# withterm/term

Hardware: AMD Instinct MI355X
Metric: validated rows/sec, 16-col null+range+unique suite (higher is better)
Workload: dtype int64+f64; 1 GPU; 16-col (8 int64 + 8 float64, 12 nullable) null+range+unique suite: completeness x16, min/max/mean x16, uniqueness x2; rows_total=1000000000, rows_per_gpu=1000000000, cols=16, parallelism=row-range shards x1, HSA_ENABLE_IPC_MODE_LEGACY=0, suite_algorithmic_bytes=129500000000, verified=True

## Files before the change

term_amd/csrc/api_internal.h:

```cpp
#pragma once
#include <hip/hip_runtime.h>
#include <math.h>
#include <stdarg.h>
#include <stdio.h>
#include <stdlib.h>
#include <string.h>

#include <algorithm>
#include <atomic>
#include <condition_variable>
#include <mutex>
#include <thread>

#include "internal.h"
#include "kll_device.h"
#include "regex_device.h"
#include "side_check.h"
#include "spearman_device.h"
#include "timegap_device.h"

using namespace tgx;

typedef long double xdouble;
constexpr size_t kArenaBytes = 8u << 20;
constexpr size_t kArenaMaxBuffer = 256u << 10;
constexpr int64_t kCoalesceMaxRows = 1 << 16;
constexpr int64_t kCoalesceFlushRows = 4 << 20;
constexpr size_t kCoalesceFlushBatches = 4096;
constexpr size_t kCoalesceArenaMax = 128u << 20;
constexpr uint32_t kWireMagic = 0x53584754;
constexpr uint32_t kWireVersion = 3;

struct Context {
  std::mutex mu;
  bool inited = false;
  int device = -1;
  int n_cu = 256;
  uint64_t distinct_hint = 0;
  bool no_coalesce = false;
  char arch[64] = {0};
};
extern TGX_HIDDEN Context g_ctx;

struct BatchKeyFacts {
  bool range_known = false;
  int64_t lo = 0, hi = 0;
  bool device_keys = false;
  int64_t data_bytes = -1;
  bool sampled = false;
  DistinctSample sample;
};

struct NumericPrep {
  bool prepared = false;
  bool partitioned = false;
  uint32_t sub_bits = 0;
  bool key16 = false;
  uint64_t n_buckets = 0;
  bool range_known = false;
  int64_t lo = 0, hi = 0;
};

struct BatchTraits {
  bool any_host = false, any_utf8 = false;
  bool any_strings = false;
  bool coalescible = true;
  bool retained = false;
};

struct DistinctTotals {
  uint64_t total = 0, non_null = 0, distinct = 0, twice = 0, empty_rows = 0;
};
static inline void distinct_fold_totals(DistinctState &d, const DistinctTotals &t) {
  d.h_total += t.total;
  d.h_non_null += t.non_null;
  d.h_distinct += t.distinct - (t.empty_rows > 0 ? 1 : 0);
  d.h_twice += t.twice - (t.empty_rows > 1 ? 1 : 0);
  d.h_empty_rows += t.empty_rows;
}
struct Gathered {
  std::vector<ScanAcc> scan;
  std::vector<CountAcc> count;
  std::vector<ComomentAcc> como;
  std::vector<DistinctTotals> distinct;
  std::vector<std::vector<uint8_t>> hll;
};

struct WindowPrep {
  bool ok = true;
  int32_t vb_count = 0;
  int32_t vb_index[kGatherViewBufs];
  int64_t vb_min[kGatherViewBufs], vb_end[kGatherViewBufs];
  bool new_dict = false;
  int64_t dict_first = 0, dict_end = 0;
};

static inline bool is_numeric(int t) { return t == TGX_INT64 || t == TGX_FLOAT64; }
static inline bool is_numeric32(int t) { return t == TGX_INT32 || t == TGX_FLOAT32; }
static inline bool is_narrow_int(int t) { return (t >= TGX_INT8 && t <= TGX_UINT32) || t == TGX_BOOL; }
static inline bool is_widened(int t) { return is_numeric32(t) || is_narrow_int(t); }
static inline bool is_keys_only(int t) { return t == TGX_UINT64 || t == TGX_BOOL; }
static inline size_t narrow_bytes(int t, int64_t slots) {
  switch (t) {
    case TGX_INT8: case TGX_UINT8: return (size_t)slots;
    case TGX_INT16: case TGX_UINT16: return (size_t)slots * 2;
    case TGX_BOOL: return (size_t)((slots + 7) / 8);
    default: return (size_t)slots * 4;
  }
}
static inline int widened_type(int t) { return t == TGX_FLOAT32 ? TGX_FLOAT64 : TGX_INT64; }
static inline int widen_mode(int t) {
  switch (t) {
    case TGX_FLOAT32: return 1;
    case TGX_INT8: return 2;
    case TGX_INT16: return 3;
    case TGX_UINT8: return 4;
    case TGX_UINT16: return 5;
    case TGX_UINT32: return 6;
    case TGX_BOOL: return 7;
    default: return 0;
  }
}
static inline bool is_string(int t) { return t == TGX_UTF8 || t == TGX_LARGE_UTF8; }
static inline bool is_any_string(int t) { return is_string(t) || t == TGX_UTF8_VIEW; }

TGX_HIDDEN void copy_pool_shutdown();
TGX_HIDDEN void coalesce_drop(tgx_state *st);
TGX_HIDDEN ScanAcc scan_acc_identity();
TGX_HIDDEN void host_two_sum(double &s, double &c, double x);
TGX_HIDDEN void scan_acc_merge(ScanAcc &a, const ScanAcc &b);
TGX_HIDDEN xdouble como_sum(const ComomentAcc &a, int k);
TGX_HIDDEN void como_store(ComomentAcc &a, int k, xdouble v);
TGX_HIDDEN void como_rebase(ComomentAcc &b, double px, double py);
TGX_HIDDEN void como_acc_merge(ComomentAcc &a, const ComomentAcc &b_in);
TGX_HIDDEN void state_init_host(tgx_state *st, const tgx_plan *plan);
TGX_HIDDEN void prof_resolve(tgx_state *st);
TGX_HIDDEN tgx_status distinct_totals(tgx_state *st, size_t slot, DistinctTotals *t, tgx_error *err,
                                  const unsigned long long *pre = nullptr);
TGX_HIDDEN tgx_status gather(tgx_state *st, Gathered *g, tgx_error *err);
TGX_HIDDEN double key_to_double(int64_t k);
TGX_HIDDEN double i128_to_double(uint64_t lo, int64_t hi);
TGX_HIDDEN void fill_stats(const ScanAcc &a, bool variance, tgx_result *r);
TGX_HIDDEN double hll_sigma(double x);
TGX_HIDDEN double hll_tau(double x);
TGX_HIDDEN uint64_t hll_estimate(const std::vector<uint8_t> &regs);
TGX_HIDDEN tgx_status stage_column(tgx_state *st, const tgx_column &c, tgx_column *out, tgx_error *err,
                               bool widen32 = true);
TGX_HIDDEN void fill_scan_desc(const tgx_column &c, bool variance, const double *pivot, ScanColDesc *d);
TGX_HIDDEN int scan_blocks_for(const ScanColDesc &d, int n_cols_in_launch, int per_cu = 8);
TGX_HIDDEN tgx_status como_pivots(tgx_state *st, const ComomentLaunch &L, int n_pairs, tgx_error *err);
TGX_HIDDEN tgx_status update_validate(const tgx_plan *plan, tgx_state *st, const tgx_column *columns, size_t n_columns,
                                  int64_t *nrows_out, BatchTraits *traits, tgx_error *err);
TGX_HIDDEN tgx_status update_impl(const tgx_plan *plan, tgx_state *st, const tgx_column *columns, int64_t nrows,
                              tgx_error *err, const std::vector<BatchKeyFacts> *facts = nullptr);
TGX_HIDDEN tgx_status coalesce_append(const tgx_plan *plan, tgx_state *st, const tgx_column *columns, int64_t nrows,
                                  const BatchTraits &traits, bool *taken, tgx_error *err);
TGX_HIDDEN tgx_status distinct_read_counters(tgx_state *st, DistinctState &ds, unsigned long long *out,
                                         tgx_error *err);
TGX_HIDDEN tgx_status distinct_tuple_update(tgx_state *st, size_t slot, const tgx_column *dev, tgx_error *err,
                                        const tgx_column *orig = nullptr);
TGX_HIDDEN tgx_status distinct_prepare_numeric(tgx_state *st, size_t slot, const tgx_column &c,
                                           const BatchKeyFacts &facts, NumericPrep *prep, tgx_error *err);
TGX_HIDDEN tgx_status distinct_update(tgx_state *st, size_t slot, const tgx_column &c, const BatchKeyFacts &facts,
                                  const NumericPrep &prep, tgx_error *err,
                                  const std::vector<DictGather> *gathers = nullptr, int stats_slot = -1,
                                  const tgx_column *orig = nullptr);
TGX_HIDDEN tgx_status pinned_readback(tgx_state *st, size_t bytes, tgx_error *err);
TGX_HIDDEN tgx_status distinct_sample_all(tgx_state *st, const tgx_column *dev, std::vector<BatchKeyFacts> &facts,
                                      tgx_error *err);
TGX_HIDDEN void stream_copy(void *dst, const void *src, size_t bytes);
TGX_HIDDEN void host_minmax_i64_plain(const int64_t *v, const uint8_t *validity, int64_t bit0, int64_t n, int64_t *lo,
                                  int64_t *hi);
TGX_HIDDEN void host_minmax_i64(const int64_t *v, const uint8_t *validity, int64_t bit0, int64_t n, int64_t *lo, int64_t *hi);
TGX_HIDDEN tgx_status coalesce_arena_ready(tgx_state *st, tgx_error *err);
TGX_HIDDEN tgx_status coalesce_prepare_window(const tgx_column &c, int64_t nrows, const CoalesceColumn &cc, int col,
                                          WindowPrep *w, tgx_error *err);
TGX_HIDDEN size_t coalesce_host_bytes(const tgx_plan *plan, const tgx_column *columns, int64_t nrows,
                                  const std::vector<WindowPrep> &prep);
TGX_HIDDEN tgx_status coalesce_release_set(tgx_state *st, int set, tgx_error *err);
```

term_amd/csrc/distinct_state.cpp:

```cpp
#include "api_internal.h"

tgx_status distinct_read_counters(tgx_state *st, DistinctState &ds, unsigned long long *out,
                                         tgx_error *err) {
  memset(out, 0, kNumDistinctCounters * sizeof(unsigned long long));
  if (!ds.counters.p) return TGX_OK;
  HIP_TRY(hipMemcpyAsync(out, ds.counters.p, kNumDistinctCounters * sizeof(unsigned long long),
                         hipMemcpyDeviceToHost, st->stream));
  HIP_TRY(hipStreamSynchronize(st->stream));
  return TGX_OK;
}

tgx_status pinned_readback(tgx_state *st, size_t bytes, tgx_error *err) {
  if (bytes <= st->h_pinned_cap) return TGX_OK;
  pinned_free(st->h_pinned, st->h_pinned_cap);
  st->h_pinned = nullptr;
  st->h_pinned_cap = 0;
  const size_t want = std::max<size_t>(bytes + bytes / 2, 4096);
  HIP_TRY(pinned_alloc(&st->h_pinned, want));
  st->h_pinned_cap = want;
  return TGX_OK;
}

namespace {

// ... 326 lines not shown
  FpLists l1, l2;
  uint32_t *fb_lo = nullptr;
  TGX_TRY(fp_lists_stage(st, ds, c.length, true, &l1, &l2, &fb_lo, err));
  ProfScope ps(st, "distinct", 0), ps_lists(st, "distinct_lists", 0);
  unsigned long long *counters = ds.counters.as<unsigned long long>();
  const Utf8ColDesc d = utf8_desc(kept, kept.variadic, st->plan->fp_key, false);
  launch_fp_partition_utf8(d, l1, fb_lo, counters, st->stream);
  launch_fp_partition_lists(l1, l2, counters, st->stream);
  if (ds.exact)
    launch_fp_count_exact_utf8(l2, mult ? 1 : 0, ds.fp_per_list.as<uint2>(), l1.offered, d, counters, st->stream);
  else
    launch_fp_count(l2, mult ? 1 : 0, ds.fp_per_list.as<uint2>(), l1.offered, counters, st->stream);
  ds.retained.push_back(kept);
  return TGX_OK;
}

tgx_status fp_lists_tuple_update(tgx_state *st, size_t slot, const TupleDesc &d,
                                        const std::vector<const tgx_column *> &cols, tgx_error *err) {
  DistinctState &ds = st->distinct[slot];
  const bool mult = st->plan->distinct[slot].multiplicity;
  FpLists l1, l2;
  uint32_t *fb_lo = nullptr;
  TGX_TRY(fp_lists_stage(st, ds, d.length, true, &l1, &l2, &fb_lo, err));
  ProfScope ps(st, "distinct", 0), ps_lists(st, "distinct_lists", 0);
  unsigned long long *counters = ds.counters.as<unsigned long long>();
  launch_fp_partition_tuples(d, l1, fb_lo, counters, st->stream);
  launch_fp_partition_lists(l1, l2, counters, st->stream);
  if (ds.exact)
    launch_fp_count_exact_tuple(l2, mult ? 1 : 0, ds.fp_per_list.as<uint2>(), d, counters, st->stream);
  else
    launch_fp_count(l2, mult ? 1 : 0, ds.fp_per_list.as<uint2>(), nullptr, counters, st->stream);
  for (const tgx_column *c : cols) ds.retained.push_back(*c);
  return TGX_OK;
}

}

tgx_status distinct_tuple_update(tgx_state *st, size_t slot, const tgx_column *dev, tgx_error *err,
                                        const tgx_column *orig) {
  const DistinctTask &task = st->plan->distinct[slot];
  DistinctState &ds = st->distinct[slot];
  std::vector<const tgx_column *> cols;
  bool any_view = false;
  for (int c2 : task.tuple) {
    cols.push_back(&dev[c2]);
    any_view |= dev[c2].type == TGX_UTF8_VIEW || (orig && is_widened(orig[c2].type));
  }
  TupleDesc d;
  TGX_TRY(tuple_desc_of(st, cols, task.multiplicity, &d, err));
  ds.col_type = TGX_UTF8;
  ds.total_rows += d.length;
  if (d.length == 0) return TGX_OK;
  if (ds.fp_staged) TGX_TRY(distinct_resolve(st, slot, err));
  bool exact_lists_ok = orig != nullptr && d.length < (int64_t)1 << 32;
  if (orig)
    for (int c2 : task.tuple) exact_lists_ok &= orig[c2].mem == TGX_MEM_DEVICE && !is_widened(orig[c2].type);
  if (ds.mode == DistinctMode::kUndecided && !any_view && (!ds.exact || exact_lists_ok) && fp_lists_fit_rows(d.length))
    return fp_lists_tuple_update(st, slot, d, cols, err);
  if (ds.mode == DistinctMode::kUndecided) {
    ds.mode = DistinctMode::kHash;
    ds.wide = true;
  }
  ProfScope ps(st, "distinct", 0);
  return table_insert_tuple(st, slot, d, err);
}

namespace {

void bitmap_shape(const DistinctState &ds, int64_t length, bool mult, uint32_t *sub_bits_out, bool *key16_out,
                         uint64_t *n_buckets_out, bool *partitioned_out) {
  const uint64_t bucket_target = mult ? 1024 : 256;
  uint32_t sub_bits = 14;
  while (sub_bits < (mult ? 19u : 20u) && ((ds.range + (1ull << sub_bits) - 1) >> sub_bits) > bucket_target) sub_bits++;
  const bool key16 = !mult && sub_bits <= 16;
  const uint64_t n_buckets = (ds.range + (1ull << sub_bits) - 1) >> sub_bits;
  uint64_t cap_slots = (uint64_t)length / std::max<uint64_t>(n_buckets, 1);
  cap_slots = cap_slots + cap_slots / 4 + 16 * (((uint64_t)length >> 15) + 1) + 4096;
  *sub_bits_out = sub_bits;
  *key16_out = key16;
  *n_buckets_out = n_buckets;
  const char *min_env = getenv("TGX_PARTITION_MIN_ROWS");
  const int64_t min_rows = min_env ? std::max<int64_t>(1, atoll(min_env)) : (int64_t)1 << 20;
  *partitioned_out = length >= min_rows && n_buckets <= kMaxPartitions && (uint64_t)length * 64 >= ds.range &&
                     cap_slots < (1ull << 32) - 64;
}

bool distinct_wants_sample(const DistinctState &ds, const BatchKeyFacts &facts, const tgx_column &c) {
  return ds.mode == DistinctMode::kUndecided && c.type == TGX_INT64 && !ds.has_hint && !facts.range_known &&
         !ds.remembered && c.length >= (1 << 16);
}
bool distinct_wants_exact_range(const DistinctState &ds, const BatchKeyFacts &facts, const tgx_column &c) {
  if (!facts.device_keys || c.type != TGX_INT64 || ds.has_hint || facts.range_known || c.length < (1 << 16))
    return false;
  return ds.mode == DistinctMode::kUndecided ||
         (ds.mode == DistinctMode::kBitmap && ds.speculative && !ds.partitioned && !ds.outliers_possible);
}

}

tgx_status distinct_sample_all(tgx_state *st, const tgx_column *dev, std::vector<BatchKeyFacts> &facts,
                               tgx_error *err) {
  const tgx_plan *plan = st->plan;
  std::vector<size_t> who;
  for (size_t q = 0; q < plan->distinct.size(); q++) {
    const DistinctTask &t = plan->distinct[q];
    if (!t.tuple.empty() || !is_numeric(dev[t.column].type) || dev[t.column].length == 0) continue;
    bool lane = false;
    for (size_t h = 0; h < plan->hll.size(); h++)
      lane |= plan->hll[h].distinct_slot == (int)q && st->hll_mode[h] == 1;
    if (lane) continue;
    if (distinct_wants_sample(st->distinct[q], facts[q], dev[t.column]) ||
        distinct_wants_exact_range(st->distinct[q], facts[q], dev[t.column]))
      who.push_back(q);
  }
  if (who.empty()) return TGX_OK;
  TGX_TRY(pinned_readback(st, who.size() * sizeof(DistinctSample), err));
  DistinctSample *got = (DistinctSample *)st->h_pinned;
  for (size_t k = 0; k < who.size(); k++) {
    DistinctState &ds = st->distinct[who[k]];
    const tgx_column &c = dev[plan->distinct[who[k]].column];
    DistinctColDesc d = numeric_desc(c, false);
    d.pad = distinct_wants_exact_range(ds, facts[who[k]], c) ? 1 : 0;
    HIP_TRY(ds.sample.reserve(sizeof(DistinctSample)));
    launch_distinct_init(ds.sample.as<DistinctSample>(), nullptr, st->stream);
    launch_distinct_sample(d, ds.sample.as<DistinctSample>(), st->stream);
    HIP_TRY(hipMemcpyAsync(&got[k], ds.sample.p, sizeof(DistinctSample), hipMemcpyDeviceToHost, st->stream));
  }
  HIP_TRY(hipStreamSynchronize(st->stream));
  for (size_t k = 0; k < who.size(); k++) {
    BatchKeyFacts &kf = facts[who[k]];
    if (distinct_wants_exact_range(st->distinct[who[k]], kf, dev[plan->distinct[who[k]].column])) {
      if (got[k].count) {
        kf.range_known = true;
        kf.lo = got[k].min_v;
        kf.hi = got[k].max_v;
      }
      continue;
    }
    kf.sample = got[k];
    kf.sampled = true;
  }
  return TGX_OK;
}

namespace {

tgx_status bitmap_grow(tgx_state *st, DistinctState &ds, bool mult, int64_t lo, int64_t hi, int64_t incoming,
                              tgx_error *err) {
  const uint64_t old_top = (uint64_t)ds.base + (ds.range - 1);
  auto u = [](int64_t v) { return (uint64_t)v ^ 0x8000000000000000ull; };
  const bool below = u(lo) < u(ds.base), above = u(hi) > u((int64_t)old_top);
  if (!below && !above) return TGX_OK;
  constexpr uint64_t kSlice = 1ull << 20;
  uint64_t add_below = 0, add_above = 0;
  if (below) {
    const uint64_t need = u(ds.base) - u(lo);
    add_below = (std::max(need, ds.range) + kSlice - 1) / kSlice * kSlice;
    if (add_below > u(ds.base)) add_below = u(ds.base) / kSlice * kSlice;
    if (add_below < need) return TGX_OK;
  }
  if (above) {
    const uint64_t need = u(hi) - u((int64_t)old_top);
    add_above = std::max(need, ds.range);
    const uint64_t room = 0xFFFFFFFFFFFFFFFFull - u((int64_t)old_top);
    if (add_above > room) add_above = room;
    if (add_above < need) return TGX_OK;
  }
  auto sum3 = [](uint64_t a, uint64_t b, uint64_t c, uint64_t *out) {
    uint64_t t = 0;
    return !__builtin_add_overflow(a, b, &t) && !__builtin_add_overflow(t, c, out);
  };
  uint64_t new_range = 0;
  const bool fits = sum3(ds.range, add_below, add_above, &new_range);
  const uint64_t rows_seen = (uint64_t)std::max<int64_t>(ds.total_rows + incoming, 1);
  if (!fits || new_range >= (1ull << 34) || new_range / 16 > std::max<uint64_t>(rows_seen, g_ctx.distinct_hint)) {
    add_below = below ? ((u(ds.base) - u(lo)) + kSlice - 1) / kSlice * kSlice : 0;
    add_above = above ? u(hi) - u((int64_t)old_top) : 0;
    uint64_t tight = 0;
    if (!sum3(ds.range, add_below, add_above, &tight)) return TGX_OK;
    if (tight >= (1ull << 34) || tight / 16 > std::max<uint64_t>(rows_seen, g_ctx.distinct_hint)) return TGX_OK;
  }
  const uint64_t range = ds.range + add_below + add_above;
  const size_t old_words = (size_t)ds.bitmap_words;
  const size_t words = (size_t)(((range + kSlice - 1) >> 20) << 15) + 4;
  const size_t shift_words = (size_t)(add_below >> 5);
  auto regrow = [&](DevBuf &buf) -> tgx_status {
    DevBuf bigger;
    HIP_TRY(bigger.reserve(words * 4));
    HIP_TRY(hipMemsetAsync(bigger.p, 0, words * 4, st->stream));
    HIP_TRY(hipMemcpyAsync((uint32_t *)bigger.p + shift_words, buf.p, old_words * 4, hipMemcpyDeviceToDevice, st->stream));
    st->parked.emplace_back(std::move(buf));
    buf = std::move(bigger);
    return TGX_OK;
  };
  TGX_TRY(regrow(ds.seen));
  if (mult) TGX_TRY(regrow(ds.twice));
  ds.base = (int64_t)((uint64_t)ds.base - add_below);
  ds.range = range;
  ds.bitmap_words = words - 4;
  return TGX_OK;
}

}

tgx_status distinct_prepare_numeric(tgx_state *st, size_t slot, const tgx_column &c, const BatchKeyFacts &facts,
                                    NumericPrep *prep, tgx_error *err) {
  const DistinctTask &task = st->plan->distinct[slot];
  DistinctState &ds = st->distinct[slot];
  const bool mult = task.multiplicity;
  prep->prepared = true;
  prep->partitioned = false;
  prep->range_known = facts.range_known;
  prep->lo = facts.lo;
  prep->hi = facts.hi;
  if (ds.mode == DistinctMode::kUndecided) {
    bool have_range = false;
    int64_t lo = 0, hi = 0;
    if (c.type == TGX_INT64 && ds.has_hint) {
      have_range = true;
      lo = ds.hint_lo;
      hi = ds.hint_hi;
    } else if (c.type == TGX_INT64 && facts.range_known) {
      have_range = true;
      lo = facts.lo;
      hi = facts.hi;
    } else if (c.type == TGX_INT64 && ds.remembered && c.length >= (1 << 16)) {
      have_range = true;
      lo = ds.remembered_lo;
      hi = ds.remembered_hi;
    } else if (distinct_wants_sample(ds, facts, c)) {
      DistinctSample got = facts.sample;
      if (!facts.sampled) {
        HIP_TRY(ds.sample.reserve(sizeof(DistinctSample)));
        launch_distinct_init(ds.sample.as<DistinctSample>(), nullptr, st->stream);
        launch_distinct_sample(numeric_desc(c, false), ds.sample.as<DistinctSample>(), st->stream);
        HIP_TRY(hipMemcpyAsync(&got, ds.sample.p, sizeof(got), hipMemcpyDeviceToHost, st->stream));
        HIP_TRY(hipStreamSynchronize(st->stream));
      }
      if (got.count == 0 && c.length > 65536) {
        DistinctColDesc d = numeric_desc(c, false);
        d.pad = 1;
        HIP_TRY(ds.sample.reserve(sizeof(DistinctSample)));
        launch_distinct_init(ds.sample.as<DistinctSample>(), nullptr, st->stream);
        launch_distinct_sample(d, ds.sample.as<DistinctSample>(), st->stream);
        HIP_TRY(hipMemcpyAsync(&got, ds.sample.p, sizeof(got), hipMemcpyDeviceToHost, st->stream));
        HIP_TRY(hipStreamSynchronize(st->stream));
      }
      if (got.count == 0) return TGX_OK;
      have_range = true;
      lo = got.min_v;
      hi = got.max_v;
    }
    bool use_bitmap = false;
    if (c.type == TGX_INT64 && have_range) {
      uint64_t width = (uint64_t)hi - (uint64_t)lo;
      uint64_t expect = std::max<uint64_t>((uint64_t)c.length, g_ctx.distinct_hint);
      if (width < (1ull << 34) && width / 16 <= expect) {
        uint64_t slack = ds.has_hint ? 0 : std::min<uint64_t>(width / 64 + 4096, 1ull << 30);
        int64_t base = (lo < INT64_MIN + (int64_t)slack) ? INT64_MIN : lo - (int64_t)slack;
        uint64_t top = (hi > INT64_MAX - (int64_t)slack) ? (uint64_t)INT64_MAX : (uint64_t)(hi + (int64_t)slack);
        ds.base = base;
        ds.range = top - (uint64_t)base + 1;
        use_bitmap = true;
      }
    }
    if (use_bitmap) {
      size_t words = (size_t)(((ds.range + (1u << 20) - 1) >> 20) << 15) + 4;
      ds.bitmap_words = words - 4;
      if (ds.seen.cap < words * 4 && ds.spare_seen.cap >= words * 4) std::swap(ds.seen, ds.spare_seen);
      if (ds.twice.cap < words * 4 && ds.spare_twice.cap >= words * 4) std::swap(ds.twice, ds.spare_twice);
      HIP_TRY(ds.seen.reserve(words * 4));
      HIP_TRY(hipMemsetAsync(ds.seen.p, 0, words * 4, st->stream));
      if (mult) {
        HIP_TRY(ds.twice.reserve(words * 4));
        HIP_TRY(hipMemsetAsync(ds.twice.p, 0, words * 4, st->stream));
      }
      ds.mode = DistinctMode::kBitmap;
      ds.speculative = !ds.has_hint;
      if (ds.speculative && !facts.range_known) {
        ds.remembered = true;
        ds.remembered_lo = lo;
        ds.remembered_hi = hi;
      }
    } else {
      ds.mode = DistinctMode::kHash;
      ds.remembered = false;
    }
  }
  if (ds.mode == DistinctMode::kBitmap && ds.speculative && !ds.partitioned && facts.range_known &&
      !ds.outliers_possible)
    TGX_TRY(bitmap_grow(st, ds, mult, facts.lo, facts.hi, c.length, err));
  if (ds.mode == DistinctMode::kBitmap && ds.speculative) {
    auto u = [](int64_t v) { return (uint64_t)v ^ 0x8000000000000000ull; };
    const bool covered = facts.range_known && u(facts.lo) >= u(ds.base) && u(facts.hi) - u(ds.base) < ds.range;
    if (!covered) ds.outliers_possible = true;
  }
  if (ds.mode == DistinctMode::kBitmap) {
    bitmap_shape(ds, c.length, mult, &prep->sub_bits, &prep->key16, &prep->n_buckets, &prep->partitioned);
    if (ds.partitioned) prep->partitioned = false;
  }
  return TGX_OK;
}

namespace {

tgx_status distinct_run_numeric(tgx_state *st, size_t slot, const tgx_column &c, const NumericPrep &prep,
                                       int stats_slot, tgx_error *err, const tgx_column *orig) {
  const DistinctTask &task = st->plan->distinct[slot];
  const tgx_column &keep = (orig && orig->mem == TGX_MEM_DEVICE && is_widened(orig->type)) ? *orig : c;
  DistinctState &ds = st->distinct[slot];
  const bool mult = task.multiplicity;
  const DistinctColDesc d = numeric_desc(c, mult);
  const uint64_t bytes = (uint64_t)c.length * 8 + (c.validity ? (uint64_t)(c.length + 7) / 8 : 0);
  if (ds.mode == DistinctMode::kUndecided) return TGX_OK;
  if (ds.mode == DistinctMode::kBitmap) {
    if (ds.speculative) ds.retained.push_back(keep);
    if (prep.partitioned) {
      PartitionParams pp;
      memset(&pp, 0, sizeof(pp));
      pp.values = c.values;
      pp.validity = c.validity;
      pp.offset = c.offset;
      pp.length = c.length;
      pp.base = ds.base;
      pp.range = ds.range;
      pp.sub_bits = prep.sub_bits;
      pp.n_buckets = (uint32_t)prep.n_buckets;
      const uint64_t tiles = ((uint64_t)c.length + kPartitionTile - 1) / kPartitionTile;
      pp.bucket0 = 0;
      pp.n_lists = pp.n_buckets;
      if (prep.range_known) {
        auto u = [](int64_t v) { return (uint64_t)v ^ 0x8000000000000000ull; };
        const uint64_t ub = u(ds.base);
        const uint64_t rlo = u(prep.lo) > ub ? u(prep.lo) - ub : 0;
        uint64_t rhi = u(prep.hi) > ub ? u(prep.hi) - ub : 0;
        rhi = std::min(rhi, ds.range - 1);
        if (rlo <= rhi) {
          pp.bucket0 = (uint32_t)(rlo >> pp.sub_bits);
          pp.n_lists = (uint32_t)(rhi >> pp.sub_bits) - pp.bucket0 + 1;
        }
      }
      const char *p20 = getenv("TGX_PACK20");
      const bool no_pack20 = p20 && atoi(p20) == 0;
      const bool pack20 = !prep.key16 && prep.sub_bits <= (mult ? 19u : 20u) && !no_pack20;
      uint64_t cap = (uint64_t)c.length / pp.n_lists;
      cap = cap + cap / 4 + (prep.key16 ? 32 : pack20 ? 24 : 16) * tiles + 4096;
      pp.cap = prep.key16 ? (cap + 31) & ~31ull : pack20 ? (cap + 23) / 24 * 24 : (cap + 15) & ~15ull;
      if (pp.cap >= (1ull << 32) - 64) return fail(err, TGX_INTERNAL, "distinct: list capacity out of range");
      pp.want_multiplicity = mult ? 1 : 0;
      pp.key16 = prep.key16 ? 1 : pack20 ? 2 : 0;
      pp.force_form = ds.remembered_form;
      HIP_TRY(ds.lists.reserve(prep.key16 ? (uint64_t)pp.n_lists * pp.cap * sizeof(uint16_t)
                               : pack20   ? (uint64_t)pp.n_lists * pp.cap / 3 * 8
                                          : (uint64_t)pp.n_lists * pp.cap * sizeof(uint32_t)));
      HIP_TRY(ds.cursors.reserve((2 * pp.n_buckets + 1) * sizeof(unsigned long long)));
      pp.lists = ds.lists.as<uint32_t>();
      pp.cursors = ds.cursors.as<unsigned long long>();
      pp.seen = ds.seen.as<uint32_t>();
      pp.twice = mult ? ds.twice.as<uint32_t>() : nullptr;
      const int grid = partition_grid(c.length, g_ctx.n_cu);
      if (stats_slot >= 0) {
        HIP_TRY(ds.stat_partials.reserve((size_t)(grid + 1) * sizeof(ScanPartial)));
        HIP_TRY(ds.outlier_stats.reserve(sizeof(OutlierStats)));
        pp.stats = ds.stat_partials.as<ScanPartial>();
        pp.outliers = ds.outlier_stats.as<OutlierStats>();
      }
      unsigned long long *cnt = ds.counters.as<unsigned long long>();
      static_assert(kCntDistinct == 0 && kCntTwice == 1, "partition_init_kernel clears the two totals together");
      launch_partition_init(pp, cnt + kCntDistinct, st->stream);
      {
        ProfScope ps(st, "distinct", bytes);
        launch_partition(pp, cnt, g_ctx.n_cu, st->stream);
        HIP_TRY(launch_bucket_apply(pp, cnt, st->stream));
      }
      if (stats_slot >= 0) {
        ScanLaunch L;
        memset(&L, 0, sizeof(L));
        L.cols[0].length = c.length;
        L.cols[0].is_float = 0;
        L.acc_index[0] = stats_slot;
        launch_scan_reduce_only(L, 1, grid, pp.stats, st->d_scan_acc.as<ScanAcc>(), st->stream, pp.outliers);
      }
    } else {
      ProfScope ps(st, "distinct", bytes);
      launch_distinct_bitmap(d, bitmap_view(ds), ds.counters.as<unsigned long long>(), st->stream);
    }
  } else {
    if (ds.fp_staged) TGX_TRY(distinct_resolve(st, slot, err));
    if (ds.capacity == 0 && fp_lists_fit(c)) {
      FpLists l1, l2;
      uint32_t *fb_lo = nullptr;
      TGX_TRY(fp_lists_stage(st, ds, c.length, false, &l1, &l2, &fb_lo, err));
      ProfScope ps(st, "distinct", bytes), ps_lists(st, "distinct_lists", 0);
      launch_key_lists(d, l1, l2, mult ? 1 : 0, ds.fp_per_list.as<uint2>(), ds.counters.as<unsigned long long>(),
                       st->stream);
      ds.retained.push_back(keep);
      return TGX_OK;
    }
    TGX_TRY(hash_ensure(st, ds, mult, (uint64_t)c.length, err));
    ProfScope ps(st, "distinct", bytes);
    launch_distinct_hash(d, hash_view(ds), ds.counters.as<unsigned long long>(), st->stream);
  }
  return TGX_OK;
}

tgx_status retained_numeric_view(tgx_state *st, const tgx_column &col, std::vector<std::unique_ptr<DevBuf>> &tmp,
                                        tgx_column *out, tgx_error *err) {
  *out = col;
  if (!is_widened(col.type)) return TGX_OK;
  const int64_t e0 = col.offset & ~(int64_t)63;
  const int64_t slots = col.offset - e0 + col.length;
  tmp.emplace_back(new DevBuf());
  DevBuf *w = tmp.back().get();
  HIP_TRY(w->reserve((size_t)slots * 8 + 16));
  launch_widen32((const uint8_t *)col.values + narrow_bytes(col.type, e0), w->p, slots, widen_mode(col.type), g_ctx.n_cu,
                 st->stream);
  out->type = widened_type(col.type);
  out->values = w->p;
  out->validity = col.validity ? col.validity + (e0 >> 3) : nullptr;
  out->offset = col.offset - e0;
  return TGX_OK;
}

}

tgx_status distinct_update(tgx_state *st, size_t slot, const tgx_column &c, const BatchKeyFacts &facts,
                           const NumericPrep &prep, tgx_error *err, const std::vector<DictGather> *gathers,
                           int stats_slot, const tgx_column *orig) {
  const DistinctTask &task = st->plan->distinct[slot];
  DistinctState &ds = st->distinct[slot];
  const bool mult = task.multiplicity;
  if (is_any_string(c.type)) {
    ds.col_type = c.type;
    ds.total_rows += c.length;
    if (c.length == 0) return TGX_OK;
    if (ds.fp_staged) TGX_TRY(distinct_resolve(st, slot, err));
    const bool exact_lists_ok = orig && orig->mem == TGX_MEM_DEVICE && c.length < (int64_t)1 << 32;
    if (ds.mode == DistinctMode::kUndecided && (!ds.exact || exact_lists_ok) && fp_lists_fit(c))
      return fp_lists_update(st, slot, c, err);
    if (ds.mode == DistinctMode::kUndecided) {
      ds.mode = DistinctMode::kHash;
      ds.wide = true;
    }
    ProfScope ps(st, "distinct", 0);
    return table_insert_utf8(st, slot, c, facts.data_bytes, err);
  }
  if (c.type == TGX_DICT32_UTF8) {
    const tgx_column &dict = *c.dictionary;
    ds.col_type = c.type;
    ds.total_rows += c.length;
    if (c.length == 0 || dict.length == 0) return TGX_OK;
    if (ds.mode == DistinctMode::kUndecided) {
      ds.mode = DistinctMode::kHash;
      ds.wide = true;
    }
    TGX_TRY(hash_ensure(st, ds, mult, (uint64_t)std::min<int64_t>(c.length, dict.length), err));
    const size_t uw = dict_usage_words(dict.length);
    HIP_TRY(ds.dict_usage.reserve(2 * uw * 4 + 16));
    const size_t scratch = dict_usage_scratch_bytes(c.length, dict.length, mult ? 1 : 0, g_ctx.n_cu);
    if (scratch)
      HIP_TRY(ds.dict_scratch.reserve(scratch));
    else
      HIP_TRY(hipMemsetAsync(ds.dict_usage.p, 0, 2 * uw * 4, st->stream));
    uint32_t *u_seen = ds.dict_usage.as<uint32_t>(), *u_twice = u_seen + uw;
    ProfScope ps(st, "distinct", 0);
    if (gathers && !gathers->empty() && scratch) {
      const uint8_t *hits[4];
      unsigned long long *pc[4];
      int32_t niv[4];
      const int k = (int)std::min<size_t>(gathers->size(), 4);
      for (int i = 0; i < k; i++) {
        hits[i] = (*gathers)[i].hits;
        pc[i] = (*gathers)[i].counters;
        niv[i] = (*gathers)[i].null_is_valid;
      }
      launch_dict_usage_fused((const int32_t *)c.values, c.validity, c.offset, c.length, dict.length, mult ? 1 : 0, k,
                              hits, pc, niv, u_seen, u_twice, ds.dict_scratch.as<uint32_t>(),
                              ds.counters.as<unsigned long long>(), g_ctx.n_cu, st->stream);
    } else {
      launch_dict_usage((const int32_t *)c.values, c.validity, c.offset, c.length, dict.validity, dict.offset,
                        dict.length, mult ? 1 : 0, u_seen, u_twice, ds.dict_scratch.as<uint32_t>(),
                        ds.counters.as<unsigned long long>(), g_ctx.n_cu, st->stream);
    }
    if (ds.exact) TGX_TRY(key_store_reserve_utf8(st, ds, dict, u_seen, facts.data_bytes, err));
    launch_dict_insert(utf8_desc(dict, nullptr, st->plan->fp_key, mult), u_seen, u_twice, hash_view(ds),
                       ds.counters.as<unsigned long long>(), st->stream);
    return TGX_OK;
  }
  if (!is_numeric(c.type))
    return fail(err, TGX_UNSUPPORTED, "DISTINCT on column type %d is not supported yet", c.type);
  ds.col_type = c.type;
  ds.total_rows += c.length;
  if (c.length == 0) return TGX_OK;
  NumericPrep ready = prep;
  if (!ready.prepared) TGX_TRY(distinct_prepare_numeric(st, slot, c, facts, &ready, err));
  return distinct_run_numeric(st, slot, c, ready, stats_slot, err, orig);
}

tgx_status tgx::distinct_resolve(tgx_state *st, size_t slot, tgx_error *err) {
  DistinctState &ds = st->distinct[slot];
  std::vector<std::unique_ptr<DevBuf>> widened;
  if (ds.fp_staged && st->device_ready) {
    const bool mult = st->plan->distinct[slot].multiplicity;
    unsigned long long c[kNumDistinctCounters];
    TGX_TRY(distinct_read_counters(st, ds, c, err));
    ds.fp_staged = false;
    const bool exact_lists = ds.fp_exact_lists;
    ds.fp_exact_lists = false;
    if (c[kCntOutOfRange] != 0 || (exact_lists && !ds.retained.empty())) {
      if (ds.retained.empty())
        return fail(err, TGX_INTERNAL, "distinct: overflowed fingerprint lists and no batch to redo");
      HIP_TRY(hipMemsetAsync(ds.counters.p, 0, kNumDistinctCounters * sizeof(unsigned long long), st->stream));
      const DistinctTask &task = st->plan->distinct[slot];
      if (!task.tuple.empty()) {
        std::vector<const tgx_column *> cols;
        for (const tgx_column &col : ds.retained) cols.push_back(&col);
        TupleDesc d;
        TGX_TRY(tuple_desc_of(st, cols, mult, &d, err));
        TGX_TRY(table_insert_tuple(st, slot, d, err));
      } else {
        for (const tgx_column &kept : ds.retained) {
          tgx_column col;
          TGX_TRY(retained_numeric_view(st, kept, widened, &col, err));
          if (ds.wide) {
            TGX_TRY(table_insert_utf8(st, slot, col, -1, err));
            continue;
          }
          TGX_TRY(hash_ensure(st, ds, mult, (uint64_t)col.length, err));
          launch_distinct_hash(numeric_desc(col, mult), hash_view(ds), ds.counters.as<unsigned long long>(), st->stream);
        }
      }
    } else if (exact_lists) {
      FpLists l1, l2;
      fp_views(ds, &l1, &l2);
      TGX_TRY(hash_ensure(st, ds, mult, c[kCntDistinct], err));
      unsigned long long cur = 0;
      HIP_TRY(hipMemcpyAsync(&cur, ds.key_cursor.p, sizeof(cur), hipMemcpyDeviceToHost, st->stream));
      HIP_TRY(hipStreamSynchronize(st->stream));
      TGX_TRY(key_store_ensure(st, ds, cur, 2 * (c[kCntDistinct] + 1), err));
      ds.key_words_ub = cur + 2 * (c[kCntDistinct] + 1);
      TGX_TRY(key_store_measure_begin(st, ds, (uint64_t)kFpFan * kFpFan * l2.cap, err));
      HIP_TRY(hipMemsetAsync(ds.counters.p, 0, 2 * sizeof(unsigned long long), st->stream));
      launch_fp_demote(l2, ds.fp_fb_lo.as<uint32_t>(), hash_view(ds), mult ? 1 : 0, ds.counters.as<unsigned long long>(),
                       st->stream);
    } else {
      FpLists l1, l2;
      fp_views(ds, &l1, &l2);
      TGX_TRY(hash_ensure(st, ds, mult, c[kCntDistinct], err));
      if (ds.wide)
        launch_fp_insert(l2, hash_view(ds), mult ? 1 : 0, st->stream);
      else
        launch_key_insert(l2, hash_view(ds), mult ? 1 : 0, st->stream);
    }
    HIP_TRY(hipStreamSynchronize(st->stream));
    ds.retained.clear();
    return TGX_OK;
  }
  if (!ds.speculative || ds.retained.empty() || !st->device_ready) {
    ds.retained.clear();
    return TGX_OK;
  }
  const bool mult = st->plan->distinct[slot].multiplicity;
  unsigned long long c[kNumDistinctCounters];
  TGX_TRY(distinct_read_counters(st, ds, c, err));
  const uint64_t n_out = c[kCntOutOfRange];
  if (n_out == 0 || ds.mode != DistinctMode::kBitmap) {
    ds.retained.clear();
    ds.outliers_possible = false;
    return TGX_OK;
  }
  const int64_t old_base = ds.base;
  const uint64_t old_range = ds.range;
  ds.remembered = false;
  TGX_TRY(bitmap_to_hash(st, ds, mult, n_out, err));
  TGX_TRY(hash_ensure(st, ds, mult, n_out, err));
  for (const tgx_column &kept : ds.retained) {
    tgx_column col;
    TGX_TRY(retained_numeric_view(st, kept, widened, &col, err));
    launch_distinct_outliers(numeric_desc(col, mult), old_base, old_range, hash_view(ds), ds.counters.as<unsigned long long>(), st->stream);
  }
  HIP_TRY(hipMemsetAsync(ds.counters.as<unsigned long long>() + kCntOutOfRange, 0, sizeof(unsigned long long), st->stream));
  HIP_TRY(hipStreamSynchronize(st->stream));
  ds.retained.clear();
  ds.speculative = false;
  return TGX_OK;
}

tgx_status tgx::distinct_resolve_all(tgx_state *st, tgx_error *err) {
  bool pending = false;
  for (auto &ds : st->distinct) pending |= (ds.speculative || ds.fp_staged) && !ds.retained.empty();
  if (!pending || !st->device_ready || !st->d_distinct_counters.p) {
    for (auto &ds : st->distinct) ds.retained.clear();
    return TGX_OK;
  }
  std::vector<unsigned long long> all(st->distinct.size() * kNumDistinctCounters);
  TGX_TRY(pinned_readback(st, all.size() * sizeof(unsigned long long), err));
  HIP_TRY(hipMemcpyAsync(st->h_pinned, st->d_distinct_counters.p, all.size() * sizeof(unsigned long long),
                         hipMemcpyDeviceToHost, st->stream));
  HIP_TRY(hipStreamSynchronize(st->stream));
  memcpy(all.data(), st->h_pinned, all.size() * sizeof(unsigned long long));
  for (size_t k = 0; k < st->distinct.size(); k++) {
    DistinctState &ds = st->distinct[k];
    if ((ds.speculative || ds.fp_staged) && !ds.retained.empty() &&
        (all[k * kNumDistinctCounters + kCntOutOfRange] != 0 || (ds.fp_staged && ds.fp_exact_lists)))
      TGX_TRY(distinct_resolve(st, k, err));
    else {
      ds.retained.clear();
      ds.outliers_possible = false;
    }
  }
  return TGX_OK;
}


namespace {
uint32_t host_owner_of(uint64_t key, uint32_t world) {
  uint64_t x = key ^ 0x9e3779b97f4a7c15ULL;
  x ^= x >> 30; x *= 0xbf58476d1ce4e5b9ULL; x ^= x >> 27; x *= 0x94d049bb133111ebULL; x ^= x >> 31;
  return (uint32_t)((x >> 32) % world);
}
}

tgx_status tgx::distinct_export_impl(tgx_state *st, size_t slot, uint32_t world,
                                       const void **device_records, uint64_t *counts, tgx_error *err) {
  TGX_TRY(coalesce_flush(st, err));
  DistinctState &ds = st->distinct[slot];
  const bool mult = st->plan->distinct[slot].multiplicity;
  TGX_TRY(state_init_device(st, err));
  TGX_TRY(distinct_resolve(st, slot, err));
  std::vector<unsigned long long> h_counts(world, 0);
  unsigned long long c[kNumDistinctCounters];
  TGX_TRY(distinct_read_counters(st, ds, c, err));
  const uint64_t empty_rows = c[kCntEmptyRows];
  HIP_TRY(ds.export_counts.reserve(2 * world * sizeof(unsigned long long)));
  unsigned long long *d_counts = ds.export_counts.as<unsigned long long>();
  unsigned long long *d_cursors = d_counts + world;
  HIP_TRY(hipMemsetAsync(d_counts, 0, 2 * world * sizeof(unsigned long long), st->stream));
  if (ds.mode == DistinctMode::kHash && ds.wide)
    launch_hash_export_count128(hash_view(ds), world, d_counts, st->stream);
  else if (ds.mode == DistinctMode::kHash)
    launch_hash_export_count(hash_view(ds), world, d_counts, st->stream);
  else if (ds.mode == DistinctMode::kBitmap)
    launch_bitmap_export_count(bitmap_view(ds), world, d_counts, st->stream);
  HIP_TRY(hipMemcpyAsync(h_counts.data(), d_counts, world * sizeof(unsigned long long), hipMemcpyDeviceToHost, st->stream));
  HIP_TRY(hipStreamSynchronize(st->stream));
  uint32_t empty_owner = 0;
  if (empty_rows > 0) {
    empty_owner = host_owner_of(kEmptyKey, world);
    h_counts[empty_owner] += 1;
  }
  std::vector<unsigned long long> starts(world, 0);
  uint64_t total = 0;
  for (uint32_t r = 0; r < world; r++) {
    starts[r] = total;
    total += h_counts[r];
  }
  const size_t rec_bytes = ds.wide ? sizeof(KeyRecord128) : sizeof(KeyRecord);
  HIP_TRY(ds.export_records.reserve(std::max<uint64_t>(total, 1) * rec_bytes));
  HIP_TRY(hipMemcpyAsync(d_cursors, starts.data(), world * sizeof(unsigned long long), hipMemcpyHostToDevice, st->stream));
  HIP_TRY(hipStreamSynchronize(st->stream));
  if (ds.mode == DistinctMode::kHash && ds.wide)
    launch_hash_export_scatter128(hash_view(ds), world, mult ? 1 : 0, d_cursors, ds.export_records.as<KeyRecord128>(),
                                  st->stream);
  else if (ds.mode == DistinctMode::kHash)
    launch_hash_export_scatter(hash_view(ds), world, mult ? 1 : 0, d_cursors, ds.export_records.as<KeyRecord>(), st->stream);
  else if (ds.mode == DistinctMode::kBitmap)
    launch_bitmap_export_scatter(bitmap_view(ds), world, mult ? 1 : 0, d_cursors, ds.export_records.as<KeyRecord>(), st->stream);
  if (empty_rows > 0) {
    KeyRecord rec{kEmptyKey, std::min<uint64_t>(empty_rows, 2)};
    uint64_t pos = starts[empty_owner] + h_counts[empty_owner] - 1;
    HIP_TRY(hipMemcpyAsync(ds.export_records.as<KeyRecord>() + pos, &rec, sizeof(rec), hipMemcpyHostToDevice, st->stream));
  }
  HIP_TRY(hipStreamSynchronize(st->stream));
  for (uint32_t r = 0; r < world; r++) counts[r] = h_counts[r];
  *device_records = ds.export_records.p;
  return TGX_OK;
}

extern "C" size_t tgx_distinct_record_bytes(const tgx_plan *plan, const tgx_state *st, size_t spec_index) {
  if (!plan || !st || st->plan != plan || spec_index >= plan->specs.size() ||
      plan->specs[spec_index].kind != TGX_CHECK_DISTINCT)
    return 0;
  return records_are_wide(st->distinct[plan->bind[spec_index].slot]) ? sizeof(KeyRecord128) : sizeof(KeyRecord);
}

extern "C" tgx_status tgx_distinct_export(const tgx_plan *plan, tgx_state *st, size_t spec_index,
                                          uint32_t world, const void **device_records, uint64_t *counts,
                                          tgx_error *err) try {
  bind_thread();
  size_t slot = 0;
  TGX_TRY(spec_slot(plan, st, spec_index, TGX_CHECK_DISTINCT, "DISTINCT", &slot, err));
  if (world == 0 || world > 256 || !device_records || !counts)
    return fail(err, TGX_INVALID_ARGUMENT, "bad arguments (world must be 1..256)");
  TGX_TRY(need_device(err));
  return distinct_export_impl(st, slot, world, device_records, counts, err);
} catch (...) {
  return tgx::abi_exception(err);
}

tgx_status tgx::distinct_import_records(tgx_state *st, size_t slot, const void *d_recs, uint64_t n, bool wide,
                                          tgx_error *err) {
  DistinctState &ds = st->distinct[slot];
  const bool mult = st->plan->distinct[slot].multiplicity;
  TGX_TRY(state_init_device(st, err));
  TGX_TRY(distinct_resolve(st, slot, err));
  if (ds.mode == DistinctMode::kBitmap) TGX_TRY(bitmap_to_hash(st, ds, mult, n, err));
  if (ds.mode == DistinctMode::kHash && ds.capacity > 0 && ds.wide != wide)
    return fail(err, TGX_INVALID_ARGUMENT, "distinct: cannot unite a Utf8 key set with a numeric one");
  ds.mode = DistinctMode::kHash;
  ds.wide = wide;
  TGX_TRY(hash_ensure(st, ds, mult, n, err));
  if (ds.exact && wide) {
    unsigned long long cur = 0;
    HIP_TRY(hipMemcpyAsync(&cur, ds.key_cursor.p, sizeof(cur), hipMemcpyDeviceToHost, st->stream));
    HIP_TRY(hipStreamSynchronize(st->stream));
    TGX_TRY(key_store_ensure(st, ds, cur, 2 * n, err));
    ds.key_words_ub = cur + 2 * n;
    TGX_TRY(key_store_measure_begin(st, ds, n, err));
  }
  if (wide)
    launch_hash_import128((const KeyRecord128 *)d_recs, n, hash_view(ds), mult ? 1 : 0,
                          ds.counters.as<unsigned long long>(), st->stream);
  else
    launch_hash_import((const KeyRecord *)d_recs, n, hash_view(ds), mult ? 1 : 0,
                       ds.counters.as<unsigned long long>(), st->stream);
  return TGX_OK;
}

tgx_status tgx::distinct_replace_by_records(tgx_state *st, size_t slot, const void *d_recs, uint64_t n, bool wide,
                                            tgx_error *err) {
  DistinctState &ds = st->distinct[slot];
  static_assert(kCntDistinct == 0 && kCntTwice == 1 && kCntEmptyRows == 2, "the three totals of the keys lie together");
  HIP_TRY(hipMemsetAsync(ds.counters.as<unsigned long long>() + kCntDistinct, 0, 3 * sizeof(unsigned long long),
                         st->stream));
  ds.capacity = 0;
  ds.rows_upper_bound = 0;
  ds.mode = DistinctMode::kHash;
  ds.wide = wide;
  TGX_TRY(distinct_import_records(st, slot, d_recs, n, wide, err));
  ds.partitioned = true;
  return TGX_OK;
}

extern "C" tgx_status tgx_distinct_import(const tgx_plan *plan, tgx_state *st, size_t spec_index,
                                          const void *device_records, uint64_t n_records, tgx_error *err) try {
  bind_thread();
  size_t slot = 0;
  TGX_TRY(spec_slot(plan, st, spec_index, TGX_CHECK_DISTINCT, "DISTINCT", &slot, err));
  TGX_TRY(need_device(err));
  TGX_TRY(coalesce_flush(st, err));
  DistinctState &ds = st->distinct[slot];
  TGX_TRY(state_init_device(st, err));
  const bool wide = records_are_wide(ds);
  HIP_TRY(hipStreamSynchronize(st->stream));
  ds.seen.release();
  ds.twice.release();
  ds.keys.release();
  ds.dup.release();
  static_assert(kCntValidRows + 1 == kCntOutOfRange, "the words behind the row counter");
  HIP_TRY(hipMemsetAsync(ds.counters.as<unsigned long long>() + kCntOutOfRange, 0,
                         (kNumDistinctCounters - kCntOutOfRange) * sizeof(unsigned long long), st->stream));
  TGX_TRY(distinct_replace_by_records(st, slot, device_records, n_records, wide, err));
  HIP_TRY(hipStreamSynchronize(st->stream));
  return TGX_OK;
} catch (...) {
  return tgx::abi_exception(err);
}

extern "C" tgx_status tgx_distinct_range_hint(const tgx_plan *plan, tgx_state *st, size_t spec_index, int64_t lo,
                                              int64_t hi, tgx_error *err) try {
  size_t slot = 0;
  TGX_TRY(spec_slot(plan, st, spec_index, TGX_CHECK_DISTINCT, "DISTINCT", &slot, err));
  TGX_TRY(coalesce_flush(st, err));
  DistinctState &ds = st->distinct[slot];
  if (ds.mode != DistinctMode::kUndecided)
    return fail(err, TGX_INVALID_ARGUMENT, "range hint must be given before the first batch (after tgx_state_reset)");
  if (hi < lo) return fail(err, TGX_INVALID_ARGUMENT, "range hint: hi < lo");
  ds.has_hint = true;
  ds.hint_lo = lo;
  ds.hint_hi = hi;
  return TGX_OK;
} catch (...) {
  return tgx::abi_exception(err);
}

extern "C" tgx_status tgx_distinct_bitmap_view(const tgx_plan *plan, tgx_state *st, size_t spec_index, int64_t *base,
                                               uint64_t *n_words, const void **seen, const void **twice,
                                               tgx_error *err) try {
  bind_thread();
  size_t slot = 0;
  TGX_TRY(spec_slot(plan, st, spec_index, TGX_CHECK_DISTINCT, "DISTINCT", &slot, err));
  TGX_TRY(coalesce_flush(st, err));
  TGX_TRY(distinct_resolve(st, slot, err));
  DistinctState &ds = st->distinct[slot];
  if (ds.mode != DistinctMode::kBitmap)
    return fail(err, TGX_UNSUPPORTED, "the key set is not a range bitmap; use tgx_distinct_export / _import");
  HIP_TRY(hipStreamSynchronize(st->stream));
  if (base) *base = ds.base;
  if (n_words) *n_words = ds.bitmap_words;
// ... 59 lines not shown
```

term_amd/csrc/internal.h:

```cpp
#pragma once
#include <hip/hip_runtime.h>
#include <stdint.h>
#include <stdio.h>

#include <atomic>
#include <deque>
#include <map>
#include <memory>
#include <new>
#include <stdexcept>
#include <string>
#include <vector>

#include "../../include/tgx.h"
#include "kernels/device_types.h"
#include "kernels/distinct_types.h"
#include "kll_host.h"

namespace tgx {

inline tgx_status abi_exception(tgx_error *err) {
  tgx_status code = TGX_INTERNAL;
  const char *what = "unknown C++ exception";
  try {
    throw;
  } catch (const std::bad_alloc &) {
    code = TGX_OUT_OF_MEMORY;
    what = "host allocation failed (std::bad_alloc)";
  } catch (const std::exception &e) {
    what = e.what();
  } catch (...) {
  }
  if (err) {
    err->code = (int32_t)code;
    snprintf(err->msg, sizeof(err->msg), "%s", what);
  }
  return code;
}

void launch_scan_pivot(const ScanLaunch &L, int n_cols, double *d_pivots, int32_t *d_pivot_set, PivotSearch *d_search,
                       hipStream_t stream);
void launch_scan_main_only(const ScanLaunch &L, int n_cols, int blocks_per_col, ScanPartial *d_partials,
                           ScanAcc *d_accs, hipStream_t stream);
void launch_scan_kll(const ScanLaunch &L, int n_cols, int blocks_per_col, size_t lds_bytes, ScanPartial *d_partials,
                     hipStream_t stream);
void launch_scan_pairs(const ScanPairLaunch &L, int n_pairs, int blocks_per_pair, size_t lds_bytes,
                       ScanPartial *d_partials, void *d_como_partials, const ComomentAcc *d_como_accs,
                       hipStream_t stream);
void launch_scan_hll(const ScanLaunch &L, int n_cols, int blocks_per_col, ScanPartial *d_partials, hipStream_t stream);
void launch_como_pivot(const ComomentLaunch &L, int n_pairs, ComomentAcc *d_accs, PivotSearch *d_search, hipStream_t stream);
void launch_comoments_reduce(const ComomentLaunch &L, int n_pairs, int blocks_per_pair, const void *d_partials,
                             ComomentAcc *d_accs, hipStream_t stream);
void launch_widen32(const void *src, void *dst, int64_t n, int mode, int n_cu, hipStream_t stream);
void launch_scan_reduce_only(const ScanLaunch &L, int n_cols, int blocks_per_col, ScanPartial *d_partials,
                             ScanAcc *d_accs, hipStream_t stream, const OutlierStats *outliers = nullptr);
void launch_count(const CountLaunch &L, int n_cols, int blocks_per_col, unsigned long long *d_block_counts,
                  CountAcc *d_accs, hipStream_t stream);
size_t comoments_partial_bytes();
void launch_comoments(const ComomentLaunch &L, int n_pairs, int blocks_per_pair, void *d_partials,
                      ComomentAcc *d_accs, hipStream_t stream);
void launch_distinct_hash(const DistinctColDesc &d, const HashSetView &t,
                          unsigned long long *d_counters, hipStream_t stream);
void launch_distinct_bitmap(const DistinctColDesc &d, const BitmapView &bm,
                            unsigned long long *d_counters, hipStream_t stream);
int partition_grid(int64_t length, int n_cu);
void launch_distinct_init(DistinctSample *sample, OutlierStats *outliers, hipStream_t stream);
void launch_partition_init(const PartitionParams &p, unsigned long long *totals, hipStream_t stream);
void launch_distinct_sample(const DistinctColDesc &d, DistinctSample *out, hipStream_t stream);
void launch_distinct_outliers(const DistinctColDesc &d, int64_t base, uint64_t range, const HashSetView &t,
                              unsigned long long *d_counters, hipStream_t stream);
void launch_partition(const PartitionParams &p, unsigned long long *d_counters, int n_cu, hipStream_t stream);
hipError_t launch_bucket_apply(const PartitionParams &p, unsigned long long *d_counters, hipStream_t stream);
void launch_bitmap_adopt(const uint32_t *seen_slices, const uint32_t *twice_slices, uint32_t n_slices,
                         uint64_t slice_words, uint64_t stride_words, uint32_t *out_seen, uint32_t *out_twice,
                         unsigned long long *d_counters, hipStream_t stream);
void launch_bitmap_rebase(const uint32_t *src, uint64_t src_words, long long delta_bits, uint32_t world,
                          uint64_t slice_words, uint64_t row_words, uint64_t col_words, uint32_t *send,
                          hipStream_t stream);
void launch_distinct_utf8(const Utf8ColDesc &d, const HashSetView &t, unsigned long long *d_counters,
                          hipStream_t stream);
void launch_exact_measure_utf8(const Utf8ColDesc &d, const uint32_t *dict_seen, unsigned long long *out,
                               hipStream_t stream);
void launch_exact_measure_tuple(const TupleDesc &d, unsigned long long *out, hipStream_t stream);
void launch_gather_segments(const GatherSeg *d_segs, int n_segs, int parts, hipStream_t stream);
void launch_state_reset(const StateResetArgs &a, hipStream_t stream);
int tgx_num_cus();
void launch_dict_count_hits(const int32_t *indices, const uint8_t *validity, int64_t offset, int64_t length,
                            int64_t dict_length, int dict_has_nulls, const uint8_t *hits, int null_is_valid,
                            unsigned long long *d_counters, int n_cu, hipStream_t stream);
void launch_dict_count(const int32_t *indices, const uint8_t *validity, int64_t offset, int64_t length,
                       const uint8_t *dict_validity, int64_t dict_offset, int64_t dict_length, CountAcc *acc, int n_cu,
                       hipStream_t stream);
int dict_fuse_capacity(int64_t length, int64_t dict_length, int want_mult, int n_cu);
void launch_dict_usage_fused(const int32_t *indices, const uint8_t *validity, int64_t offset, int64_t length,
                             int64_t dict_length, int want_mult, int n_patterns, const uint8_t *const *hits,
                             unsigned long long *const *pattern_counters, const int32_t *null_is_valid, uint32_t *seen,
                             uint32_t *twice, uint32_t *scratch, unsigned long long *d_counters, int n_cu,
                             hipStream_t stream);
size_t dict_usage_words(int64_t dict_length);
size_t dict_usage_scratch_bytes(int64_t length, int64_t dict_length, int want_mult, int n_cu);
void launch_dict_usage(const int32_t *indices, const uint8_t *validity, int64_t offset, int64_t length,
                       const uint8_t *dict_validity, int64_t dict_offset, int64_t dict_length, int want_mult,
                       uint32_t *seen, uint32_t *twice, uint32_t *scratch, unsigned long long *d_counters, int n_cu,
                       hipStream_t stream);
void launch_dict_insert(const Utf8ColDesc &d, const uint32_t *seen, const uint32_t *twice, const HashSetView &t,
                        unsigned long long *d_counters, hipStream_t stream);
void launch_distinct_tuple(const TupleDesc &d, const HashSetView &t, unsigned long long *d_counters,
                           hipStream_t stream);
void launch_fp_partition_utf8(const Utf8ColDesc &d, const FpLists &level1, uint32_t *exact_fb_lo,
                              unsigned long long *d_counters, hipStream_t stream);
void launch_fp_partition_tuples(const TupleDesc &d, const FpLists &level1, uint32_t *exact_fb_lo,
                                unsigned long long *d_counters, hipStream_t stream);
void launch_fp_count_exact_utf8(const FpLists &level2, int want_mult, uint2 *per_list, const uint32_t *offered1,
                                const Utf8ColDesc &d, unsigned long long *d_counters, hipStream_t stream);
void launch_fp_count_exact_tuple(const FpLists &level2, int want_mult, uint2 *per_list, const TupleDesc &d,
                                 unsigned long long *d_counters, hipStream_t stream);
void launch_fp_demote(const FpLists &level2, const uint32_t *fb_lo, const HashSetView &t, int want_mult,
                      unsigned long long *d_counters, hipStream_t stream);
void launch_fp_partition_lists(const FpLists &level1, const FpLists &level2, unsigned long long *d_counters,
                               hipStream_t stream);
void launch_fp_count(const FpLists &level2, int want_mult, uint2 *per_list, const uint32_t *offered1,
                     unsigned long long *d_counters, hipStream_t stream);
void launch_fp_insert(const FpLists &level2, const HashSetView &t, int want_mult, hipStream_t stream);
void launch_key_lists(const DistinctColDesc &d, const FpLists &level1, const FpLists &level2, int want_mult,
                      uint2 *per_list, unsigned long long *d_counters, hipStream_t stream);
void launch_key_insert(const FpLists &level2, const HashSetView &t, int want_mult, hipStream_t stream);
void launch_hash_rehash128(const HashSetView &src, const HashSetView &dst, int want_mult,
                           unsigned long long *d_counters, hipStream_t stream);
void launch_hash_import128(const KeyRecord128 *recs, uint64_t n, const HashSetView &dst, int want_mult,
                           unsigned long long *d_counters, hipStream_t stream);
void launch_hash_export_count128(const HashSetView &src, uint32_t world, unsigned long long *d_counts,
                                 hipStream_t stream);
void launch_hash_export_scatter128(const HashSetView &src, uint32_t world, int want_mult,
                                   unsigned long long *d_cursors, KeyRecord128 *out, hipStream_t stream);
void launch_hash_rehash(const HashSetView &src, const HashSetView &dst, int want_mult,
                        unsigned long long *d_counters, hipStream_t stream);
void launch_bitmap_to_hash(const BitmapView &bm, const HashSetView &dst, int want_mult,
                           unsigned long long *d_counters, hipStream_t stream);
void launch_hash_import(const KeyRecord *recs, uint64_t n, const HashSetView &dst, int want_mult,
                        unsigned long long *d_counters, hipStream_t stream);
void launch_hash_export_count(const HashSetView &src, uint32_t world, unsigned long long *d_counts,
                              hipStream_t stream);
void launch_hash_export_scatter(const HashSetView &src, uint32_t world, int want_mult,
                                unsigned long long *d_cursors, KeyRecord *out, hipStream_t stream);
void launch_bitmap_export_count(const BitmapView &bm, uint32_t world, unsigned long long *d_counts,
                                hipStream_t stream);
void launch_bitmap_export_scatter(const BitmapView &bm, uint32_t world, int want_mult,
                                  unsigned long long *d_cursors, KeyRecord *out, hipStream_t stream);

struct ScanTask {
  int column;
  bool variance;
  bool stats_needed = false;
  bool stats_spec = false;
  bool read_by_spec = false;
};
struct CountTask {
  int column;
};
struct DistinctTask {
  int column;
  bool multiplicity;
  int scan_slot;
  std::vector<int> tuple;
  bool approx_only = false;
  bool exact = false;
};
struct HllTask {
  int column;
  int scan_slot;
  int distinct_slot;
};
struct ComomentTask {
  int col_x, col_y;
};
struct KllTask {
  int column;
  uint32_t k;
};
struct JointTask {
  int col_x, col_y;
  bool binned;
  JointBinning binning;
};
struct TemporalTask {
  int column, column2, spec_index;
  bool set;
  uint32_t flags;
  TemporalParams params;
};
struct HistTask {
  int column;
  bool counted = false;
  std::vector<double> edges;
  uint32_t buckets() const { return counted ? (uint32_t)edges.size() - 1 : 0; }
};

struct ValueRuleTask {
  int column, spec_index, slot, leader;
  bool set;
  tgx_value_rule_params params;
};

struct ValueCountsTask {
  int column, spec_index;
  bool set;
  tgx_value_counts_params params;
};

struct PairCountsTask {
  int col_x, col_y, spec_index;
  bool set;
  tgx_pair_counts_params params;
};

constexpr int kGroupMaxTuple = 8;
struct GroupCountsTask {
  int column, group, spec_index, slot, leader, member;
  int n_tuple;
  int tuple[kGroupMaxTuple];
  bool set;
  tgx_group_counts_params params;
};

struct GroupSumsTask {
  int column, group, spec_index;
  int n_tuple;
  int tuple[kGroupMaxTuple];
  bool set;
  tgx_group_sums_params params;
};

enum KeyProbeMode : uint32_t {
  kKpPlain = 0, kKpCounted = 1, kKpStrings = 2, kKpRows = 3, kKpStringsCounted = 4, kKpRowsStrings = 5,
  kKpTuples = 6, kKpTuplesCounted = 7, kKpRowsTuples = 8
};
inline bool kp_string_set(KeyProbeMode m) { return m == kKpStrings || m == kKpStringsCounted; }
inline bool kp_counts(KeyProbeMode m) { return m == kKpCounted || m == kKpStringsCounted || m == kKpTuplesCounted; }
inline bool kp_gathers(KeyProbeMode m) { return m == kKpRows || m == kKpRowsStrings || m == kKpRowsTuples; }
inline bool kp_string_column(KeyProbeMode m) { return kp_string_set(m) || m == kKpRowsStrings; }
inline bool kp_tuples(KeyProbeMode m) { return m == kKpTuples || m == kKpTuplesCounted || m == kKpRowsTuples; }
inline bool kp_tuple_set(KeyProbeMode m) { return m == kKpTuples || m == kKpTuplesCounted; }
inline bool kp_fingerprint_set(KeyProbeMode m) { return kp_string_set(m) || kp_tuple_set(m); }
constexpr int kKeyProbeMaxTuple = 8;
struct KeyProbeTask {
  int column, spec_index;
  int n_tuple;
  int tuple[kKeyProbeMaxTuple];
  bool set;
  KeyProbeMode mode;
  uint32_t max_value_bytes;
  tgx_key_probe_params params;
};

constexpr int kRowPredicateMaxCols = 8;
struct RowPredicateTask {
  int spec_index;
  int n_columns;
  int columns[kRowPredicateMaxCols];
  bool set;
  tgx_row_predicate_params params;
};

struct TypeClassesTask {
  int column, spec_index;
};

struct SideCheck;
constexpr int kNumSide = 11;

enum class Source { kScan, kCount };

struct SpecBinding {
  int kind;
  int slot;
  Source count_src;
};

}

struct tgx_plan {
  std::vector<tgx_check_spec> specs;
  std::vector<std::string> patterns;
  std::vector<tgx::SpecBinding> bind;
  std::vector<tgx::ScanTask> scan;
  std::vector<tgx::CountTask> count;
  std::vector<tgx::DistinctTask> distinct;
  std::vector<tgx::ComomentTask> como;
  std::vector<tgx::KllTask> kll;
  std::vector<tgx::HllTask> hll;
  std::vector<tgx::JointTask> joint;
  std::vector<tgx::TemporalTask> temporal;
  std::vector<tgx::HistTask> hist;
  std::vector<tgx::ValueRuleTask> rules;
  std::vector<tgx::ValueCountsTask> value_counts;
  std::vector<tgx::PairCountsTask> pair_counts;
  std::vector<tgx::GroupCountsTask> group_counts;
  std::vector<tgx::GroupSumsTask> group_sums;
  std::vector<tgx::KeyProbeTask> key_probes;
  std::vector<tgx::RowPredicateTask> row_predicates;
  std::vector<tgx::TypeClassesTask> type_classes;
  int n_columns_needed = 0;
  std::vector<char> used, reads_values, needs_wide;
  std::vector<char> key_column;
  std::vector<char> side_on[tgx::kNumSide];
  std::vector<char> stats_on;
  tgx::FpKey fp_key;
  mutable std::atomic<bool> fp_key_locked{false};
  void *regex = nullptr;
  void *spearman = nullptr;
  void *timegap = nullptr;
  std::vector<char> timegap_on;
};

namespace tgx {

size_t cache_size_class(size_t bytes);
hipError_t dev_alloc(void **p, size_t *cap, size_t bytes);
void dev_free(void *p, size_t cap);
hipError_t pinned_alloc(void **p, size_t bytes);
void pinned_free(void *p, size_t bytes);
hipError_t stream_acquire(hipStream_t *out, bool high_priority);
void stream_release(hipStream_t s, bool high_priority);
void dev_cache_trim();
void dev_cache_set_live(bool on);
void dev_cache_stats(tgx_cache_stats *out);
struct QuiescedScope {
  QuiescedScope();
  ~QuiescedScope();
  QuiescedScope(const QuiescedScope &) = delete;
  QuiescedScope &operator=(const QuiescedScope &) = delete;
};

struct DevBuf {
  void *p = nullptr;
  size_t cap = 0;
  bool owned = true;
  DevBuf() = default;
  DevBuf(const DevBuf &) = delete;
  DevBuf &operator=(const DevBuf &) = delete;
  DevBuf(DevBuf &&o) noexcept : p(o.p), cap(o.cap), owned(o.owned) {
    o.p = nullptr;
    o.cap = 0;
    o.owned = true;
  }
  DevBuf &operator=(DevBuf &&o) noexcept {
    if (this != &o) {
      release();
      p = o.p;
      cap = o.cap;
      owned = o.owned;
      o.p = nullptr;
      o.cap = 0;
      o.owned = true;
    }
    return *this;
  }
  ~DevBuf() { release(); }
  void release() {
    if (p && owned) dev_free(p, cap);
    p = nullptr;
    cap = 0;
    owned = true;
  }
  void borrow(void *ptr, size_t bytes) {
    release();
    p = ptr;
    cap = bytes;
    owned = false;
  }
  hipError_t reserve(size_t bytes) {
    if (bytes <= cap) return hipSuccess;
    release();
    return dev_alloc(&p, &cap, bytes);
  }
// ... 309 lines not shown
```

term_amd/csrc/kernels/distinct_types.h:

```cpp
#pragma once
#include <stdint.h>

namespace tgx {

constexpr uint64_t kEmptyKey = 0xFFFFFFFFFFFFFFFFULL;

struct DistinctColDesc {
  const void *values;
  const uint8_t *validity;
  int64_t offset;
  int64_t length;
  int32_t want_multiplicity;
  int32_t pad;
};

struct HashSetView {
  uint64_t *keys;
  uint32_t *dup;
  uint64_t mask;
  uint64_t *store;
  unsigned long long *store_cursor;
  uint64_t store_words;
  uint64_t *pending;
  uint32_t *pending_counts;
  uint64_t pending_region;
  uint32_t pending_waves, pad_;
};
inline uint32_t exact_blocks(uint64_t items) {
  uint64_t blocks = (items + 255) / 256;
  if (blocks < 1) blocks = 1;
  if (blocks > 2048) blocks = 2048;
  return (uint32_t)blocks;
}
inline uint32_t exact_waves(uint64_t items) { return exact_blocks(items) * 4; }
inline uint64_t exact_region(uint64_t items) {
  const uint64_t threads = (uint64_t)exact_blocks(items) * 256;
  return (items + threads - 1) / threads * 64;
}

struct FpKey {
  uint32_t k[4], k1[4], k2[4];
};
inline void fp_key_times_two(const uint32_t in[4], uint32_t out[4]) {
  const uint32_t carry = (in[3] >> 31) ? 0x87u : 0u;
  out[3] = (in[3] << 1) | (in[2] >> 31);
  out[2] = (in[2] << 1) | (in[1] >> 31);
  out[1] = (in[1] << 1) | (in[0] >> 31);
  out[0] = (in[0] << 1) ^ carry;
}
inline FpKey fp_key_expand(const uint32_t k[4]) {
  FpKey key;
  for (int i = 0; i < 4; i++) key.k[i] = k[i];
  fp_key_times_two(key.k, key.k1);
  fp_key_times_two(key.k1, key.k2);
  return key;
}

struct Utf8ColDesc {
  const void *offsets;
  const uint8_t *data;
  const uint8_t *validity;
  int64_t offset;
  int64_t length;
  int32_t large_offsets;
  int32_t want_multiplicity;
  const void *views;
  const uint8_t *const *buffers;
  FpKey key;
};

struct BitmapView {
  uint32_t *seen;
  uint32_t *twice;
  int64_t base;
  uint64_t range;
};

constexpr uint32_t kMaxPartitions = 2048;
constexpr uint32_t kListPad = 0xFFFFFFFFu;
constexpr int kRunPad4 = 16, kRunPad2 = 32;
constexpr int kPartitionThreads = 1024;
constexpr int kPartitionKeysPerThread = 32;
constexpr int kPartitionTile = kPartitionThreads * kPartitionKeysPerThread;
constexpr int kSliceWordsLds = 32768;

struct PartitionParams {
  const void *values;
  const uint8_t *validity;
  int64_t offset;
  int64_t length;
  int64_t base;
  uint64_t range;
  uint32_t sub_bits;
  uint32_t n_buckets;
  uint64_t cap;
  uint32_t *lists;
  unsigned long long *cursors;
  uint32_t *seen;
  uint32_t *twice;
  int32_t want_multiplicity;
  int32_t key16;
  struct ScanPartial *stats;
  struct OutlierStats *outliers;
  uint32_t bucket0, n_lists;
  int32_t force_form;
};

struct OutlierStats {
  long long mn, mx;
  unsigned long long lo32_sum;
  long long hi32_sum;
  unsigned long long count;
};

struct DistinctSample {
  int64_t min_v, max_v;
  unsigned long long count;
  unsigned long long pad;
};

struct KeyRecord {
  uint64_t key;
  uint64_t count;
};

struct KeyRecord128 {
  uint64_t a, b;
  uint64_t count;
  uint64_t pad;
};

constexpr int kFpFan = 256;
constexpr int kFpXcds = 8;
constexpr int kFpTile = 2048;
constexpr uint32_t kFpSlots = 4096;
constexpr uint32_t kFpListMax = 24576;
constexpr int64_t kFpMinRows = 1 << 21;
struct FpLists {
  uint64_t *recs;
  uint32_t *offered;
  uint64_t cap;
};

enum {
  kCntDistinct = 0,
  kCntTwice = 1,
  kCntEmptyRows = 2,
  kCntValidRows = 3,
  kCntOutOfRange = 4,
  kCntSpare = 5,
  kCntStoreFull = 6,
  kCntForm = 7,
  kNumDistinctCounters = 8
};

struct TupleCol {
  int32_t kind;
  int32_t dict_large;
  const void *values;
  const void *offsets;
  const uint8_t *data;
  const uint8_t *const *buffers;
  const uint8_t *validity;
  int64_t offset;
  const uint8_t *dict_validity;
  int64_t dict_offset;
};
constexpr int kMaxTupleCols = 8;
struct TupleDesc {
  TupleCol cols[kMaxTupleCols];
  int32_t n_cols;
  int32_t want_multiplicity;
  int64_t length;
  FpKey key;
};
struct KeyProbeTupleDesc {
  TupleDesc d;
  int64_t dict_length[kMaxTupleCols];
};

}
```

term_amd/csrc/kernels/partition.hip:

```cpp
#include <hip/hip_runtime.h>

#include <type_traits>

#include "device_types.h"
#include "distinct_types.h"
#include "keyset_device.h"

namespace tgx {

template <int THREADS, int KPT, bool VALIDITY>
__device__ __forceinline__ void partition_load_tile(const PartitionParams &p, int64_t tile, bool wide,
                                                    int64_t (&key)[KPT], uint32_t &ok) {
  constexpr int kPartitionThreads = THREADS;
  constexpr int kTile = kPartitionThreads * KPT;
  global_i64_ptr vals = (global_i64_ptr)(uintptr_t)((const int64_t *)p.values + p.offset);
  global_u8_ptr vbits = VALIDITY ? (global_u8_ptr)(uintptr_t)p.validity : (global_u8_ptr) nullptr;
  const uint32_t tid = threadIdx.x;
  const int64_t row0 = tile * kTile;
  const bool full = row0 + kTile <= p.length;
  ok = 0;
  if (full && wide) {
    typedef long long i64x2 __attribute__((ext_vector_type(2)));
    typedef const i64x2 __attribute__((address_space(1))) *global_i64x2_ptr;
    global_i64x2_ptr pv = (global_i64x2_ptr)(vals + row0) + tid;
    const bool pair_bytes = vbits && (p.offset & 1) == 0;
    ok = (uint32_t)((1ull << KPT) - 1ull);
    if (pair_bytes) {
      uint8_t vb[KPT / 2];
#pragma unroll
      for (int j = 0; j < KPT / 2; j++) {
        const int64_t bit = p.offset + row0 + (int64_t)j * 2 * kPartitionThreads + 2 * tid;
        vb[j] = vbits[bit >> 3];
      }
      ok = 0;
#pragma unroll
      for (int j = 0; j < KPT / 2; j++) {
        const int64_t bit = p.offset + row0 + (int64_t)j * 2 * kPartitionThreads + 2 * tid;
        ok |= (uint32_t)((vb[j] >> (bit & 7)) & 3) << (2 * j);
      }
    } else if (vbits) {
      ok = 0;
#pragma unroll
      for (int j = 0; j < KPT; j++) {
        const int64_t bit = p.offset + row0 + (int64_t)(j / 2) * 2 * kPartitionThreads + 2 * tid + (j & 1);
        ok |= (uint32_t)TGX_VALID_BIT(vbits, bit) << j;
      }
    }
    if (VALIDITY) asm volatile("" : "+v"(ok));
#pragma unroll
    for (int j = 0; j < KPT / 2; j++) {
      i64x2 v = pv[(int64_t)j * kPartitionThreads];
      key[2 * j] = v.x;
      key[2 * j + 1] = v.y;
    }
  } else {
#pragma unroll
    for (int j = 0; j < KPT; j++) {
      const int64_t i = row0 + (int64_t)j * kPartitionThreads + tid;
      const bool in = i < p.length;
      key[j] = vals[in ? i : p.length - 1];
      bool valid = in;
      if (in && vbits) {
        const int64_t bit = p.offset + i;
        valid = TGX_VALID_BIT(vbits, bit);
      }
      ok |= (uint32_t)valid << j;
    }
  }
}

template <int THREADS, int KPT, int MAXP, int PAD, bool KEY16, bool PACK20, bool CLUSTERED, class MidFn, class StoreFn>
__device__ __forceinline__ void partition_process_tile(const PartitionParams &p, uint32_t *sorted, uint32_t *hist,
                                                       uint32_t *toff, uint32_t *gbase, uint32_t *wave_sums,
                                                       uint32_t *long_runs, const uint32_t (&rel)[KPT], uint64_t ok,
                                                       MidFn &&mid,
                                                       StoreFn &&before_stores) {
  constexpr uint32_t NW = THREADS / 64;
  constexpr int BPT = MAXP / THREADS;
  constexpr int NS = MAXP / (NW * 64);
  static_assert(MAXP % THREADS == 0 && MAXP % (NW * 64) == 0 && PAD % 4 == 0, "shape");
  constexpr uint32_t RPAD = PACK20 ? 24u : KEY16 ? (uint32_t)kRunPad2 : (uint32_t)PAD;
  auto pad_up = [](uint32_t h) -> uint32_t { return PACK20 ? (h + 23u) / 24u * 24u : (h + (RPAD - 1u)) & ~(RPAD - 1u); };
  const bool fill = p.want_multiplicity != 0;
  auto pack6 = [&](uint32_t o, uint32_t h, uint32_t i) -> uint4 {
    uint64_t w[2];
    if (!fill) {
#pragma unroll
      for (int q = 0; q < 2; q++) {
        const uint32_t i0 = i + 3u * q;
        const uint64_t a = sorted[o + (i0 < h ? i0 : h - 1)], b = sorted[o + (i0 + 1 < h ? i0 + 1 : h - 1)],
                       c = sorted[o + (i0 + 2 < h ? i0 + 2 : h - 1)];
        w[q] = a | (b << 20) | (c << 40);
      }
    } else {
#pragma unroll
      for (int q = 0; q < 2; q++) {
        uint64_t e[3];
#pragma unroll
        for (uint32_t j = 0; j < 3; j++) {
          const uint32_t at = i + 3u * q + j;
          e[j] = at < h ? (uint64_t)sorted[o + at] : 0xFFFFFull;
        }
        w[q] = e[0] | (e[1] << 20) | (e[2] << 40);
      }
    }
    return make_uint4((uint32_t)w[0], (uint32_t)(w[0] >> 32), (uint32_t)w[1], (uint32_t)(w[1] >> 32));
  };
  const uint32_t tid = threadIdx.x;
  const uint32_t lane = tid & 63, wave = tid >> 6;
  const uint32_t sub_mask = (uint32_t)((1ull << p.sub_bits) - 1);
  for (uint32_t b = tid; b < (uint32_t)MAXP; b += THREADS) hist[b] = 0;
  constexpr uint32_t kLongRun = 1024, kMaxLongRuns = THREADS * KPT / kLongRun;
  if (CLUSTERED && tid == 0) long_runs[kMaxLongRuns] = 0;
  __syncthreads();
  bool whole = false;
  if (CLUSTERED) {
    uint32_t agreed = 0;
#pragma unroll
    for (int j = 0; j < KPT; j++) {
      const bool okj = (ok >> j) & 1;
      const uint32_t b = rel[j] >> p.sub_bits;
      const uint64_t act = __ballot(okj);
      const uint32_t first = act ? (uint32_t)__builtin_ctzll(act) : 0u;
      const uint32_t b0 = (uint32_t)__builtin_amdgcn_readlane((int)b, (int)first);
      agreed |= (__ballot(okj && b != b0) == 0 ? 1u : 0u) << j;
    }
    whole = agreed == (uint32_t)((1ull << KPT) - 1ull);
  }
  if (CLUSTERED && whole) {
#pragma unroll
    for (int j = 0; j < KPT; j++) {
      const uint64_t act = __ballot((ok >> j) & 1);
      const uint32_t first = act ? (uint32_t)__builtin_ctzll(act) : 64u;
      if (lane == first) atomicAdd(&hist[rel[j] >> p.sub_bits], (uint32_t)__builtin_popcountll(act));
    }
  } else {
#pragma unroll
    for (int j = 0; j < KPT; j++)
      if ((ok >> j) & 1) atomicAdd(&hist[rel[j] >> p.sub_bits], 1u);
  }
  __syncthreads();
  {
    uint32_t h[BPT], sum = 0;
#pragma unroll
    for (int k = 0; k < BPT; k++) {
      h[k] = hist[BPT * tid + k];
      sum += h[k];
    }
    uint32_t incl = sum;
#pragma unroll
    for (int d = 1; d < 64; d <<= 1) {
      uint32_t up = __shfl_up(incl, d, 64);
      if (lane >= (uint32_t)d) incl += up;
    }
    if (lane == 63) wave_sums[wave] = incl;
    __syncthreads();
    uint32_t excl = incl - sum;
    for (uint32_t w = 0; w < wave; w++) excl += wave_sums[w];
#pragma unroll
    for (int k = 0; k < BPT; k++) {
      const uint32_t b = BPT * tid + k;
      toff[b] = excl;
      hist[b] = excl;
      uint32_t g = 0;
      if (h[k] && b - p.bucket0 >= p.n_lists) {
        g = 0xFFFFFFFFu;
      } else if (h[k]) {
        const unsigned long long padded = pad_up(h[k]);
        const unsigned long long at = atomicAdd(&p.cursors[b], padded);
        if (at + padded > p.cap) {
          atomicMin(&p.cursors[p.n_buckets + b], at);
          g = 0xFFFFFFFFu;
        } else {
          g = (uint32_t)at;
          if (CLUSTERED && h[k] >= kLongRun) long_runs[atomicAdd(&long_runs[kMaxLongRuns], 1u)] = b;
        }
      }
      gbase[b] = g;
      excl += h[k];
    }
    if (tid == THREADS - 1) toff[MAXP] = excl;
  }
  __syncthreads();
  __builtin_amdgcn_sched_barrier(0);
  mid();
  __builtin_amdgcn_sched_barrier(0);
  if (CLUSTERED && whole) {
#pragma unroll
    for (int j = 0; j < KPT; j++) {
      const bool okj = (ok >> j) & 1;
      const uint64_t act = __ballot(okj);
      const uint32_t first = act ? (uint32_t)__builtin_ctzll(act) : 64u;
      uint32_t at = 0;
      if (lane == first) at = atomicAdd(&hist[rel[j] >> p.sub_bits], (uint32_t)__builtin_popcountll(act));
      at = (uint32_t)__builtin_amdgcn_readlane((int)at, (int)(first & 63u));
      const uint32_t before =
          __builtin_amdgcn_mbcnt_hi((uint32_t)(act >> 32), __builtin_amdgcn_mbcnt_lo((uint32_t)act, 0u));
      if (okj) sorted[at + before] = rel[j] & sub_mask;
    }
  } else {
#pragma unroll
    for (int j = 0; j < KPT; j++) {
      if (!((ok >> j) & 1)) continue;
      const uint32_t pos = atomicAdd(&hist[rel[j] >> p.sub_bits], 1u);
      sorted[pos] = rel[j] & sub_mask;
    }
  }
  __syncthreads();
  __builtin_amdgcn_sched_barrier(0);
  before_stores();
  __builtin_amdgcn_sched_barrier(0);
  {
    uint32_t m_o[NS], m_h[NS], m_g[NS];
#pragma unroll
    for (int s2 = 0; s2 < NS; s2++) {
      const uint32_t b = (lane + 64 * s2) * NW + wave;
      const bool in = b < p.n_buckets;
      const uint32_t o = in ? toff[b] : 0;
      m_o[s2] = o;
      m_h[s2] = in ? toff[b + 1] - o : 0;
      m_g[s2] = in ? gbase[b] : 0;
    }
    const uint32_t n_meta = (p.n_buckets > wave) ? (p.n_buckets - wave + NW - 1) / NW : 0;
    constexpr uint32_t LPB = (KEY16 || PACK20) ? 4u : 16u, BPS = 64u / LPB, KPL = PACK20 ? 6u : KEY16 ? 8u : 4u;
    const uint32_t grp = lane / LPB, sub = lane % LPB;
#pragma unroll
    for (int s2 = 0; s2 < NS; s2++) {
      const uint32_t m_end = n_meta > 64u * s2 ? (n_meta - 64u * s2 < 64u ? n_meta - 64u * s2 : 64u) : 0;
      for (uint32_t m0 = 0; m0 < m_end; m0 += BPS) {
        const uint32_t m = m0 + grp, src = m & 63;
        const uint32_t o = __shfl(m_o[s2], src, 64), g = __shfl(m_g[s2], src, 64);
        uint32_t h = __shfl(m_h[s2], src, 64);
        if (m >= m_end) h = 0;
        if (CLUSTERED && h >= kLongRun && g != 0xFFFFFFFFu) h = 0;
        if (h == 0) continue;
        const uint32_t b = (m + 64 * s2) * NW + wave;
        if (g != 0xFFFFFFFFu) {
          const uint32_t padded = pad_up(h);
          if (PACK20) {
            uint8_t *dst = (uint8_t *)p.lists + ((uint64_t)(b - p.bucket0) * p.cap + g) / 3 * 8;
            for (uint32_t i = KPL * sub; i < padded; i += KPL * LPB) *(uint4 *)(dst + (uint64_t)(i / 3) * 8) = pack6(o, h, i);
          } else if (KEY16) {
            uint16_t *dst = (uint16_t *)p.lists + (uint64_t)(b - p.bucket0) * p.cap + g;
            for (uint32_t i = KPL * sub; i < padded; i += KPL * LPB) {
              uint32_t k8[8];
#pragma unroll
              for (uint32_t j = 0; j < 8; j++) k8[j] = sorted[o + (i + j < h ? i + j : h - 1)];
              uint4 v;
              v.x = k8[0] | (k8[1] << 16);
              v.y = k8[2] | (k8[3] << 16);
              v.z = k8[4] | (k8[5] << 16);
              v.w = k8[6] | (k8[7] << 16);
              *(uint4 *)&dst[i] = v;
            }
          } else {
            uint32_t *dst = p.lists + (uint64_t)(b - p.bucket0) * p.cap + g;
            for (uint32_t i = KPL * sub; i < padded; i += KPL * LPB) {
              uint4 v;
              v.x = i < h ? sorted[o + i] : kListPad;
              v.y = i + 1 < h ? sorted[o + i + 1] : kListPad;
              v.z = i + 2 < h ? sorted[o + i + 2] : kListPad;
              v.w = i + 3 < h ? sorted[o + i + 3] : kListPad;
              *(uint4 *)&dst[i] = v;
            }
          }
        } else {
          for (uint32_t i = sub; i < h; i += LPB) {
            const uint64_t r = ((uint64_t)b << p.sub_bits) | sorted[o + i];
            const uint32_t bit = 1u << (r & 31);
            const uint32_t prev = atomicOr(&p.seen[r >> 5], bit);
            if ((prev & bit) && p.want_multiplicity) atomicOr(&p.twice[r >> 5], bit);
          }
        }
      }
    }
  }
  if (CLUSTERED) {
    const uint32_t n_long = long_runs[kMaxLongRuns];
    for (uint32_t q = 0; q < n_long; q++) {
      const uint32_t b = long_runs[q];
      const uint32_t o = toff[b], h = toff[b + 1] - o, g = gbase[b];
      const uint32_t padded = pad_up(h);
      if (PACK20) {
        uint8_t *dst = (uint8_t *)p.lists + ((uint64_t)(b - p.bucket0) * p.cap + g) / 3 * 8;
        for (uint32_t i = 6u * tid; i < padded; i += 6u * THREADS) *(uint4 *)(dst + (uint64_t)(i / 3) * 8) = pack6(o, h, i);
      } else if (KEY16) {
        uint16_t *dst = (uint16_t *)p.lists + (uint64_t)(b - p.bucket0) * p.cap + g;
        for (uint32_t i = 8u * tid; i < padded; i += 8u * THREADS) {
          uint32_t k8[8];
#pragma unroll
          for (uint32_t j = 0; j < 8; j++) k8[j] = sorted[o + (i + j < h ? i + j : h - 1)];
          uint4 v;
          v.x = k8[0] | (k8[1] << 16);
          v.y = k8[2] | (k8[3] << 16);
          v.z = k8[4] | (k8[5] << 16);
          v.w = k8[6] | (k8[7] << 16);
          *(uint4 *)&dst[i] = v;
        }
      } else {
        uint32_t *dst = p.lists + (uint64_t)(b - p.bucket0) * p.cap + g;
        for (uint32_t i = 4u * tid; i < padded; i += 4u * THREADS) {
          uint4 v;
          v.x = i < h ? sorted[o + i] : kListPad;
          v.y = i + 1 < h ? sorted[o + i + 1] : kListPad;
          v.z = i + 2 < h ? sorted[o + i + 2] : kListPad;
          v.w = i + 3 < h ? sorted[o + i + 3] : kListPad;
          *(uint4 *)&dst[i] = v;
        }
      }
    }
  }
  __syncthreads();
}

template <int G>
__device__ __forceinline__ bool merge_word_group(uint32_t cw, uint32_t &cb) {
  const uint32_t lane = threadIdx.x & 63;
#pragma unroll
  for (int d = 1; d < G; d <<= 1) {
    const uint32_t ow = __shfl_xor(cw, d, 64), ob = __shfl_xor(cb, d, 64);
    if (ow == cw) cb |= ob;
  }
  const uint32_t lead = lane & ~(uint32_t)(G - 1);
  const uint64_t agree = __ballot(cw == (uint32_t)__shfl(cw, (int)lead, 64));
  const bool whole = ((agree >> lead) & ((1ull << G) - 1)) == ((1ull << G) - 1);
  return !whole || lane == lead;
}

template <int KPT>
__device__ __forceinline__ void partition_relative(const PartitionParams &p, const int64_t (&key)[KPT],
                                                   uint32_t (&rel)[KPT], uint32_t &outm) {
  outm = 0;
#pragma unroll
  for (int j = 0; j < KPT; j++) {
    const uint64_t r = (uint64_t)key[j] - (uint64_t)p.base;
    outm |= (r >= p.range ? 1u : 0u) << j;
    rel[j] = (uint32_t)r;
    asm volatile("" : "+v"(rel[j]));
  }
  __builtin_amdgcn_sched_barrier(0);
}

template <int KPT, bool STATS>
__device__ __forceinline__ void partition_relative_plain(const PartitionParams &p, const int64_t (&key)[KPT],
                                                         uint32_t (&rel)[KPT], uint64_t &ok, unsigned long long &n_out) {
#pragma unroll
  for (int j = 0; j < KPT; j++) {
    const uint64_t r = (uint64_t)key[j] - (uint64_t)p.base;
    if (((ok >> j) & 1) && r >= p.range) {
      ok &= ~(1ull << j);
      n_out++;
      if (STATS) {
        const long long k = (long long)key[j];
        atomicMin(&p.outliers->mn, k);
        atomicMax(&p.outliers->mx, k);
        atomicAdd(&p.outliers->lo32_sum, (unsigned long long)((uint64_t)k & 0xFFFFFFFFull));
        atomicAdd((unsigned long long *)&p.outliers->hi32_sum, (unsigned long long)(k >> 32));
        atomicAdd(&p.outliers->count, 1ull);
      }
    }
    rel[j] = (uint32_t)r;
    asm volatile("" : "+v"(rel[j]));
  }
  __builtin_amdgcn_sched_barrier(0);
}

template <int THREADS, int KPT>
__device__ __forceinline__ void partition_outlier_stats(const PartitionParams &p, int64_t tile, bool wide, uint32_t outm,
                                                     OutlierStats *lds_out) {
  constexpr int kTile = THREADS * KPT;
  global_i64_ptr vals = (global_i64_ptr)(uintptr_t)((const int64_t *)p.values + p.offset);
  const int64_t row0 = tile * kTile;
  const bool paired = row0 + kTile <= p.length && wide;
  unsigned long long cnt = 0;
  for (int j = 0; j < KPT; j++) {
    if (!((outm >> j) & 1)) continue;
    const int64_t i = paired ? row0 + (int64_t)(j / 2) * 2 * THREADS + 2 * threadIdx.x + (j & 1)
                             : row0 + (int64_t)j * THREADS + threadIdx.x;
    const long long k = vals[i];
    if (k < *(volatile long long *)&lds_out->mn) atomicMin(&lds_out->mn, k);
    if (k > *(volatile long long *)&lds_out->mx) atomicMax(&lds_out->mx, k);
    atomicAdd(&lds_out->lo32_sum, (unsigned long long)((uint64_t)k & 0xFFFFFFFFull));
    atomicAdd((unsigned long long *)&lds_out->hi32_sum, (unsigned long long)(k >> 32));
    cnt++;
  }
  atomicAdd(&lds_out->count, cnt);
}

template <int THREADS, int KPT, int MAXP, int PAD, bool VALIDITY, bool KEY16, bool STATS, bool FORM_CLUSTERED, bool PACK20 = false>
__global__ __launch_bounds__(THREADS) __attribute__((amdgpu_waves_per_eu(4, 4))) void partition_kernel(
    PartitionParams p, unsigned long long *counters) {
  if ((p.force_form ? p.force_form == 2 : __builtin_amdgcn_readfirstlane((int)p.cursors[2 * p.n_buckets]) != 0) != FORM_CLUSTERED)
    return;
  constexpr int kTile = THREADS * KPT;
  __shared__ uint32_t sorted[kTile];
  __shared__ uint32_t hist[MAXP];
  __shared__ uint32_t toff[MAXP + 1];
  __shared__ uint32_t gbase[MAXP];
  __shared__ uint32_t wave_sums[16];
  __shared__ uint32_t long_runs[kTile / 1024 + 1];
  __shared__ uint32_t t_lo, t_hi;
  const bool wide = (((uintptr_t)p.values + (uintptr_t)p.offset * 8) & 15) == 0;
  unsigned long long n_valid = 0, n_out = 0;
  const int64_t n_tiles = (p.length + kTile - 1) / kTile;
  uint32_t rel[KPT];
  __shared__ uint32_t st_min, st_max;
  __shared__ unsigned long long st_sum, st_cnt;
  __shared__ OutlierStats st_out;
  if (STATS && threadIdx.x == 0) {
    st_min = 0xFFFFFFFFu;
    st_max = 0;
    st_sum = 0;
    st_cnt = 0;
    st_out.mn = INT64_MAX;
    st_out.mx = INT64_MIN;
    st_out.lo32_sum = 0;
    st_out.hi32_sum = 0;
    st_out.count = 0;
  }
  if (STATS) __syncthreads();
  auto tile_loop = [&](auto clustered_tag) __attribute__((always_inline)) {
  constexpr bool CLUSTERED = decltype(clustered_tag)::value;
  for (int64_t tile = blockIdx.x; tile < n_tiles; tile += gridDim.x) {
    uint64_t ok;
    {
      int64_t key[KPT];
      uint32_t ok32 = 0;
      partition_load_tile<THREADS, KPT, VALIDITY>(p, tile, wide, key, ok32);
      ok = ok32;
      n_valid += __builtin_popcountll(ok);
      if (CLUSTERED) {
        uint32_t outm;
        partition_relative<KPT>(p, key, rel, outm);
        outm &= ok32;
        ok = ok32 & ~outm;
        if (__ballot(outm != 0)) {
          n_out += __builtin_popcount(outm);
          if (STATS && outm) partition_outlier_stats<THREADS, KPT>(p, tile, wide, outm, &st_out);
        }
      } else {
        partition_relative_plain<KPT, STATS>(p, key, rel, ok, n_out);
      }
    }
    if (STATS) {
      uint32_t tmin = 0xFFFFFFFFu, tmax = 0;
      unsigned long long tsum = 0;
#pragma unroll
      for (int j = 0; j < KPT; j++) {
        const bool in = (ok >> j) & 1;
        tmin = (in && rel[j] < tmin) ? rel[j] : tmin;
        tmax = (in && rel[j] > tmax) ? rel[j] : tmax;
        tsum += in ? rel[j] : 0u;
      }
      unsigned long long tcnt = __builtin_popcountll(ok);
#pragma unroll
      for (int d = 32; d >= 1; d >>= 1) {
        const uint32_t omin = __shfl_down(tmin, d, 64), omax = __shfl_down(tmax, d, 64);
        tmin = omin < tmin ? omin : tmin;
        tmax = omax > tmax ? omax : tmax;
        tsum += __shfl_down(tsum, d, 64);
        tcnt += __shfl_down(tcnt, d, 64);
      }
      if ((threadIdx.x & 63) == 0 && tcnt) {
        atomicMin(&st_min, tmin);
        atomicMax(&st_max, tmax);
        atomicAdd(&st_sum, tsum);
        atomicAdd(&st_cnt, tcnt);
      }
    }
    if (CLUSTERED && !p.want_multiplicity) {
      if (threadIdx.x == 0) {
        t_lo = 0xFFFFFFFFu;
        t_hi = 0;
      }
      __syncthreads();
      uint32_t lo = 0xFFFFFFFFu, hi = 0;
#pragma unroll
      for (int j = 0; j < KPT; j++) {
        const bool in = (ok >> j) & 1;
        lo = (in && rel[j] < lo) ? rel[j] : lo;
        hi = (in && rel[j] > hi) ? rel[j] : hi;
      }
#pragma unroll
      for (int d = 32; d >= 1; d >>= 1) {
        const uint32_t olo = __shfl_xor(lo, d, 64), ohi = __shfl_xor(hi, d, 64);
        lo = olo < lo ? olo : lo;
        hi = ohi > hi ? ohi : hi;
      }
      if ((threadIdx.x & 63) == 0 && lo <= hi) {
        atomicMin(&t_lo, lo);
        atomicMax(&t_hi, hi);
      }
      __syncthreads();
      const uint32_t tlo = t_lo, thi = t_hi;
      if (tlo > thi) continue;
      const uint32_t w0 = tlo >> 5, nw = (thi >> 5) - w0 + 1;
      if (nw <= (uint32_t)kTile) {
        for (uint32_t w = threadIdx.x; w < nw; w += THREADS) sorted[w] = 0;
        __syncthreads();
#pragma unroll
        for (int j = 0; j < KPT; j += 2) {
          uint32_t cw = 0xFFFFFFFFu, cb = 0;
          if ((ok >> j) & 1) {
            cw = (rel[j] >> 5) - w0;
            cb = 1u << (rel[j] & 31);
          }
          if ((ok >> (j + 1)) & 1) {
            const uint32_t w1 = (rel[j + 1] >> 5) - w0, b1 = 1u << (rel[j + 1] & 31);
            if (w1 == cw) {
              cb |= b1;
            } else {
              if (cb) atomicOr(&sorted[cw], cb);
              cw = w1;
              cb = b1;
            }
          }
          const bool send = merge_word_group<16>(cw, cb);
          if (send && cb) atomicOr(&sorted[cw], cb);
        }
        __syncthreads();
        for (uint32_t w = threadIdx.x; w < nw; w += THREADS) {
          const uint32_t v = sorted[w];
          if (v) atomicOr(&p.seen[w0 + w], v);
        }
        __syncthreads();
        continue;
      }
    }
    partition_process_tile<THREADS, KPT, MAXP, PAD, KEY16, PACK20, CLUSTERED>(p, sorted, hist, toff, gbase, wave_sums, long_runs, rel, ok,
                                                                      [] {}, [] {});
  }
  };
  tile_loop(std::integral_constant<bool, FORM_CLUSTERED>{});
  if (STATS) {
    __syncthreads();
    if (threadIdx.x == 0) {
      ScanPartial out;
      out.min_k = INT64_MAX;
      out.max_k = INT64_MIN;
      out.sum_lo = 0;
      out.sum_hi = 0;
      out.non_null = (int64_t)st_cnt;
      out.sum = out.comp = out.s1 = out.s2 = 0.0;
      if (st_cnt) {
        out.min_k = (int64_t)((uint64_t)p.base + st_min);
        out.max_k = (int64_t)((uint64_t)p.base + st_max);
        const __int128 sum = (__int128)st_sum + (__int128)st_cnt * (__int128)p.base;
        out.sum_lo = (uint64_t)sum;
        out.sum_hi = (int64_t)(sum >> 64);
      }
      p.stats[blockIdx.x] = out;
      if (st_out.count) {
        atomicMin(&p.outliers->mn, st_out.mn);
        atomicMax(&p.outliers->mx, st_out.mx);
        atomicAdd(&p.outliers->lo32_sum, st_out.lo32_sum);
        atomicAdd((unsigned long long *)&p.outliers->hi32_sum, (unsigned long long)st_out.hi32_sum);
        atomicAdd(&p.outliers->count, st_out.count);
      }
    }
  }
  block_add2_any(n_valid, n_out, &counters[kCntValidRows], &counters[kCntOutOfRange]);
}


template <int LDS_WORDS, bool KEY16 = false, bool PACK20 = false>
__global__ __launch_bounds__(kPartitionThreads) void bucket_apply_kernel(PartitionParams p,
                                                                         unsigned long long *counters) {
  __shared__ __attribute__((aligned(16))) uint32_t lds[LDS_WORDS];
  const uint32_t tid = threadIdx.x;
  const uint32_t b = blockIdx.x;
  const uint32_t slice_words = (uint32_t)((1ull << p.sub_bits) >> 5);
  uint32_t *l_seen = lds;
  uint32_t *l_twice = lds + slice_words;
  uint32_t *g_seen = p.seen + (uint64_t)b * slice_words;
  uint32_t *g_twice = p.want_multiplicity ? p.twice + (uint64_t)b * slice_words : nullptr;
  for (uint32_t w = tid * 4; w < slice_words; w += kPartitionThreads * 4) {
    *(uint4 *)&l_seen[w] = *(const uint4 *)&g_seen[w];
    if (g_twice) *(uint4 *)&l_twice[w] = *(const uint4 *)&g_twice[w];
  }
  __syncthreads();
  unsigned long long cnt = p.cursors[b];
  const unsigned long long limit = p.cursors[p.n_buckets + b];
  if (cnt > limit) cnt = limit;
  const bool clustered = p.cursors[2 * p.n_buckets] != 0;
  const uint32_t li = b - p.bucket0;
  if (li >= p.n_lists) cnt = 0;
  if (PACK20) {
    const uint8_t *list = (const uint8_t *)p.lists + (uint64_t)li * p.cap / 3 * 8;
    constexpr uint64_t kStepP = (uint64_t)kPartitionThreads * 6;
    for (uint64_t w0 = (uint64_t)(tid & ~63u) * 6; w0 < cnt; w0 += 4 * kStepP) {
      const uint64_t i0 = w0 + (uint64_t)(tid & 63u) * 6;
      typedef unsigned int u32x4 __attribute__((ext_vector_type(4)));
      u32x4 k4[4];
#pragma unroll
      for (int q = 0; q < 4; q++) {
        const uint64_t i = i0 + q * kStepP;
        k4[q] = u32x4{0, 0, 0, 0};
        if (i < cnt) k4[q] = __builtin_nontemporal_load((const u32x4 *)(list + i / 3 * 8));
      }
#pragma unroll
      for (int q = 0; q < 4; q++) {
        if (i0 + q * kStepP >= cnt) continue;
        const uint64_t w[2] = {(uint64_t)k4[q].x | ((uint64_t)k4[q].y << 32), (uint64_t)k4[q].z | ((uint64_t)k4[q].w << 32)};
#pragma unroll
        for (int u = 0; u < 6; u++) {
          const uint32_t k = (uint32_t)(w[u / 3] >> (20 * (u % 3))) & 0xFFFFFu;
          const uint32_t bit = 1u << (k & 31);
          if (g_twice) {
            if (k == 0xFFFFFu) continue;
            const uint32_t prev = atomicOr(&l_seen[k >> 5], bit);
            if (prev & bit) atomicOr(&l_twice[k >> 5], bit);
          } else {
            atomicOr(&l_seen[k >> 5], bit);
          }
        }
      }
    }
  } else if (KEY16) {
    const uint16_t *list16 = (const uint16_t *)p.lists + (uint64_t)li * p.cap;
    constexpr uint64_t kStep16 = (uint64_t)kPartitionThreads * 8;
    for (uint64_t w0 = (uint64_t)(tid & ~63u) * 8; w0 < cnt; w0 += 4 * kStep16) {
      const uint64_t i0 = w0 + (uint64_t)(tid & 63u) * 8;
      typedef unsigned int u32x4 __attribute__((ext_vector_type(4)));
      u32x4 k4[4];
#pragma unroll
      for (int q = 0; q < 4; q++) {
        const uint64_t i = i0 + q * kStep16;
        k4[q] = u32x4{0, 0, 0, 0};
        if (i < cnt) k4[q] = __builtin_nontemporal_load((const u32x4 *)&list16[i]);
      }
      if (clustered) {
#pragma unroll
        for (int q = 0; q < 4; q++) {
          const bool in = i0 + q * kStep16 < cnt;
          const uint32_t w4[4] = {k4[q].x, k4[q].y, k4[q].z, k4[q].w};
          uint32_t cw = 0xFFFFFFFFu, cb = 0;
#pragma unroll
          for (int u = 0; u < 8; u++) {
            const uint32_t k = (u & 1) ? w4[u / 2] >> 16 : w4[u / 2] & 0xFFFFu;
            if (!in) continue;
            if ((k >> 5) != cw) {
              if (cb) atomicOr(&l_seen[cw], cb);
              cw = k >> 5;
              cb = 0;
            }
            cb |= 1u << (k & 31);
          }
          const bool send = merge_word_group<4>(cw, cb);
          if (send && cb) atomicOr(&l_seen[cw], cb);
        }
      } else {
#pragma unroll
      for (int q = 0; q < 4; q++) {
        if (i0 + q * kStep16 >= cnt) continue;
        const uint32_t w4[4] = {k4[q].x, k4[q].y, k4[q].z, k4[q].w};
#pragma unroll
        for (int u = 0; u < 4; u++) {
          const uint32_t ka = w4[u] & 0xFFFFu, kb = w4[u] >> 16;
          atomicOr(&l_seen[ka >> 5], 1u << (ka & 31));
          atomicOr(&l_seen[kb >> 5], 1u << (kb & 31));
        }
      }
      }
    }
  } else {
  const uint32_t *list = p.lists + (uint64_t)li * p.cap;
  constexpr uint64_t kStep = (uint64_t)kPartitionThreads * 4;
  for (uint64_t w0 = (uint64_t)(tid & ~63u) * 4; w0 < cnt; w0 += 4 * kStep) {
    const uint64_t i0 = w0 + (uint64_t)(tid & 63u) * 4;
    uint4 k4[4];
#pragma unroll
    for (int q = 0; q < 4; q++) {
      const uint64_t i = i0 + q * kStep;
      typedef unsigned int u32x4 __attribute__((ext_vector_type(4)));
      u32x4 v = {kListPad, kListPad, kListPad, kListPad};
      if (i < cnt) v = __builtin_nontemporal_load((const u32x4 *)&list[i]);
      k4[q] = make_uint4(v.x, v.y, v.z, v.w);
    }
    if (clustered && !g_twice) {
#pragma unroll
      for (int q = 0; q < 4; q++) {
        const uint32_t ks[4] = {k4[q].x, k4[q].y, k4[q].z, k4[q].w};
        uint32_t cw = 0xFFFFFFFFu, cb = 0;
#pragma unroll
        for (int u = 0; u < 4; u++) {
          if (ks[u] == kListPad) continue;
          if ((ks[u] >> 5) != cw) {
            if (cb) atomicOr(&l_seen[cw], cb);
            cw = ks[u] >> 5;
            cb = 0;
          }
          cb |= 1u << (ks[u] & 31);
        }
        const bool send = merge_word_group<8>(cw, cb);
        if (send && cb) atomicOr(&l_seen[cw], cb);
      }
      continue;
    }
#pragma unroll
    for (int q = 0; q < 4; q++) {
      const uint32_t ks[4] = {k4[q].x, k4[q].y, k4[q].z, k4[q].w};
#pragma unroll
      for (int u = 0; u < 4; u++) {
        if (ks[u] == kListPad) continue;
        const uint32_t bit = 1u << (ks[u] & 31);
        if (g_twice) {
          const uint32_t prev = atomicOr(&l_seen[ks[u] >> 5], bit);
          if (prev & bit) atomicOr(&l_twice[ks[u] >> 5], bit);
        } else {
          atomicOr(&l_seen[ks[u] >> 5], bit);
        }
      }
    }
  }
  }
  __syncthreads();
  unsigned long long n_seen = 0, n_twice = 0;
  for (uint32_t w = tid * 4; w < slice_words; w += kPartitionThreads * 4) {
    const uint4 s4 = *(const uint4 *)&l_seen[w];
    *(uint4 *)&g_seen[w] = s4;
    n_seen += __builtin_popcount(s4.x) + __builtin_popcount(s4.y) + __builtin_popcount(s4.z) +
              __builtin_popcount(s4.w);
    if (g_twice) {
      const uint4 t4 = *(const uint4 *)&l_twice[w];
      *(uint4 *)&g_twice[w] = t4;
      n_twice += __builtin_popcount(t4.x) + __builtin_popcount(t4.y) + __builtin_popcount(t4.z) +
                 __builtin_popcount(t4.w);
    }
  }
  block_add2_any(n_seen, n_twice, &counters[kCntDistinct], &counters[kCntTwice]);
}

__global__ __launch_bounds__(1024) void partition_init_kernel(PartitionParams p, unsigned long long *totals) {
  unsigned long long *cursors = p.cursors;
  const uint32_t n_buckets = p.n_buckets;
  OutlierStats *outliers = p.outliers;
  for (uint32_t b = threadIdx.x; b < n_buckets; b += blockDim.x) {
    cursors[b] = 0;
    cursors[n_buckets + b] = ~0ull;
  }
  if (threadIdx.x == 0) {
    if (outliers) {
      outliers->mn = INT64_MAX;
      outliers->mx = INT64_MIN;
      outliers->lo32_sum = 0;
      outliers->hi32_sum = 0;
      outliers->count = 0;
    }
    totals[kCntDistinct] = 0;
    totals[kCntTwice] = 0;
  }
  __shared__ uint32_t agree, asked;
  if (threadIdx.x == 0) agree = asked = 0;
  __syncthreads();
  const uint32_t lane = threadIdx.x & 63, wave = threadIdx.x >> 6;
  const int64_t n_groups = p.length / 128;
  global_i64_ptr vals = (global_i64_ptr)(uintptr_t)((const int64_t *)p.values + p.offset);
  global_u8_ptr vbits = (global_u8_ptr)(uintptr_t)p.validity;
  uint64_t rr[4][2];
  uint32_t vb[4][2];
  bool have[4];
#pragma unroll
  for (int k = 0; k < 4; k++) {
    const uint32_t g = wave + 16u * k;
    have[k] = (int64_t)g < n_groups;
    const int64_t group = n_groups <= 64 ? (int64_t)g : (int64_t)g * (n_groups / 64);
#pragma unroll
    for (int h = 0; h < 2; h++) {
      const int64_t i = group * 128 + h * 64 + lane;
      rr[k][h] = have[k] ? (uint64_t)vals[i] - (uint64_t)p.base : ~0ull;
      vb[k][h] = (have[k] && vbits) ? (uint32_t)TGX_VALID_BIT(vbits, p.offset + i) : 1u;
    }
  }
#pragma unroll
  for (int k = 0; k < 4; k++) {
    if (!have[k]) continue;
    bool same = true;
    uint32_t b0 = 0xFFFFFFFFu;
#pragma unroll
    for (int h = 0; h < 2; h++) {
      const uint64_t r = rr[k][h];
      const bool okr = r < p.range && vb[k][h] != 0;
      const uint64_t act = __ballot(okr);
      if (act == 0) continue;
      const uint32_t b = (uint32_t)(r >> p.sub_bits);
      if (b0 == 0xFFFFFFFFu) b0 = (uint32_t)__builtin_amdgcn_readlane((int)b, (int)__builtin_ctzll(act));
      same = same && __ballot(okr && b != b0) == 0;
    }
    if (lane == 0) {
      atomicAdd(&asked, 1u);
      if (same) atomicAdd(&agree, 1u);
    }
  }
  __syncthreads();
  if (threadIdx.x == 0) {
    const unsigned long long in_order = (asked >= 4 && 4 * agree >= 3 * asked) ? 1ull : 0ull;
    cursors[2 * n_buckets] = in_order;
    totals[kCntForm] = 1ull + in_order;
  }
}

int partition_grid(int64_t length, int n_cu) {
  int64_t n_tiles = (length + kPartitionTile - 1) / kPartitionTile;
  int grid = (int)(n_tiles < (int64_t)n_cu ? n_tiles : (int64_t)n_cu);
  return grid < 1 ? 1 : grid;
}

void launch_partition(const PartitionParams &p, unsigned long long *d_counters, int n_cu,
                      hipStream_t stream) {
  const int grid = partition_grid(p.length, n_cu);
  const bool plain = p.force_form != 2, in_order = p.force_form != 1;
#define TGX_PART(VAL, K16, ST)                                                                                      \
  do {                                                                                                              \
    if (plain)                                                                                                      \
      hipLaunchKernelGGL((partition_kernel<kPartitionThreads, kPartitionKeysPerThread, (int)kMaxPartitions, kRunPad4, VAL, K16, ST, false>), \
                         dim3(grid), dim3(kPartitionThreads), 0, stream, p, d_counters);                            \
    if (in_order)                                                                                                   \
      hipLaunchKernelGGL((partition_kernel<kPartitionThreads, kPartitionKeysPerThread, (int)kMaxPartitions, kRunPad4, VAL, K16, ST, true>), \
                         dim3(grid), dim3(kPartitionThreads), 0, stream, p, d_counters);                            \
  } while (0)
#define TGX_PART20(VAL, ST)                                                                                         \
  do {                                                                                                              \
    if (plain)                                                                                                      \
      hipLaunchKernelGGL((partition_kernel<kPartitionThreads, kPartitionKeysPerThread, (int)kMaxPartitions, kRunPad4, VAL, false, ST, false, true>), \
                         dim3(grid), dim3(kPartitionThreads), 0, stream, p, d_counters);                            \
    if (in_order)                                                                                                   \
      hipLaunchKernelGGL((partition_kernel<kPartitionThreads, kPartitionKeysPerThread, (int)kMaxPartitions, kRunPad4, VAL, false, ST, true, true>), \
                         dim3(grid), dim3(kPartitionThreads), 0, stream, p, d_counters);                            \
  } while (0)
  if (p.key16 == 2) {
    if (p.stats) {
      if (p.validity) TGX_PART20(true, true); else TGX_PART20(false, true);
    } else {
      if (p.validity) TGX_PART20(true, false); else TGX_PART20(false, false);
    }
    return;
  }
  if (p.stats) {
    if (p.key16) {
      if (p.validity) TGX_PART(true, true, true); else TGX_PART(false, true, true);
    } else {
      if (p.validity) TGX_PART(true, false, true); else TGX_PART(false, false, true);
    }
  } else if (p.key16) {
    if (p.validity) TGX_PART(true, true, false); else TGX_PART(false, true, false);
  } else {
    if (p.validity) TGX_PART(true, false, false); else TGX_PART(false, false, false);
  }
#undef TGX_PART
#undef TGX_PART20
}

hipError_t launch_bucket_apply(const PartitionParams &p, unsigned long long *d_counters,
                               hipStream_t stream) {
  const size_t words = ((size_t)1 << p.sub_bits) / 32 * (p.want_multiplicity ? 2 : 1);
  const dim3 grid(p.n_buckets), block(kPartitionThreads);
#define TGX_APPLY(W)                                                                                  \
  if (words <= W) {                                                                                   \
    if (p.key16 == 2)                                                                                 \
      hipLaunchKernelGGL((bucket_apply_kernel<W, false, true>), grid, block, 0, stream, p, d_counters); \
    else if (p.key16)                                                                                 \
      hipLaunchKernelGGL((bucket_apply_kernel<W, true>), grid, block, 0, stream, p, d_counters);      \
    else                                                                                              \
      hipLaunchKernelGGL((bucket_apply_kernel<W, false>), grid, block, 0, stream, p, d_counters);     \
    return hipGetLastError();                                                                         \
  }
  TGX_APPLY(1024)
  TGX_APPLY(2048)
  TGX_APPLY(4096)
  TGX_APPLY(8192)
  TGX_APPLY(16384)
  TGX_APPLY(32768)
#undef TGX_APPLY
  return hipErrorInvalidValue;
}

void launch_partition_init(const PartitionParams &p, unsigned long long *totals, hipStream_t stream) {
  hipLaunchKernelGGL(partition_init_kernel, dim3(1), dim3(1024), 0, stream, p, totals);
}

}
```

term_amd/csrc/kernels/scan.hip:

```cpp
#include <hip/hip_runtime.h>

#include "device_types.h"
#include "distinct_types.h"
#include "pivot_search.h"

namespace tgx {

typedef long long i64x2 __attribute__((ext_vector_type(2)));
typedef const uint64_t __attribute__((address_space(4))) *const_u64_ptr;
typedef const i64x2 __attribute__((address_space(1))) *global_i64x2_ptr;
typedef const int64_t __attribute__((address_space(1))) *global_i64_ptr;
typedef const uint8_t __attribute__((address_space(1))) *global_u8_ptr;
typedef const uint64_t __attribute__((address_space(1))) *global_u64_ptr;

struct LaneAcc {
  int64_t mn, mx;
  uint64_t lo;
  int64_t hi;
  double s, c;
  double s1, s2;
  int64_t cnt;
};

__device__ __forceinline__ void acc_init(LaneAcc &a) {
// ... 702 lines not shown
      hi = __builtin_fmax(hi, __shfl_xor(hi, d, 64));
    }
    if (lo == 0.0) lo = __longlong_as_double(1LL);
    if (hi == 0.0) hi = __longlong_as_double((long long)0x8000000000000001ULL);
    const long long lb = __double_as_longlong(lo), hb = __double_as_longlong(hi);
    c.lo = ((int64_t)__builtin_amdgcn_readfirstlane((int)(lb >> 32)) << 32) |
           (uint32_t)__builtin_amdgcn_readfirstlane((int)lb);
    c.hi = ((int64_t)__builtin_amdgcn_readfirstlane((int)(hb >> 32)) << 32) |
           (uint32_t)__builtin_amdgcn_readfirstlane((int)hb);
  } else {
    int64_t lo = a.mn, hi = a.mx;
#pragma unroll
    for (int d = 32; d >= 1; d >>= 1) {
      const int64_t ol = __shfl_xor(lo, d, 64), oh = __shfl_xor(hi, d, 64);
      lo = ol < lo ? ol : lo;
      hi = oh > hi ? oh : hi;
    }
    c.lo = ((int64_t)__builtin_amdgcn_readfirstlane((int)(lo >> 32)) << 32) |
           (uint32_t)__builtin_amdgcn_readfirstlane((int)lo);
    c.hi = ((int64_t)__builtin_amdgcn_readfirstlane((int)(hi >> 32)) << 32) |
           (uint32_t)__builtin_amdgcn_readfirstlane((int)hi);
  }
}

template <bool XF, bool YF, bool KLL>
__device__ __forceinline__ void pair_rows(const ScanPairDesc &P, LaneAcc &ax, LaneAcc &ay, ColFast<XF> &fx,
                                          ColFast<YF> &fy, unsigned long long &out_x, unsigned long long &out_y,
                                          ComoTile &m, i64x2 vx, i64x2 vy, uint32_t bx, uint32_t by, KllLane &Kx,
                                          KllLane &Ky, double *rx, double *ry, double pvx, double pvy) {
  out_x |= col_fast_value<XF>(fx, ax, vx.x, (bx & 1u) != 0);
  out_x |= col_fast_value<XF>(fx, ax, vx.y, (bx & 2u) != 0);
  out_y |= col_fast_value<YF>(fy, ay, vy.x, (by & 1u) != 0);
  out_y |= col_fast_value<YF>(fy, ay, vy.y, (by & 2u) != 0);
  const double x0 = kll_value<XF>(vx.x), x1 = kll_value<XF>(vx.y);
  const double y0 = kll_value<YF>(vy.x), y1 = kll_value<YF>(vy.y);
  como_tile_add(m, x0 - pvx, y0 - pvy, (bx & by & 1u) != 0);
  como_tile_add(m, x1 - pvx, y1 - pvy, (bx & by & 2u) != 0);
  if (KLL) {
    if (P.x.kll.picks) {
      kll_push<false>(Kx, rx, x0, (bx & 1u) != 0 && x0 == x0);
      kll_push<false>(Kx, rx, x1, (bx & 2u) != 0 && x1 == x1);
    }
    if (P.y.kll.picks) {
      kll_push<false>(Ky, ry, y0, (by & 1u) != 0 && y0 == y0);
      kll_push<false>(Ky, ry, y1, (by & 2u) != 0 && y1 == y1);
    }
  }
}

template <bool F>
__device__ __forceinline__ void col_exact_tile(ColFast<F> &c, LaneAcc &a, i64x2 v0, i64x2 v1, i64x2 v2, i64x2 v3,
                                               uint32_t b0, uint32_t b1, uint32_t b2, uint32_t b3) {
  col_exact_value<F>(c, a, v0.x, (b0 & 1u) != 0);
  col_exact_value<F>(c, a, v0.y, (b0 & 2u) != 0);
  col_exact_value<F>(c, a, v1.x, (b1 & 1u) != 0);
  col_exact_value<F>(c, a, v1.y, (b1 & 2u) != 0);
  col_exact_value<F>(c, a, v2.x, (b2 & 1u) != 0);
  col_exact_value<F>(c, a, v2.y, (b2 & 2u) != 0);
  col_exact_value<F>(c, a, v3.x, (b3 & 1u) != 0);
  col_exact_value<F>(c, a, v3.y, (b3 & 2u) != 0);
  col_refresh_bounds<F>(c, a);
}

template <bool XF, bool YF, bool KLL>
__device__ void pair_ragged(const ScanPairDesc &P, int64_t r0, int64_t r1, int lane, int stride, LaneAcc &ax,
                            LaneAcc &ay, ComoLane &m, int64_t &n_both, KllLane &Kx, KllLane &Ky, double *rx, double *ry,
                            uint32_t wave_slot, double pvx, double pvy) {
  global_i64_ptr xs = (global_i64_ptr)(uintptr_t)((const int64_t *)P.x.values + P.x.offset);
  global_i64_ptr ys = (global_i64_ptr)(uintptr_t)((const int64_t *)P.y.values + P.y.offset);
  global_u8_ptr xv = (global_u8_ptr)(uintptr_t)P.x.validity, yv = (global_u8_ptr)(uintptr_t)P.y.validity;
  for (int64_t i0 = r0; i0 < r1; i0 += stride) {
    const int64_t i = i0 + lane;
    const bool in = i < r1;
    bool vx = in, vy = in;
    if (in && xv) {
      const int64_t b = P.x.offset + i;
      vx = (xv[b >> 3] >> (b & 7)) & 1;
    }
    if (in && yv) {
      const int64_t b = P.y.offset + i;
      vy = (yv[b >> 3] >> (b & 7)) & 1;
    }
    const int64_t xb = in ? xs[i] : 0, yb = in ? ys[i] : 0;
    acc_value<XF, false>(ax, xb, vx, 0.0);
    acc_value<YF, false>(ay, yb, vy, 0.0);
    ax.cnt += vx ? 1 : 0;
    ay.cnt += vy ? 1 : 0;
    const double a = kll_value<XF>(xb), b = kll_value<YF>(yb);
    como_fold(m, a - pvx, b - pvy, vx && vy);
    n_both += (int64_t)__builtin_popcountll(__builtin_amdgcn_ballot_w64(vx && vy));

    if (KLL) {
      if (P.x.kll.picks) {
        kll_push(Kx, rx, a, vx && a == a);
        kll_drain(Kx, rx, P.x.kll, wave_slot, lane);
      }
      if (P.y.kll.picks) {
        kll_push(Ky, ry, b, vy && b == b);
        kll_drain(Ky, ry, P.y.kll, wave_slot, lane);
      }
    }
  }
}

__device__ __forceinline__ void write_partial(ScanPartial *out, const LaneAcc &r, int64_t cnt) {
  ScanPartial p;
  p.non_null = cnt;
  p.min_k = r.mn;
  p.max_k = r.mx;
  p.sum_lo = r.lo;
  p.sum_hi = r.hi;
  p.sum = r.s;
  p.comp = r.c;
  p.s1 = r.s1;
  p.s2 = r.s2;
  *out = p;
}

template <bool XF, bool YF, bool KLL>
__device__ __forceinline__ void pair_body(const ScanPairDesc &P, ScanPartial *out_x, ScanPartial *out_y,
                                          ComomentPartial *out_c, int wave, int lane, double pvx, double pvy) {
  LaneAcc ax, ay;
  acc_init(ax);
  acc_init(ay);
  ComoLane m;
#pragma unroll
  for (int k = 0; k < 5; k++) m.s[k] = m.c[k] = 0.0;
  KllLane Kx, Ky;
  kll_lane_init(Kx, P.x.kll.top);
  kll_lane_init(Ky, P.y.kll.top);
  double *rx = nullptr, *ry = nullptr;
  if (KLL) {
    const size_t rx_n = P.x.kll.picks ? ((size_t)1 << P.x.kll.top) + kTileRows : 0;
    const size_t ry_n = P.y.kll.picks ? ((size_t)1 << P.y.kll.top) + kTileRows : 0;
    rx = scan_dyn_lds + (size_t)wave * (rx_n + ry_n);
    ry = rx + rx_n;
  }
  const int64_t wave_global = (int64_t)blockIdx.x * kWavesPerBlock + wave;
  const int64_t n_waves = (int64_t)gridDim.x * kWavesPerBlock;
  const uint32_t wave_slot = (uint32_t)wave_global;
  const ScanColDesc &cx = P.x, &cy = P.y;
  int64_t cnt_x = 0, cnt_y = 0, n_both = 0;
  uint32_t lane_cnt_x = 0, lane_cnt_y = 0, lane_both = 0;
  ColFast<XF> fx;
  ColFast<YF> fy;
  col_fast_init<XF>(fx);
  col_fast_init<YF>(fy);
  if (cx.n_tiles > 0) {
    global_i64x2_ptr px = (global_i64x2_ptr)(uintptr_t)((const int64_t *)cx.values + cx.offset + cx.head);
    global_i64x2_ptr py = (global_i64x2_ptr)(uintptr_t)((const int64_t *)cy.values + cy.offset + cy.head);
    const bool hx = cx.validity != nullptr, hy = cy.validity != nullptr;
    global_u8_ptr vbx = (global_u8_ptr)(uintptr_t)(cx.validity + ((cx.offset + cx.head) >> 3));
    global_u8_ptr vby = (global_u8_ptr)(uintptr_t)(cy.validity + ((cy.offset + cy.head) >> 3));
    const int32_t n_tiles32 = (int32_t)cx.n_tiles, step32 = (int32_t)n_waves;
    for (int32_t t = (int32_t)wave_global; t < n_tiles32; t += step32) {
      const int64_t p = (int64_t)t * (kTileRows / 2) + lane;
      const i64x2 x0 = __builtin_nontemporal_load(px + p), x1 = __builtin_nontemporal_load(px + p + 64);
      const i64x2 x2 = __builtin_nontemporal_load(px + p + 128), x3 = __builtin_nontemporal_load(px + p + 192);
      const i64x2 y0 = __builtin_nontemporal_load(py + p), y1 = __builtin_nontemporal_load(py + p + 64);
      const i64x2 y2 = __builtin_nontemporal_load(py + p + 128), y3 = __builtin_nontemporal_load(py + p + 192);
      uint32_t bx0 = 3, bx1 = 3, bx2 = 3, bx3 = 3, by0 = 3, by1 = 3, by2 = 3, by3 = 3;
      {
        const int64_t vbyte = (int64_t)t * (kTileRows / 8) + (lane >> 2);
        const uint32_t sh2 = 2u * (uint32_t)(lane & 3);
        if (hx) {
          const uint32_t v0 = vbx[vbyte], v1 = vbx[vbyte + 16], v2 = vbx[vbyte + 32], v3 = vbx[vbyte + 48];
          bx0 = (v0 >> sh2) & 3u;
          bx1 = (v1 >> sh2) & 3u;
          bx2 = (v2 >> sh2) & 3u;
          bx3 = (v3 >> sh2) & 3u;
        }
        if (hy) {
          const uint32_t v0 = vby[vbyte], v1 = vby[vbyte + 16], v2 = vby[vbyte + 32], v3 = vby[vbyte + 48];
          by0 = (v0 >> sh2) & 3u;
          by1 = (v1 >> sh2) & 3u;
          by2 = (v2 >> sh2) & 3u;
          by3 = (v3 >> sh2) & 3u;
        }
      }
      ComoTile q;
#pragma unroll
      for (int k = 0; k < 5; k++) q.t[k] = 0.0;
      lane_cnt_x += (bx0 & 1u) + (bx0 >> 1) + (bx1 & 1u) + (bx1 >> 1) + (bx2 & 1u) + (bx2 >> 1) + (bx3 & 1u) + (bx3 >> 1);
      lane_cnt_y += (by0 & 1u) + (by0 >> 1) + (by1 & 1u) + (by1 >> 1) + (by2 & 1u) + (by2 >> 1) + (by3 & 1u) + (by3 >> 1);
      {
        const uint32_t c0 = bx0 & by0, c1 = bx1 & by1, c2 = bx2 & by2, c3 = bx3 & by3;
        lane_both += (c0 & 1u) + (c0 >> 1) + (c1 & 1u) + (c1 >> 1) + (c2 & 1u) + (c2 >> 1) + (c3 & 1u) + (c3 >> 1);
      }
      unsigned long long out_x = 0, out_y = 0;
      pair_rows<XF, YF, KLL>(P, ax, ay, fx, fy, out_x, out_y, q, x0, y0, bx0, by0, Kx, Ky, rx, ry, pvx, pvy);
      pair_rows<XF, YF, KLL>(P, ax, ay, fx, fy, out_x, out_y, q, x1, y1, bx1, by1, Kx, Ky, rx, ry, pvx, pvy);
      pair_rows<XF, YF, KLL>(P, ax, ay, fx, fy, out_x, out_y, q, x2, y2, bx2, by2, Kx, Ky, rx, ry, pvx, pvy);
      pair_rows<XF, YF, KLL>(P, ax, ay, fx, fy, out_x, out_y, q, x3, y3, bx3, by3, Kx, Ky, rx, ry, pvx, pvy);
      if (out_x) col_exact_tile<XF>(fx, ax, x0, x1, x2, x3, bx0, bx1, bx2, bx3);
      if (out_y) col_exact_tile<YF>(fy, ay, y0, y1, y2, y3, by0, by1, by2, by3);
      como_tile_flush(m, q);
      if (XF) {
        two_sum_add(ax.s, ax.c, fx.tsum);
        fx.tsum = 0.0;
      }
      if (YF) {
        two_sum_add(ay.s, ay.c, fy.tsum);
        fy.tsum = 0.0;
      }
      if (KLL) {
        if (P.x.kll.picks) kll_drain(Kx, rx, P.x.kll, wave_slot, lane);
        if (P.y.kll.picks) kll_drain(Ky, ry, P.y.kll, wave_slot, lane);
      }
    }
    if (blockIdx.x == gridDim.x - 1) {
      const int64_t tail0 = cx.head + cx.n_tiles * kTileRows;
      if (wave == 0)
        pair_ragged<XF, YF, KLL>(P, 0, cx.head, lane, 64, ax, ay, m, n_both, Kx, Ky, rx, ry, wave_slot, pvx, pvy);
      if (wave == 1)
        pair_ragged<XF, YF, KLL>(P, tail0, cx.length, lane, 64, ax, ay, m, n_both, Kx, Ky, rx, ry, wave_slot, pvx, pvy);
    }
  } else {
    pair_ragged<XF, YF, KLL>(P, wave_global * 64, cx.length, lane, (int)(n_waves * 64), ax, ay, m, n_both, Kx, Ky,
                             rx, ry, wave_slot, pvx, pvy);
  }
  if (KLL) {
    Kx.mn = __builtin_fmin(Kx.mn, fx.dmn);
    Kx.mx = __builtin_fmax(Kx.mx, fx.dmx);
    Ky.mn = __builtin_fmin(Ky.mn, fy.dmn);
    Ky.mx = __builtin_fmax(Ky.mx, fy.dmx);
    if (P.x.kll.picks) kll_finish_wave(Kx, rx, P.x.kll, wave_slot, lane);
    if (P.y.kll.picks) kll_finish_wave(Ky, ry, P.y.kll, wave_slot, lane);
  }
  ax.cnt += lane_cnt_x;
  ay.cnt += lane_cnt_y;
  {
    int64_t both = lane_both;
#pragma unroll
    for (int d = 32; d >= 1; d >>= 1) both += shfl_down_i64(both, d);
    n_both += __shfl(both, 0, 64);
  }
#pragma unroll
  for (int d = 32; d >= 1; d >>= 1) {
    LaneAcc bx = acc_shfl_down(ax, d), by = acc_shfl_down(ay, d);
    acc_merge(ax, bx, XF);
    acc_merge(ay, by, YF);
#pragma unroll
    for (int k = 0; k < 5; k++) {
      const double os = __shfl_down(m.s[k], d, 64), oc = __shfl_down(m.c[k], d, 64);
      m.c[k] += oc;
      two_sum_add(m.s[k], m.c[k], os);
    }
  }
  __shared__ LaneAcc s_x[kWavesPerBlock], s_y[kWavesPerBlock];
  __shared__ ComoLane s_m[kWavesPerBlock];
  __shared__ int64_t s_n[kWavesPerBlock][3];
  if (lane == 0) {
    s_x[wave] = ax;
    s_y[wave] = ay;
    s_m[wave] = m;
    s_n[wave][0] = cnt_x;
    s_n[wave][1] = cnt_y;
    s_n[wave][2] = n_both;
  }
  __syncthreads();
  if (threadIdx.x == 0) {
    LaneAcc rxa = s_x[0], rya = s_y[0];
    ComomentPartial c;
    c.n = s_n[0][2];
    int64_t cx_n = s_n[0][0], cy_n = s_n[0][1];
#pragma unroll
    for (int k = 0; k < 5; k++) {
      c.s[k] = s_m[0].s[k];
      c.c[k] = s_m[0].c[k];
    }
    for (int w = 1; w < kWavesPerBlock; w++) {
      acc_merge(rxa, s_x[w], XF);
      acc_merge(rya, s_y[w], YF);
      cx_n += s_n[w][0];
      cy_n += s_n[w][1];
      c.n += s_n[w][2];
      for (int k = 0; k < 5; k++) {
        c.c[k] += s_m[w].c[k];
        two_sum_add(c.s[k], c.c[k], s_m[w].s[k]);
      }
    }
    write_partial(out_x, rxa, cx_n + rxa.cnt);
    write_partial(out_y, rya, cy_n + rya.cnt);
    *out_c = c;
  }
}

template <bool XF, bool YF, bool KLL>
__global__ __launch_bounds__(kScanBlock) void scan_pair_kernel(const ScanPairLaunch L, int first,
                                                                ScanPartial *__restrict__ partials,
                                                                ComomentPartial *__restrict__ como,
                                                                const ComomentAcc *__restrict__ como_accs) {
  const int pair = first + (int)blockIdx.y;
  const ScanPairDesc &P = L.pairs[pair];
  const double pvx = como_accs[P.como_acc].px, pvy = como_accs[P.como_acc].py;
  const int wave = __builtin_amdgcn_readfirstlane(threadIdx.x >> 6);
  const int lane = threadIdx.x & 63;
  ScanPartial *ox = partials + ((size_t)2 * pair) * gridDim.x + blockIdx.x;
  ScanPartial *oy = partials + ((size_t)2 * pair + 1) * gridDim.x + blockIdx.x;
  ComomentPartial *oc = como + (size_t)pair * gridDim.x + blockIdx.x;
  pair_body<XF, YF, KLL>(P, ox, oy, oc, wave, lane, pvx, pvy);
}

__global__ __launch_bounds__(64) void scan_reduce_kernel(const ScanLaunch L,
                                                          const ScanPartial *__restrict__ partials,
                                                          int blocks_per_col,
                                                          ScanAcc *__restrict__ accs,
                                                          const OutlierStats *__restrict__ outliers) {
  const int col = blockIdx.x;
  const int lane = threadIdx.x;
  if (L.acc_index[col] < 0) return;
  const ScanColDesc c = L.cols[col];
  const ScanPartial *p = partials + (size_t)col * blocks_per_col;
  LaneAcc a;
  acc_init(a);
  if (outliers && lane == 0 && outliers->count) {
    LaneAcc b;
    acc_init(b);
    b.mn = outliers->mn;
    b.mx = outliers->mx;
    const __int128 sum = (__int128)(unsigned __int128)outliers->lo32_sum + (((__int128)outliers->hi32_sum) << 32);
    b.lo = (uint64_t)sum;
    b.hi = (int64_t)(sum >> 64);
    b.cnt = (int64_t)outliers->count;
    acc_merge(a, b, c.is_float);
  }
  for (int i0 = lane; i0 < blocks_per_col; i0 += 256) {
    LaneAcc b[4];
#pragma unroll
    for (int u = 0; u < 4; u++) {
      const int i = i0 + 64 * u;
      if (i < blocks_per_col) {
        b[u].mn = p[i].min_k;
        b[u].mx = p[i].max_k;
        b[u].lo = p[i].sum_lo;
        b[u].hi = p[i].sum_hi;
        b[u].s = p[i].sum;
        b[u].c = p[i].comp;
        b[u].s1 = p[i].s1;
        b[u].s2 = p[i].s2;
        b[u].cnt = p[i].non_null;
      }
    }
#pragma unroll
    for (int u = 0; u < 4; u++)
      if (i0 + 64 * u < blocks_per_col) acc_merge(a, b[u], c.is_float);
  }
#pragma unroll
  for (int d = 32; d >= 1; d >>= 1) {
    LaneAcc b = acc_shfl_down(a, d);
    acc_merge(a, b, c.is_float);
  }
  if (lane == 0) scan_fold(accs[L.acc_index[col]], a, c);
}

__global__ __launch_bounds__(256) void scan_pivot_kernel(const ScanLaunch L,
                                                          double *__restrict__ pivots,
                                                          int32_t *__restrict__ pivot_set,
                                                          PivotSearch *__restrict__ search) {
  const ScanColDesc c = L.cols[blockIdx.y];
  if (!c.want_variance || c.length <= 0) return;
  const int slot = L.acc_index[blockIdx.y];
  __shared__ double s_sum[256], s_one[256];
  __shared__ int s_cnt[256];
  __shared__ int s_done;
  global_i64_ptr vals = (global_i64_ptr)(uintptr_t)((const int64_t *)c.values + c.offset);
  global_i32_ptr vals32 = (global_i32_ptr)(uintptr_t)((const int32_t *)c.values + c.offset);
  global_u8_ptr vbits = (global_u8_ptr)(uintptr_t)c.validity;
  auto valid = [&](int64_t i) {
    if (!c.validity) return true;
    const int64_t b = c.offset + i;
    return ((vbits[b >> 3] >> (b & 7)) & 1) != 0;
  };
  auto value = [&](int64_t i) {
    if (c.elem32) return c.is_float ? (double)__int_as_float(vals32[i]) : (double)vals32[i];
    return c.is_float ? __longlong_as_double(vals[i]) : (double)vals[i];
  };
  if (threadIdx.x == 0) s_done = pivot_set[slot];
  __syncthreads();
  const int64_t n = c.length < 4096 ? c.length : 4096;
  for (int look = 0; look < 2 && blockIdx.x == 0 && !s_done; look++) {
    const int64_t step = look == 0 ? 1 : c.length / n;
    if (look == 1 && step == 1) break;
    double sum = 0.0, one = 0.0;
    int cnt = 0;
    for (int64_t k = threadIdx.x; k < n; k += 256) {
      const int64_t i = k * step;
      if (!valid(i)) continue;
      const double x = value(i);
      if (x - x != 0.0) continue;
      if (cnt == 0) one = x;
      sum += x;
      cnt++;
    }
    s_sum[threadIdx.x] = sum;
    s_one[threadIdx.x] = one;
    s_cnt[threadIdx.x] = cnt;
    __syncthreads();
    if (threadIdx.x == 0) {
      double t = 0.0, first = 0.0;
      int k = 0;
      for (int i = 0; i < 256; i++) {
        if (k == 0 && s_cnt[i] > 0) first = s_one[i];
        t += s_sum[i];
        k += s_cnt[i];
      }
      if (k > 0) {
        double p = t / (double)k;
        if (p - p != 0.0) p = first;
        pivots[slot] = p;
        pivot_set[slot] = 1;
        s_done = 1;
      }
    }
    __syncthreads();
  }
  if (blockIdx.x > 0 && !s_done) {
    const int64_t i = threadIdx.x;
    bool hit = false;
    if (i < c.length && valid(i)) {
      const double x = value(i);
      hit = x - x == 0.0;
    }
    if (__syncthreads_or(hit)) return;
  }
  if (!s_done) {
    int64_t lo, hi;
    pivot_search_stretch(c.length, &lo, &hi);
    const int64_t end_byte = (c.offset + c.length + 7) >> 3;
    const int64_t row = first_valid_finite_row(
        lo, hi, [&](int64_t r) { return validity_bits64((const uint8_t *)c.validity, c.offset + r, end_byte); },
        [&](int64_t i) {
          const double x = value(i);
          return x - x == 0.0;
        });
    pivot_search_offer(&search[slot], row);
  }
}

__global__ __launch_bounds__(64) void scan_pivot_finish_kernel(const ScanLaunch L, double *__restrict__ pivots,
                                                                int32_t *__restrict__ pivot_set,
                                                                PivotSearch *__restrict__ search) {
  const ScanColDesc c = L.cols[blockIdx.x];
  if (!c.want_variance || c.length <= 0 || threadIdx.x != 0) return;
  const int slot = L.acc_index[blockIdx.x];
  const unsigned long long best = search[slot].best;
  if (!best) return;
  search[slot].best = 0;
  if (pivot_set[slot]) return;
  const int64_t i = (int64_t)~best;
  double x;
  if (c.elem32)
    x = c.is_float ? (double)__int_as_float(((const int32_t *)c.values)[c.offset + i])
                   : (double)((const int32_t *)c.values)[c.offset + i];
  else
    x = c.is_float ? __longlong_as_double(((const int64_t *)c.values)[c.offset + i])
                   : (double)((const int64_t *)c.values)[c.offset + i];
  pivots[slot] = x;
  pivot_set[slot] = 1;
}

__global__ __launch_bounds__(256) void count_kernel(const CountLaunch L,
                                                     unsigned long long *__restrict__ block_counts,
                                                     CountAcc *__restrict__ direct) {
  const CountColDesc c = L.cols[blockIdx.y];
  const int64_t bit0 = c.offset, bit1 = c.offset + c.length;
  const uintptr_t base = (uintptr_t)c.validity;
  const int64_t mis = (int64_t)(base & 7);
  global_u64_ptr words = (global_u64_ptr)(base - mis);
  const int64_t b0 = bit0 + mis * 8, b1 = bit1 + mis * 8;
  const int64_t w0 = b0 >> 6, w1 = (b1 + 63) >> 6;
  int64_t cnt = 0;
  for (int64_t w = w0 + (int64_t)blockIdx.x * blockDim.x + threadIdx.x; w < w1;
       w += (int64_t)gridDim.x * blockDim.x) {
    uint64_t x = words[w];
    if (w == w0) x &= ~0ull << (b0 & 63);
    if (w == w1 - 1 && (b1 & 63)) x &= ~0ull >> (64 - (b1 & 63));
    cnt += __builtin_popcountll(x);
  }
#pragma unroll
  for (int d = 32; d >= 1; d >>= 1) cnt += shfl_down_i64(cnt, d);
  __shared__ int64_t s[kWavesPerBlock];
  if ((threadIdx.x & 63) == 0) s[threadIdx.x >> 6] = cnt;
  __syncthreads();
  if (threadIdx.x == 0) {
    const int64_t total = s[0] + s[1] + s[2] + s[3];
    if (direct && gridDim.x == 1) {
      CountAcc &a = direct[L.acc_index[blockIdx.y]];
      a.total += c.length;
      a.non_null += total;
    } else {
      block_counts[(size_t)blockIdx.y * gridDim.x + blockIdx.x] = (unsigned long long)total;
    }
  }
}

__global__ __launch_bounds__(64) void count_reduce_kernel(const CountLaunch L,
                                                           const unsigned long long *__restrict__ bc,
                                                           int blocks_per_col,
                                                           CountAcc *__restrict__ accs) {
  const int col = blockIdx.x;
  int64_t cnt = 0;
  for (int i = threadIdx.x; i < blocks_per_col; i += 64)
    cnt += (int64_t)bc[(size_t)col * blocks_per_col + i];
#pragma unroll
  for (int d = 32; d >= 1; d >>= 1) cnt += shfl_down_i64(cnt, d);
  if (threadIdx.x == 0) {
    CountAcc &a = accs[L.acc_index[col]];
    a.total += L.cols[col].length;
    a.non_null += cnt;
  }
}

__global__ __launch_bounds__(256) void widen_narrow_kernel(const void *__restrict__ src, long long *__restrict__ dst,
                                                           int64_t n, int mode) {
  const int64_t stride = (int64_t)gridDim.x * blockDim.x;
  for (int64_t i = (int64_t)blockIdx.x * blockDim.x + threadIdx.x; i < n; i += stride) {
    long long v;
    switch (mode) {
      case 2: v = (long long)((const int8_t *)src)[i]; break;
      case 3: v = (long long)((const int16_t *)src)[i]; break;
      case 4: v = (long long)((const uint8_t *)src)[i]; break;
      case 5: v = (long long)((const uint16_t *)src)[i]; break;
      case 6: v = (long long)((const uint32_t *)src)[i]; break;
      default: v = (long long)((((const uint8_t *)src)[i >> 3] >> (i & 7)) & 1); break;
    }
    dst[i] = v;
  }
}

__global__ __launch_bounds__(256) void widen32_kernel(const void *__restrict__ src, void *__restrict__ dst, int64_t n,
                                                      int is_float) {
  const int64_t stride = (int64_t)gridDim.x * blockDim.x;
  const bool aligned = (((uintptr_t)src) & 15) == 0;
  const int64_t n4 = aligned ? n >> 2 : 0;
  for (int64_t q = (int64_t)blockIdx.x * blockDim.x + threadIdx.x; q < n4; q += stride) {
    const int4 v = ((const int4 *)src)[q];
    longlong2 *o = (longlong2 *)dst + 2 * q;
    if (is_float) {
      o[0] = make_longlong2(f32_widen_bits((uint32_t)v.x), f32_widen_bits((uint32_t)v.y));
      o[1] = make_longlong2(f32_widen_bits((uint32_t)v.z), f32_widen_bits((uint32_t)v.w));
    } else {
      o[0] = make_longlong2((long long)v.x, (long long)v.y);
      o[1] = make_longlong2((long long)v.z, (long long)v.w);
    }
  }
  for (int64_t i = 4 * n4 + (int64_t)blockIdx.x * blockDim.x + threadIdx.x; i < n; i += stride) {
    const int v = ((const int *)src)[i];
    ((long long *)dst)[i] = is_float ? f32_widen_bits((uint32_t)v) : (long long)v;
  }
}

void launch_widen32(const void *src, void *dst, int64_t n, int mode, int n_cu, hipStream_t stream) {
  if (n <= 0) return;
  int64_t blocks = (n / 4 + 255) / 256;
  if (blocks > (int64_t)n_cu * 16) blocks = (int64_t)n_cu * 16;
  if (blocks < 1) blocks = 1;
  if (mode >= 2) {
    hipLaunchKernelGGL(widen_narrow_kernel, dim3((int)blocks), dim3(256), 0, stream, src, (long long *)dst, n, mode);
    return;
  }
  hipLaunchKernelGGL(widen32_kernel, dim3((int)blocks), dim3(256), 0, stream, src, dst, n, mode);
}

void launch_scan_pivot(const ScanLaunch &L, int n_cols, double *d_pivots, int32_t *d_pivot_set, PivotSearch *d_search,
                       hipStream_t stream) {
  int64_t longest = 0;
  for (int k = 0; k < n_cols; k++)
    if (L.cols[k].want_variance && L.cols[k].length > longest) longest = L.cols[k].length;
  hipLaunchKernelGGL(scan_pivot_kernel, dim3(pivot_search_blocks(longest), n_cols), dim3(256), 0, stream, L, d_pivots,
                     d_pivot_set, d_search);
  hipLaunchKernelGGL(scan_pivot_finish_kernel, dim3(n_cols), dim3(64), 0, stream, L, d_pivots, d_pivot_set, d_search);
}

void launch_scan_main_only(const ScanLaunch &L, int n_cols, int blocks_per_col, ScanPartial *d_partials,
                           ScanAcc *d_accs, hipStream_t stream) {
  hipLaunchKernelGGL(scan_kernel<3>, dim3(blocks_per_col, n_cols), dim3(kScanBlock), 0, stream, L, d_partials,
                     blocks_per_col == 1 ? d_accs : nullptr);
}

void launch_scan_kll(const ScanLaunch &L, int n_cols, int blocks_per_col, size_t lds_bytes, ScanPartial *d_partials,
                     hipStream_t stream) {
  hipLaunchKernelGGL(scan_kll_kernel<1>, dim3(blocks_per_col, n_cols), dim3(kScanBlock), lds_bytes, stream, L,
                     d_partials);
}

void launch_scan_hll(const ScanLaunch &L, int n_cols, int blocks_per_col, ScanPartial *d_partials, hipStream_t stream) {
  hipLaunchKernelGGL(scan_hll_kernel<3>, dim3(blocks_per_col, n_cols), dim3(kScanBlock), 0, stream, L, d_partials);
  const int slices = blocks_per_col >= 64 ? 32 : (blocks_per_col >= 8 ? 4 : 1);
  const int rows_per_slice = (blocks_per_col + slices - 1) / slices;
  hipLaunchKernelGGL(hll_reduce_kernel, dim3(kHllRegisters / 4 / 256 * slices, n_cols), dim3(256), 0, stream, L,
                     blocks_per_col, rows_per_slice);
}

template <bool KLL>
__global__ __launch_bounds__(kScanBlock) __attribute__((amdgpu_waves_per_eu(4, 4))) void scan_pair_ff_kernel(
    const ScanPairLaunch L, int first, ScanPartial *__restrict__ partials, ComomentPartial *__restrict__ como,
    const ComomentAcc *__restrict__ como_accs) {
  const int pair = first + (int)blockIdx.y;
  const ScanPairDesc &P = L.pairs[pair];
  const double pvx = como_accs[P.como_acc].px, pvy = como_accs[P.como_acc].py;
  const int wave = __builtin_amdgcn_readfirstlane(threadIdx.x >> 6);
  const int lane = threadIdx.x & 63;
  ScanPartial *ox = partials + ((size_t)2 * pair) * gridDim.x + blockIdx.x;
  ScanPartial *oy = partials + ((size_t)2 * pair + 1) * gridDim.x + blockIdx.x;
  ComomentPartial *oc = como + (size_t)pair * gridDim.x + blockIdx.x;
  pair_body<true, true, KLL>(P, ox, oy, oc, wave, lane, pvx, pvy);
}

template <bool XF, bool YF>
static void launch_scan_pairs_of(const ScanPairLaunch &L, int first, int count, int blocks_per_pair, size_t lds_bytes,
                                 ScanPartial *d_partials, void *d_como_partials, const ComomentAcc *d_como_accs,
                                 hipStream_t stream) {
  if (XF && YF) {
    if (lds_bytes)
      hipLaunchKernelGGL(scan_pair_ff_kernel<true>, dim3(blocks_per_pair, count), dim3(kScanBlock), lds_bytes, stream, L,
                         first, d_partials, (ComomentPartial *)d_como_partials, d_como_accs);
    else
      hipLaunchKernelGGL(scan_pair_ff_kernel<false>, dim3(blocks_per_pair, count), dim3(kScanBlock), 0, stream, L, first,
                         d_partials, (ComomentPartial *)d_como_partials, d_como_accs);
    return;
  }
  if (lds_bytes)
    hipLaunchKernelGGL((scan_pair_kernel<XF, YF, true>), dim3(blocks_per_pair, count), dim3(kScanBlock), lds_bytes, stream,
                       L, first, d_partials, (ComomentPartial *)d_como_partials, d_como_accs);
  else
    hipLaunchKernelGGL((scan_pair_kernel<XF, YF, false>), dim3(blocks_per_pair, count), dim3(kScanBlock), 0, stream, L,
                       first, d_partials, (ComomentPartial *)d_como_partials, d_como_accs);
}

void launch_scan_pairs(const ScanPairLaunch &L, int n_pairs, int blocks_per_pair, size_t lds_bytes,
                       ScanPartial *d_partials, void *d_como_partials, const ComomentAcc *d_como_accs,
                       hipStream_t stream) {
  int first = 0;
  while (first < n_pairs) {
    const bool xf = L.pairs[first].x.is_float != 0, yf = L.pairs[first].y.is_float != 0;
    int count = 1;
    while (first + count < n_pairs && (L.pairs[first + count].x.is_float != 0) == xf &&
           (L.pairs[first + count].y.is_float != 0) == yf)
      count++;
    if (xf && yf)
      launch_scan_pairs_of<true, true>(L, first, count, blocks_per_pair, lds_bytes, d_partials, d_como_partials, d_como_accs, stream);
    else if (xf)
      launch_scan_pairs_of<true, false>(L, first, count, blocks_per_pair, lds_bytes, d_partials, d_como_partials, d_como_accs, stream);
    else if (yf)
      launch_scan_pairs_of<false, true>(L, first, count, blocks_per_pair, lds_bytes, d_partials, d_como_partials, d_como_accs, stream);
    else
      launch_scan_pairs_of<false, false>(L, first, count, blocks_per_pair, lds_bytes, d_partials, d_como_partials, d_como_accs, stream);
    first += count;
  }
}

void launch_scan_reduce_only(const ScanLaunch &L, int n_cols, int blocks_per_col, ScanPartial *d_partials,
                             ScanAcc *d_accs, hipStream_t stream, const OutlierStats *outliers) {
  hipLaunchKernelGGL(scan_reduce_kernel, dim3(n_cols), dim3(64), 0, stream, L, d_partials, blocks_per_col,
                     d_accs, outliers);
}

void launch_count(const CountLaunch &L, int n_cols, int blocks_per_col, unsigned long long *d_block_counts,
                  CountAcc *d_accs, hipStream_t stream) {
  hipLaunchKernelGGL(count_kernel, dim3(blocks_per_col, n_cols), dim3(256), 0, stream, L, d_block_counts,
                     blocks_per_col == 1 ? d_accs : nullptr);
  if (blocks_per_col > 1)
    hipLaunchKernelGGL(count_reduce_kernel, dim3(n_cols), dim3(64), 0, stream, L, d_block_counts,
                       blocks_per_col, d_accs);
}

__global__ __launch_bounds__(256) void state_reset_kernel(StateResetArgs a) {
  for (int r = 0; r < a.n_zero; r++) {
    uint32_t *p = (uint32_t *)a.zero[r];
    const uint32_t words = a.zero_bytes[r] >> 2;
    for (uint32_t i = blockIdx.x * 256u + threadIdx.x; i < words; i += gridDim.x * 256u) p[i] = 0;
  }
  constexpr uint32_t W = sizeof(ScanAcc) / 8;
  static_assert(sizeof(ScanAcc) % 8 == 0 && offsetof(ScanAcc, min_k) == 16 && offsetof(ScanAcc, max_k) == 24, "layout");
  long long *dst = (long long *)a.ident;
  for (uint32_t i = blockIdx.x * 256u + threadIdx.x; i < a.n_ident * W; i += gridDim.x * 256u) {
    const uint32_t w = i % W;
    dst[i] = w == 2 ? INT64_MAX : w == 3 ? INT64_MIN : 0;
  }
}
void launch_state_reset(const StateResetArgs &a, hipStream_t stream) {
  uint32_t most = a.n_ident * (uint32_t)sizeof(ScanAcc);
  for (int r = 0; r < a.n_zero; r++) most = a.zero_bytes[r] > most ? a.zero_bytes[r] : most;
  const unsigned blocks = most <= 4096u ? 1u : (most / 4096u > 64u ? 64u : most / 4096u);
  hipLaunchKernelGGL(state_reset_kernel, dim3(blocks), dim3(256), 0, stream, a);
}

}
```

term_amd/csrc/update.cpp:

```cpp
#include "api_internal.h"

#include <chrono>
namespace {
struct UpdateMarks {
  bool on;
  std::chrono::steady_clock::time_point t0;
  char line[512];
  int len = 0;
  UpdateMarks() {
    static const bool enabled = getenv("TGX_UPDATE_TIMING") != nullptr;
    on = enabled;
    if (on) t0 = std::chrono::steady_clock::now();
  }
  void mark(const char *what) {
    if (!on) return;
    const double us = std::chrono::duration<double, std::micro>(std::chrono::steady_clock::now() - t0).count();
    len += snprintf(line + len, sizeof(line) - (size_t)len > 0 ? sizeof(line) - (size_t)len : 0, " %s %.1f", what, us);
    if (len > (int)sizeof(line) - 1) len = (int)sizeof(line) - 1;
  }
  ~UpdateMarks() {
    if (on && len) fprintf(stderr, "tgx_update (us):%s\n", line);
  }
};
thread_local UpdateMarks *tl_marks = nullptr;
// ... 167 lines not shown
  if (want < 1) want = 1;
  return (int)want;
}

tgx_status como_pivots(tgx_state *st, const ComomentLaunch &L, int n_pairs, tgx_error *err) {
  (void)err;
  bool want = false;
  for (int k = 0; k < n_pairs; k++) want |= L.pairs[k].length > 0;
  if (want)
    launch_como_pivot(L, n_pairs, st->d_como_acc.as<ComomentAcc>(),
                      st->d_pivot_search.as<PivotSearch>() + st->plan->scan.size(), st->stream);
  return TGX_OK;
}


tgx_status update_validate(const tgx_plan *plan, tgx_state *st, const tgx_column *columns, size_t n_columns,
                                  int64_t *nrows_out, BatchTraits *traits, tgx_error *err) {
  (void)n_columns;
  const std::vector<char> &used = plan->used, &reads_values = plan->reads_values;
  int64_t nrows = -1;
  for (int i = 0; i < plan->n_columns_needed; i++) {
    if (!used[i]) continue;
    const tgx_column &c = columns[i];
    if (c.length < 0 || c.offset < 0) return fail(err, TGX_INVALID_ARGUMENT, "column %d: negative length/offset", i);
    if (nrows < 0) nrows = c.length;
    if (c.length != nrows)
      return fail(err, TGX_INVALID_ARGUMENT, "column %d has %lld rows, expected %lld", i, (long long)c.length,
                  (long long)nrows);
    if (c.type < TGX_INT64 || c.type > TGX_BOOL) return fail(err, TGX_INVALID_ARGUMENT, "column %d: unknown type %d", i, c.type);
    if (is_keys_only(c.type) && plan->stats_on[i])
      return fail(err, TGX_UNSUPPORTED, "column %d: a %s column takes COUNT and DISTINCT checks only", i,
                  c.type == TGX_BOOL ? "Boolean" : "UInt64");
    for (int k = 0; k < kNumSide; k++)
      if (plan->side_on[k][i]) TGX_TRY(kSideKinds[k].check_column(plan, i, c, err));
    if (plan->timegap_on[i]) TGX_TRY(timegap_check_type(plan, i, c.type, err));
    if (c.mem != TGX_MEM_HOST && c.mem != TGX_MEM_DEVICE)
      return fail(err, TGX_INVALID_ARGUMENT, "column %d: unknown memory space %d", i, c.mem);
    if (st->col_types[i] == 0) st->col_types[i] = c.type;
    if (st->col_types[i] != c.type)
      return fail(err, TGX_INVALID_ARGUMENT, "column %d changed type between batches (%d -> %d)", i,
                  st->col_types[i], c.type);
    const bool host = c.mem == TGX_MEM_HOST;
    traits->any_host |= host;
    traits->any_utf8 |= c.type == TGX_UTF8;
    traits->any_strings |= is_any_string(c.type) || c.type == TGX_DICT32_UTF8;
    traits->coalescible &= is_numeric(c.type) || is_numeric32(c.type) || c.type == TGX_UINT64 ||
                           (is_narrow_int(c.type) && host) ||
                           (is_string(c.type) && host) ||
                           (c.type == TGX_UTF8_VIEW && host) ||
                           (c.type == TGX_DICT32_UTF8 && host && c.dictionary && c.dictionary->mem == TGX_MEM_HOST);
    if (c.length > 0) {
      if ((is_numeric(c.type) || is_widened(c.type) || c.type == TGX_UINT64) && reads_values[i] && !c.values)
        return fail(err, TGX_INVALID_ARGUMENT, "column %d: values is NULL", i);
      if ((c.type == TGX_UTF8 || c.type == TGX_LARGE_UTF8) && !c.offsets)
        return fail(err, TGX_INVALID_ARGUMENT, "column %d: offsets is NULL", i);
    }
    if (c.type == TGX_UTF8_VIEW && c.length > 0) {
      if (!c.values) return fail(err, TGX_INVALID_ARGUMENT, "column %d: views (values) is NULL", i);
      if (c.n_variadic < 0 || (c.n_variadic > 0 && !c.variadic))
        return fail(err, TGX_INVALID_ARGUMENT, "column %d: malformed variadic buffer list", i);
      if (c.mem == TGX_MEM_HOST && c.n_variadic > 0 && !c.variadic_sizes)
        return fail(err, TGX_INVALID_ARGUMENT, "column %d: HOST Utf8View columns need variadic_sizes", i);
    }
    if (c.type == TGX_DICT32_UTF8) {
      const tgx_column *dc = c.dictionary;
      if (!dc || !is_string(dc->type))
        return fail(err, TGX_INVALID_ARGUMENT, "column %d: a Dictionary<Int32, Utf8> column needs a Utf8/LargeUtf8 dictionary", i);
      if (dc->length < 0 || dc->offset < 0 || (dc->length > 0 && !dc->offsets))
        return fail(err, TGX_INVALID_ARGUMENT, "column %d: malformed dictionary", i);
      if (c.length > 0 && reads_values[i] && !c.values)
        return fail(err, TGX_INVALID_ARGUMENT, "column %d: indices (values) is NULL", i);
    }
  }
  *nrows_out = nrows < 0 ? 0 : nrows;
  return TGX_OK;
}


extern "C" tgx_status tgx_update(const tgx_plan *plan, tgx_state *st, const tgx_column *columns,
                                 size_t n_columns, tgx_error *err) try {
  if (!plan || !st || st->plan != plan) return fail(err, TGX_INVALID_ARGUMENT, "state does not belong to plan");
  if ((int)n_columns < plan->n_columns_needed)
    return fail(err, TGX_INVALID_ARGUMENT, "plan reads column %d but only %zu columns were passed",
                plan->n_columns_needed - 1, n_columns);
  if (n_columns > 0 && !columns) return fail(err, TGX_INVALID_ARGUMENT, "columns is NULL");
  UpdateMarks marks;
  struct MarksScope {
    MarksScope(UpdateMarks *m) { tl_marks = m->on ? m : nullptr; }
    ~MarksScope() { tl_marks = nullptr; }
  } marks_scope(&marks);
  TGX_TRY(need_device(err));
  bool any_retained = false, any_plain_host = false;
  for (int i = 0; i < plan->n_columns_needed; i++) {
    if (!plan->used[i]) continue;
    const tgx_column &c = columns[i];
    any_retained |= c.mem == TGX_MEM_HOST_RETAINED || (c.dictionary && c.dictionary->mem == TGX_MEM_HOST_RETAINED);
    any_plain_host |= c.mem == TGX_MEM_HOST || (c.dictionary && c.dictionary->mem == TGX_MEM_HOST);
  }
  static thread_local std::vector<tgx_column> as_host, as_host_dicts;
  if (any_retained) {
    as_host.assign(columns, columns + n_columns);
    as_host_dicts.clear();
    as_host_dicts.reserve(n_columns);
    for (size_t i = 0; i < n_columns; i++) {
      if ((int)i >= plan->n_columns_needed || !plan->used[i]) continue;
      tgx_column &c = as_host[i];
      if (c.mem == TGX_MEM_HOST_RETAINED) c.mem = TGX_MEM_HOST;
      if (c.dictionary && c.dictionary->mem == TGX_MEM_HOST_RETAINED) {
        as_host_dicts.push_back(*c.dictionary);
        as_host_dicts.back().mem = TGX_MEM_HOST;
        c.dictionary = &as_host_dicts.back();
      }
    }
    columns = as_host.data();
  }
  int64_t nrows = 0;
  BatchTraits traits;
  traits.retained = any_retained && !any_plain_host;
  TGX_TRY(update_validate(plan, st, columns, n_columns, &nrows, &traits, err));
  for (auto &side : st->side)
    if (side) TGX_TRY(side->accepts(st, nrows, err));
  if (nrows == 0) {
    st->batches++;
    return TGX_OK;
  }
  const Coalescer &co = st->coalesce;
  if (traits.coalescible && nrows > 0 && nrows <= kCoalesceMaxRows && !co.disabled && !co.flushing) {
    bool taken = false;
    TGX_TRY(coalesce_append(plan, st, columns, nrows, traits, &taken, err));
    if (taken) return TGX_OK;
  }
  update_mark("validated");
  bind_thread();
  TGX_TRY(coalesce_flush(st, err));
  update_mark("flushed");
  const tgx_status rc = update_impl(plan, st, columns, nrows, err);
  update_mark("done");
  return rc;
} catch (...) {
  return tgx::abi_exception(err);
}

namespace {

struct StagedBatch {
  std::vector<tgx_column> dev;
  bool any_host = false;
  bool arena_in_use = false;
};

struct FusedPair {
  int como, x, y;
  ScanColDesc dx, dy;
};

struct BatchFusion {
  std::vector<int> kll_on_col, pair_of_col, hll_on_col;
  std::vector<char> kll_fused, como_fused;
  std::vector<char> distinct_idle;
  std::vector<FusedPair> fused_pairs;
  std::vector<BatchKeyFacts> key_facts;
  std::vector<NumericPrep> dprep;
  std::vector<int> stats_by_partition;
  std::vector<char> distinct_done;

  int stats_slot(const tgx_plan *plan, size_t q) const {
    const int s = plan->distinct[q].scan_slot;
    return (s >= 0 && stats_by_partition[s] == (int)q) ? s : -1;
  }
};

int scan_slot_of(const tgx_plan *plan, int col) {
  for (size_t q = 0; q < plan->scan.size(); q++)
    if (plan->scan[q].column == col) return (int)q;
  return -1;
}

int fused_blocks(const ScanColDesc &d, int n_tasks) {
  const int64_t units = d.n_tiles > 0 ? d.n_tiles : (d.length + 63) / 64;
  int64_t want = (units + 4 * kWavesPerBlock - 1) / (4 * kWavesPerBlock);
  const int64_t cap = std::max(32, (g_ctx.n_cu * 3) / std::max(1, n_tasks));
  return (int)std::max<int64_t>(1, std::min(want, cap));
}

int64_t rows_per_wave(const ScanColDesc &d, int blocks) {
  const int64_t waves = (int64_t)blocks * kWavesPerBlock;
  if (d.n_tiles > 0) return (d.n_tiles + waves - 1) / waves * kTileRows;
  return ((d.length + 63) / 64 + waves - 1) / waves * 64;
}

tgx_status stage_batch(const tgx_plan *plan, tgx_state *st, const tgx_column *columns, StagedBatch *b, tgx_error *err) {
  st->staging_used = 0;
  if (st->arena_used) (void)hipStreamSynchronize(st->stream);
  st->arena_used = 0;
  st->host_direct = false;
  st->dict_views.clear();
  st->pending_widen.clear();
  std::vector<tgx_column> &dev = b->dev;
  dev.assign(plan->n_columns_needed, tgx_column());
  const std::vector<char> &needs_wide = plan->needs_wide;
  for (int i = 0; i < plan->n_columns_needed; i++) {
    if (!plan->used[i]) continue;
    if (columns[i].mem == TGX_MEM_HOST && columns[i].length > 0) b->any_host = true;
    if (columns[i].length == 0) {
      dev[i] = columns[i];
      if ((is_numeric32(dev[i].type) && needs_wide[i]) || is_narrow_int(dev[i].type)) dev[i].type = widened_type(dev[i].type);
      if (dev[i].type == TGX_UINT64) dev[i].type = TGX_INT64;
      continue;
    }
    const bool widen = needs_wide[i] != 0 || (is_narrow_int(columns[i].type) && plan->reads_values[i]);
    if (is_narrow_int(columns[i].type) && !widen) {
      tgx_column bare = columns[i];
      bare.type = TGX_INT64;
      bare.values = nullptr;
      TGX_TRY(stage_column(st, bare, &dev[i], err, false));
      continue;
    }
    TGX_TRY(stage_column(st, columns[i], &dev[i], err, widen));
  }
  update_mark("staged");
  b->arena_in_use = st->arena_used != 0;
  if (b->arena_in_use)
    HIP_TRY(hipMemcpyAsync(st->arena_dev[st->arena_cur].p, st->arena_host[st->arena_cur], st->arena_used,
                           hipMemcpyHostToDevice, st->stream));
  for (const auto &w : st->pending_widen) launch_widen32(w.src, w.dst, w.n, w.mode, g_ctx.n_cu, st->stream);
  st->pending_widen.clear();
  return TGX_OK;
}

BatchFusion decide_fusion(const tgx_plan *plan, tgx_state *st, const tgx_column *dev, int64_t nrows,
                          const std::vector<BatchKeyFacts> *facts) {
  const int n_plan_cols = plan->n_columns_needed;
  BatchFusion f;
  f.kll_on_col.assign(n_plan_cols, -1);
  f.pair_of_col.assign(n_plan_cols, -1);
  f.hll_on_col.assign(n_plan_cols, -1);
  f.kll_fused.assign(plan->kll.size(), 0);
  f.como_fused.assign(plan->como.size(), 0);
  f.distinct_idle.assign(plan->distinct.size(), 0);
  f.key_facts = facts ? *facts : std::vector<BatchKeyFacts>(plan->distinct.size());
  f.dprep.resize(plan->distinct.size());
  f.stats_by_partition.assign(plan->scan.size(), -1);
  f.distinct_done.assign(plan->distinct.size(), 0);
  auto plain8 = [&](int col) { return is_numeric(dev[col].type) && dev[col].values != nullptr; };
  for (size_t q = 0; q < plan->hll.size(); q++) {
    const HllTask &t = plan->hll[q];
    const int type = dev[t.column].type;
    const bool numeric = is_numeric(type) || is_numeric32(type);
    const bool lane = numeric && plan->distinct[t.distinct_slot].approx_only && !plan->scan[t.scan_slot].variance;
    if (st->hll_mode[q] == 0) st->hll_mode[q] = lane ? 1 : 2;
    if (st->hll_mode[q] == 1) {
      if (dev[t.column].values) f.hll_on_col[t.column] = (int)q;
      f.distinct_idle[t.distinct_slot] = 1;
    }
  }
  auto has_hll = [&](int col) { return f.hll_on_col[col] >= 0; };
  if (nrows >= (1 << 20)) {
    for (size_t q = 0; q < plan->kll.size(); q++) {
      const int col = plan->kll[q].column;
      if (plain8(col) && !has_hll(col) && f.kll_on_col[col] < 0 && kll_scan_eligible(nrows)) {
        f.kll_on_col[col] = (int)q;
        f.kll_fused[q] = 1;
      }
    }
    for (size_t q = 0; q < plan->como.size() && f.fused_pairs.size() < (size_t)kMaxPairsPerLaunch; q++) {
      const int x = plan->como[q].col_x, y = plan->como[q].col_y;
      if (x == y || !plain8(x) || !plain8(y) || f.pair_of_col[x] >= 0 || f.pair_of_col[y] >= 0) continue;
      if (has_hll(x) || has_hll(y)) continue;
      const int sx = scan_slot_of(plan, x), sy = scan_slot_of(plan, y);
      if ((sx >= 0 && plan->scan[sx].variance) || (sy >= 0 && plan->scan[sy].variance)) continue;
      FusedPair fp;
      fp.como = (int)q;
      fp.x = x;
      fp.y = y;
      fill_scan_desc(dev[x], false, nullptr, &fp.dx);
      fill_scan_desc(dev[y], false, nullptr, &fp.dy);
      if (fp.dx.head != fp.dy.head || fp.dx.n_tiles != fp.dy.n_tiles) continue;
      f.pair_of_col[x] = f.pair_of_col[y] = (int)f.fused_pairs.size();
      f.como_fused[q] = 1;
      f.fused_pairs.push_back(fp);
    }
  }
  return f;
}

tgx_status early_key_passes(const tgx_plan *plan, tgx_state *st, const tgx_column *dev, const tgx_column *columns,
                            BatchFusion *f, tgx_error *err) {
  update_mark("fused");
  TGX_TRY(distinct_sample_all(st, dev, f->key_facts, err));
  update_mark("sampled");
  auto numeric_pass = [&](size_t q) {
    const DistinctTask &t = plan->distinct[q];
    return t.tuple.empty() && !f->distinct_idle[q] && is_numeric(dev[t.column].type) && dev[t.column].length > 0;
  };
  for (size_t q = 0; q < plan->distinct.size(); q++) {
    const DistinctTask &t = plan->distinct[q];
    if (!numeric_pass(q)) continue;
    TGX_TRY(distinct_prepare_numeric(st, q, dev[t.column], f->key_facts[q], &f->dprep[q], err));
    if (f->dprep[q].partitioned && dev[t.column].type == TGX_INT64 && t.scan_slot >= 0 &&
        !plan->scan[t.scan_slot].variance && f->pair_of_col[t.column] < 0 && f->kll_on_col[t.column] < 0)
      f->stats_by_partition[t.scan_slot] = (int)q;
  }
  update_mark("prepared");
  for (size_t q = 0; q < plan->distinct.size(); q++) {
    const DistinctTask &t = plan->distinct[q];
    if (!numeric_pass(q)) continue;
    TGX_TRY(distinct_update(st, q, dev[t.column], f->key_facts[q], f->dprep[q], err, nullptr, f->stats_slot(plan, q),
                            &columns[t.column]));
    f->distinct_done[q] = 1;
  }
  update_mark("keys_queued");
  if (!st->keys_ready) HIP_TRY(hipEventCreateWithFlags(&st->keys_ready, hipEventDisableTiming));
  HIP_TRY(hipEventRecord(st->keys_ready, st->stream));
  update_mark("event");
  bool all_early = true;
  for (size_t q = 0; q < plan->distinct.size(); q++) all_early &= f->distinct_done[q] || f->distinct_idle[q];
  for (size_t q = 0; q < plan->distinct.size(); q++) {
    const DistinctTask &t = plan->distinct[q];
    if (!f->distinct_done[q] || t.scan_slot < 0 || st->distinct[q].has_hint) continue;
    all_early &= f->stats_by_partition[t.scan_slot] == (int)q;
  }
  st->keys_ready_recorded = all_early && (st->passes == 0 || st->keys_ready_recorded);
  st->passes++;
  return TGX_OK;
}

enum class ScanLane { kPlain, kKll, kHll };
struct LaneColumns {
  std::vector<ScanColDesc> descs;
  std::vector<int32_t> acc_index;
  std::vector<int> kll_slots;
  void add(const ScanColDesc &d, int32_t acc, int kll = -1) {
    descs.push_back(d);
    acc_index.push_back(acc);
    if (kll >= 0) kll_slots.push_back(kll);
  }
};

tgx_status launch_scan_lane(tgx_state *st, ScanLane lane, const LaneColumns &cols, int64_t nrows, int scan_per_cu,
                            tgx_error *err) {
  for (size_t c0 = 0; c0 < cols.descs.size(); c0 += kMaxColsPerLaunch) {
    const int n = (int)std::min<size_t>(kMaxColsPerLaunch, cols.descs.size() - c0);
    ScanLaunch L;
    memset(&L, 0, sizeof(L));
    int blocks = 1;
    uint64_t chunk_bytes = 0;
    bool chunk_var = false;
    for (int k = 0; k < n; k++) {
      L.cols[k] = cols.descs[c0 + k];
      L.acc_index[k] = cols.acc_index[c0 + k];
      const int want = lane == ScanLane::kKll    ? fused_blocks(L.cols[k], n)
                       : lane == ScanLane::kHll ? scan_blocks_for(L.cols[k], n)
                                                : scan_blocks_for(L.cols[k], n, scan_per_cu);
      blocks = std::max(blocks, want);
      chunk_bytes += (uint64_t)L.cols[k].length * (L.cols[k].elem32 ? 4 : 8) +
                     (L.cols[k].validity ? (uint64_t)(L.cols[k].length + 7) / 8 : 0);
      chunk_var |= L.cols[k].want_variance != 0;
    }
    size_t lds = 0;
    if (lane == ScanLane::kKll)
      for (int k = 0; k < n; k++) {
        TGX_TRY(kll_scan_prepare(st, (size_t)cols.kll_slots[c0 + k], nrows, blocks * kWavesPerBlock,
                                 rows_per_wave(L.cols[k], blocks), &L.cols[k].kll, err));
        lds = std::max(lds, (size_t)kWavesPerBlock * (((size_t)1 << L.cols[k].kll.top) + kTileRows) * sizeof(double));
      }
    HIP_TRY(st->d_scan_partials.reserve((size_t)n * blocks * sizeof(ScanPartial)));
    if (lane == ScanLane::kHll) {
      HIP_TRY(st->d_hll_rows.reserve((size_t)n * blocks * kHllRegisters));
      for (int k = 0; k < n; k++) L.cols[k].hll = st->d_hll_rows.as<uint8_t>() + (size_t)k * blocks * kHllRegisters;
    }
    if (chunk_var)
      launch_scan_pivot(L, n, st->d_pivots.as<double>(), st->d_pivot_set.as<int32_t>(), st->d_pivot_search.as<PivotSearch>(),
                        st->stream);
    {
      ProfScope ps(st, "scan", chunk_bytes);
      if (lane == ScanLane::kPlain) {
        launch_scan_main_only(L, n, blocks, st->d_scan_partials.as<ScanPartial>(), st->d_scan_acc.as<ScanAcc>(),
                              st->stream);
      } else if (lane == ScanLane::kKll) {
        launch_scan_kll(L, n, blocks, lds, st->d_scan_partials.as<ScanPartial>(), st->stream);
      } else {
        ProfScope ps_hll(st, "scan_hll", chunk_bytes);
        launch_scan_hll(L, n, blocks, st->d_scan_partials.as<ScanPartial>(), st->stream);
      }
    }
    if (lane != ScanLane::kPlain || blocks > 1)
      launch_scan_reduce_only(L, n, blocks, st->d_scan_partials.as<ScanPartial>(), st->d_scan_acc.as<ScanAcc>(),
                              st->stream);
  }
  return TGX_OK;
}

ComomentColDesc como_desc(const tgx_column &x, const tgx_column &y) {
  ComomentColDesc d;
  d.x = x.values;
  d.y = y.values;
  d.xv = x.validity;
  d.yv = y.validity;
  d.xoff = x.offset;
  d.yoff = y.offset;
  d.length = x.length;
  d.x_is_float = x.type == TGX_FLOAT64;
  d.y_is_float = y.type == TGX_FLOAT64;
  return d;
}

tgx_status launch_fused_pairs(const tgx_plan *plan, tgx_state *st, const tgx_column *dev, int64_t nrows,
                              const BatchFusion &f, tgx_error *err) {
  std::vector<FusedPair> pairs = f.fused_pairs;
  const int n = (int)pairs.size();
  std::stable_sort(pairs.begin(), pairs.end(), [](const FusedPair &a, const FusedPair &b) {
    return 2 * a.dx.is_float + a.dy.is_float > 2 * b.dx.is_float + b.dy.is_float;
  });
  ScanPairLaunch PL;
  ScanLaunch RL;
  ComomentLaunch CL;
  memset(&PL, 0, sizeof(PL));
  memset(&RL, 0, sizeof(RL));
  memset(&CL, 0, sizeof(CL));
  int blocks = 1;
  uint64_t chunk_bytes = 0;
  for (int k = 0; k < n; k++) blocks = std::max(blocks, fused_blocks(pairs[k].dx, n));
  size_t lds = 0;
  for (int k = 0; k < n; k++) {
    FusedPair &fp = pairs[k];
    ScanPairDesc &P = PL.pairs[k];
    P.x = fp.dx;
    P.y = fp.dy;
    P.x_acc = scan_slot_of(plan, fp.x);
    P.y_acc = scan_slot_of(plan, fp.y);
    P.como_acc = fp.como;
    size_t rings = 0;
    for (int side = 0; side < 2; side++) {
      ScanColDesc &d = side ? P.y : P.x;
      const int col = side ? fp.y : fp.x;
      if (f.kll_on_col[col] >= 0) {
        TGX_TRY(kll_scan_prepare(st, (size_t)f.kll_on_col[col], nrows, blocks * kWavesPerBlock,
                                 rows_per_wave(d, blocks), &d.kll, err));
        rings += ((size_t)1 << d.kll.top) + kTileRows;
      }
      chunk_bytes += (uint64_t)d.length * 8 + (d.validity ? (uint64_t)(d.length + 7) / 8 : 0);
    }
    lds = std::max(lds, (size_t)kWavesPerBlock * rings * sizeof(double));
    RL.cols[2 * k] = P.x;
    RL.cols[2 * k + 1] = P.y;
    RL.acc_index[2 * k] = P.x_acc;
    RL.acc_index[2 * k + 1] = P.y_acc;
    CL.pairs[k] = como_desc(dev[fp.x], dev[fp.y]);
    CL.acc_index[k] = fp.como;
  }
  TGX_TRY(como_pivots(st, CL, n, err));
  HIP_TRY(st->d_scan_partials.reserve((size_t)2 * n * blocks * sizeof(ScanPartial)));
  HIP_TRY(st->d_como_partials.reserve((size_t)n * blocks * comoments_partial_bytes()));
  {
    ProfScope ps(st, "scan", chunk_bytes);
    launch_scan_pairs(PL, n, blocks, lds, st->d_scan_partials.as<ScanPartial>(), st->d_como_partials.p,
                      st->d_como_acc.as<ComomentAcc>(), st->stream);
  }
  launch_scan_reduce_only(RL, 2 * n, blocks, st->d_scan_partials.as<ScanPartial>(), st->d_scan_acc.as<ScanAcc>(),
                          st->stream);
  launch_comoments_reduce(CL, n, blocks, st->d_como_partials.p, st->d_como_acc.as<ComomentAcc>(), st->stream);
  return TGX_OK;
}

tgx_status scan_columns(const tgx_plan *plan, tgx_state *st, const tgx_column *dev, int64_t nrows,
                        const BatchFusion &f, tgx_error *err) {
  const int scan_per_cu = st->exchange_expected ? 6 : 8;
  LaneColumns plain, kll, hll;
  for (size_t s = 0; s < plan->scan.size(); s++) {
    const ScanTask &t = plan->scan[s];
    const tgx_column &c = dev[t.column];
    if (!is_numeric(c.type) && !is_numeric32(c.type)) {
      if (t.stats_spec)
        return fail(err, TGX_INVALID_ARGUMENT, "NUMERIC_STATS on non-numeric column %d (type %d)", t.column, c.type);
      continue;
    }
    if (f.pair_of_col[t.column] >= 0) continue;
    if (f.stats_by_partition[s] >= 0) continue;
    if (f.kll_on_col[t.column] < 0 && f.hll_on_col[t.column] < 0 && !t.read_by_spec) {
      bool all_hinted = true, any_distinct = false;
      for (size_t dd = 0; dd < plan->distinct.size(); dd++)
        if (plan->distinct[dd].scan_slot == (int)s) {
          any_distinct = true;
          all_hinted &= st->distinct[dd].has_hint;
        }
      if (any_distinct && all_hinted) continue;
    }
    ScanColDesc d;
    fill_scan_desc(c, t.variance, st->d_pivots.as<double>() + s, &d);
    if (f.hll_on_col[t.column] >= 0 && !t.variance) {
      d.skip_stats = t.stats_needed ? 0 : 1;
      d.hll_regs = st->d_hll.as<uint8_t>() + (size_t)f.hll_on_col[t.column] * kHllRegisters;
      hll.add(d, (int32_t)s);
    } else if (f.kll_on_col[t.column] >= 0) {
      kll.add(d, (int32_t)s, f.kll_on_col[t.column]);
    } else {
      plain.add(d, (int32_t)s);
    }
  }
  for (size_t q = 0; q < plan->kll.size(); q++) {
    const int col = plan->kll[q].column;
    if (!f.kll_fused[q] || f.pair_of_col[col] >= 0 || scan_slot_of(plan, col) >= 0) continue;
    ScanColDesc d;
    fill_scan_desc(dev[col], false, nullptr, &d);
    kll.add(d, -1, (int)q);
  }
  TGX_TRY(launch_scan_lane(st, ScanLane::kPlain, plain, nrows, scan_per_cu, err));
  TGX_TRY(launch_scan_lane(st, ScanLane::kKll, kll, nrows, scan_per_cu, err));
  TGX_TRY(launch_scan_lane(st, ScanLane::kHll, hll, nrows, scan_per_cu, err));
  if (!f.fused_pairs.empty()) TGX_TRY(launch_fused_pairs(plan, st, dev, nrows, f, err));
  return TGX_OK;
}

tgx_status count_validity(const tgx_plan *plan, tgx_state *st, const tgx_column *dev, tgx_error *err) {
  std::vector<CountColDesc> descs;
  std::vector<int32_t> index;
  int64_t max_words = 0;
  for (size_t s = 0; s < plan->count.size(); s++) {
    const tgx_column &c = dev[plan->count[s].column];
    if (c.type == TGX_DICT32_UTF8 && c.dictionary->validity && c.dictionary->length > 0) {
      launch_dict_count((const int32_t *)c.values, c.validity, c.offset, c.length, c.dictionary->validity,
                        c.dictionary->offset, c.dictionary->length, st->d_count_acc.as<CountAcc>() + s, g_ctx.n_cu,
                        st->stream);
      continue;
    }
    if (!c.validity) {
      st->h_count[s].total += c.length;
      st->h_count[s].non_null += c.length;
      continue;
    }
    descs.push_back({c.validity, c.offset, c.length});
    index.push_back((int32_t)s);
    max_words = std::max<int64_t>(max_words, (c.length + 63) / 64 + 1);
  }
  for (size_t c0 = 0; c0 < descs.size(); c0 += kMaxColsPerLaunch) {
    const int n = (int)std::min<size_t>(kMaxColsPerLaunch, descs.size() - c0);
    CountLaunch L;
    memset(&L, 0, sizeof(L));
    uint64_t chunk_bytes = 0;
    for (int k = 0; k < n; k++) {
      L.cols[k] = descs[c0 + k];
      L.acc_index[k] = index[c0 + k];
      chunk_bytes += (uint64_t)(L.cols[k].length + 7) / 8;
    }
    int blocks = (int)std::min<int64_t>(std::max<int64_t>(1, (max_words + 256 * 4 - 1) / (256 * 4)),
                                        std::max(8, (g_ctx.n_cu * 8) / n));
    HIP_TRY(st->d_count_blocks.reserve((size_t)n * blocks * sizeof(unsigned long long)));
    ProfScope ps(st, "count", chunk_bytes);
    launch_count(L, n, blocks, st->d_count_blocks.as<unsigned long long>(), st->d_count_acc.as<CountAcc>(), st->stream);
  }
  return TGX_OK;
}

tgx_status unfused_comoments(const tgx_plan *plan, tgx_state *st, const tgx_column *dev, int64_t nrows,
                             const BatchFusion &f, tgx_error *err) {
  std::vector<ComomentColDesc> descs;
  std::vector<int32_t> index;
  uint64_t bytes = 0;
  for (size_t s = 0; s < plan->como.size(); s++) {
    if (f.como_fused[s]) continue;
    const tgx_column &x = dev[plan->como[s].col_x], &y = dev[plan->como[s].col_y];
    if (!is_numeric(x.type) || !is_numeric(y.type))
      return fail(err, TGX_INVALID_ARGUMENT, "COMOMENTS needs numeric columns (%d, %d)", x.type, y.type);
    descs.push_back(como_desc(x, y));
    index.push_back((int32_t)s);
    bytes += (uint64_t)x.length * 16 + (x.validity ? (uint64_t)(x.length + 7) / 8 : 0) +
             (y.validity ? (uint64_t)(y.length + 7) / 8 : 0);
  }
  for (size_t c0 = 0; c0 < descs.size(); c0 += kMaxColsPerLaunch) {
    const int n = (int)std::min<size_t>(kMaxColsPerLaunch, descs.size() - c0);
    ComomentLaunch L;
    memset(&L, 0, sizeof(L));
    for (int k = 0; k < n; k++) {
      L.pairs[k] = descs[c0 + k];
      L.acc_index[k] = index[c0 + k];
    }
    int blocks = (int)std::min<int64_t>(std::max<int64_t>(1, (nrows + 256 * 16 - 1) / (256 * 16)),
                                        std::max(32, (g_ctx.n_cu * 12) / n));
    HIP_TRY(st->d_como_partials.reserve((size_t)n * blocks * comoments_partial_bytes()));
    TGX_TRY(como_pivots(st, L, n, err));
    ProfScope ps(st, "comoments", bytes * n / std::max<size_t>(descs.size(), 1));
    launch_comoments(L, n, blocks, st->d_como_partials.p, st->d_como_acc.as<ComomentAcc>(), st->stream);
  }
  return TGX_OK;
}

tgx_status late_key_sets(const tgx_plan *plan, tgx_state *st, const tgx_column *dev, const tgx_column *columns,
                         const BatchFusion &f, tgx_error *err) {
  DictFuse fuse;
  for (size_t s = 0; s < plan->distinct.size(); s++) {
    const DistinctTask &t = plan->distinct[s];
    if (!t.tuple.empty()) continue;
    const tgx_column &c = dev[t.column];
    if (c.type != TGX_DICT32_UTF8 || c.length == 0 || c.dictionary->length == 0 || c.dictionary->validity) continue;
    if (dict_usage_scratch_bytes(c.length, c.dictionary->length, t.multiplicity ? 1 : 0, g_ctx.n_cu) == 0) continue;
    const int cap = dict_fuse_capacity(c.length, c.dictionary->length, t.multiplicity ? 1 : 0, g_ctx.n_cu);
    if (cap > 0 && !fuse.capacity.count(t.column)) fuse.capacity[t.column] = cap;
  }
  TGX_TRY(regex_update(st, dev, err, &fuse));
  std::map<int, bool> fuse_done;
  for (size_t s = 0; s < plan->distinct.size(); s++)
    if (f.distinct_idle[s] || f.distinct_done[s]) {
      continue;
    } else if (plan->distinct[s].tuple.empty()) {
      const int col = plan->distinct[s].column;
      const std::vector<DictGather> *g = nullptr;
      auto it = fuse.by_column.find(col);
      if (it != fuse.by_column.end() && !fuse_done[col]) {
        g = &it->second;
        fuse_done[col] = true;
      }
      TGX_TRY(distinct_update(st, s, dev[col], f.key_facts[s], f.dprep[s], err, g, f.stats_slot(plan, s), &columns[col]));
    } else {
// ... 49 lines not shown
```

Measured before the change: 41.97 billion rows/s.

## Batch partition key passes across distinct columns into grouped kernel launches

Partitioned numeric distinct-count work is no longer launched column by column. Columns are collected into a key-pass batch, and init, partition, bucket-apply and key-stats reduce are each launched once per group. The partition kernel now loops over up to two columns, with a rotated starting tile so work spreads across workgroups, and bucket_apply assigns buckets from several columns to one grid. This aims to cut launch count and tail idle time, at the cost of more kernel complexity and a grid sized from the combined tile count.

```diff
diff --git a/term_amd/csrc/api_internal.h b/term_amd/csrc/api_internal.h
--- a/term_amd/csrc/api_internal.h
+++ b/term_amd/csrc/api_internal.h
@@ -59,6 +59,15 @@
   uint64_t n_buckets = 0;
   bool range_known = false;
   int64_t lo = 0, hi = 0;
+};
+
+struct KeyPassBatch {
+  struct Col {
+    PartitionParams pp;
+    uint64_t bytes;
+    int stats_slot;
+  };
+  std::vector<Col> cols;
 };
 
 struct BatchTraits {
@@ -164,7 +173,8 @@
 TGX_HIDDEN tgx_status distinct_update(tgx_state *st, size_t slot, const tgx_column &c, const BatchKeyFacts &facts,
                                   const NumericPrep &prep, tgx_error *err,
                                   const std::vector<DictGather> *gathers = nullptr, int stats_slot = -1,
-                                  const tgx_column *orig = nullptr);
+                                  const tgx_column *orig = nullptr, KeyPassBatch *batch = nullptr);
+TGX_HIDDEN tgx_status key_pass_run(tgx_state *st, const KeyPassBatch &batch, tgx_error *err);
 TGX_HIDDEN tgx_status pinned_readback(tgx_state *st, size_t bytes, tgx_error *err);
 TGX_HIDDEN tgx_status distinct_sample_all(tgx_state *st, const tgx_column *dev, std::vector<BatchKeyFacts> &facts,
                                       tgx_error *err);
diff --git a/term_amd/csrc/distinct_state.cpp b/term_amd/csrc/distinct_state.cpp
--- a/term_amd/csrc/distinct_state.cpp
+++ b/term_amd/csrc/distinct_state.cpp
@@ -652,10 +652,46 @@
   return TGX_OK;
 }
 
+tgx_status key_pass_run(tgx_state *st, const KeyPassBatch &batch, tgx_error *err) {
+  static_assert(kCntDistinct == 0 && kCntTwice == 1, "partition_init_kernel clears the two totals together");
+  for (size_t c0 = 0; c0 < batch.cols.size(); c0 += kMaxKeyPassCols) {
+    const int n = (int)std::min<size_t>(kMaxKeyPassCols, batch.cols.size() - c0);
+    KeyPassGroup all;
+    memset(&all, 0, sizeof(all));
+    all.n_cols = n;
+    uint64_t bytes = 0;
+    for (int k = 0; k < n; k++) {
+      all.cols[k] = batch.cols[c0 + k].pp;
+      bytes += batch.cols[c0 + k].bytes;
+    }
+    launch_partition_init(all, st->stream);
+    int grids[kMaxKeyPassCols] = {};
+    {
+      ProfScope ps(st, "distinct", bytes);
+      launch_partition(all, g_ctx.n_cu, grids, st->stream);
+      HIP_TRY(launch_bucket_apply(all, st->stream));
+    }
+    KeyStatsLaunch K;
+    memset(&K, 0, sizeof(K));
+    int n_stats = 0;
+    for (int k = 0; k < n; k++) {
+      if (batch.cols[c0 + k].stats_slot < 0) continue;
+      KeyStatsCol &s = K.cols[n_stats++];
+      s.partials = all.cols[k].stats;
+      s.outliers = all.cols[k].outliers;
+      s.length = all.cols[k].length;
+      s.n_partials = grids[k];
+      s.acc_index = batch.cols[c0 + k].stats_slot;
+    }
+    if (n_stats) launch_key_stats_reduce(K, n_stats, st->d_scan_acc.as<ScanAcc>(), st->stream);
+  }
+  return TGX_OK;
+}
+
 namespace {
 
 tgx_status distinct_run_numeric(tgx_state *st, size_t slot, const tgx_column &c, const NumericPrep &prep,
-                                       int stats_slot, tgx_error *err, const tgx_column *orig) {
+                                       int stats_slot, tgx_error *err, const tgx_column *orig, KeyPassBatch *batch) {
   const DistinctTask &task = st->plan->distinct[slot];
   const tgx_column &keep = (orig && orig->mem == TGX_MEM_DEVICE && is_widened(orig->type)) ? *orig : c;
   DistinctState &ds = st->distinct[slot];
@@ -708,29 +744,17 @@
       pp.cursors = ds.cursors.as<unsigned long long>();
       pp.seen = ds.seen.as<uint32_t>();
       pp.twice = mult ? ds.twice.as<uint32_t>() : nullptr;
-      const int grid = partition_grid(c.length, g_ctx.n_cu);
       if (stats_slot >= 0) {
-        HIP_TRY(ds.stat_partials.reserve((size_t)(grid + 1) * sizeof(ScanPartial)));
+        HIP_TRY(ds.stat_partials.reserve((size_t)(g_ctx.n_cu + 1) * sizeof(ScanPartial)));
         HIP_TRY(ds.outlier_stats.reserve(sizeof(OutlierStats)));
         pp.stats = ds.stat_partials.as<ScanPartial>();
         pp.outliers = ds.outlier_stats.as<OutlierStats>();
       }
-      unsigned long long *cnt = ds.counters.as<unsigned long long>();
-      static_assert(kCntDistinct == 0 && kCntTwice == 1, "partition_init_kernel clears the two totals together");
-      launch_partition_init(pp, cnt + kCntDistinct, st->stream);
-      {
-        ProfScope ps(st, "distinct", bytes);
-        launch_partition(pp, cnt, g_ctx.n_cu, st->stream);
-        HIP_TRY(launch_bucket_apply(pp, cnt, st->stream));
-      }
-      if (stats_slot >= 0) {
-        ScanLaunch L;
-        memset(&L, 0, sizeof(L));
-        L.cols[0].length = c.length;
-        L.cols[0].is_float = 0;
-        L.acc_index[0] = stats_slot;
-        launch_scan_reduce_only(L, 1, grid, pp.stats, st->d_scan_acc.as<ScanAcc>(), st->stream, pp.outliers);
-      }
+      pp.counters = ds.counters.as<unsigned long long>();
+      KeyPassBatch alone;
+      KeyPassBatch &into = batch ? *batch : alone;
+      into.cols.push_back({pp, bytes, stats_slot});
+      if (!batch) TGX_TRY(key_pass_run(st, alone, err));
     } else {
       ProfScope ps(st, "distinct", bytes);
       launch_distinct_bitmap(d, bitmap_view(ds), ds.counters.as<unsigned long long>(), st->stream);
@@ -776,7 +800,7 @@
 
 tgx_status distinct_update(tgx_state *st, size_t slot, const tgx_column &c, const BatchKeyFacts &facts,
                            const NumericPrep &prep, tgx_error *err, const std::vector<DictGather> *gathers,
-                           int stats_slot, const tgx_column *orig) {
+                           int stats_slot, const tgx_column *orig, KeyPassBatch *batch) {
   const DistinctTask &task = st->plan->distinct[slot];
   DistinctState &ds = st->distinct[slot];
   const bool mult = task.multiplicity;
@@ -844,7 +868,7 @@
   if (c.length == 0) return TGX_OK;
   NumericPrep ready = prep;
   if (!ready.prepared) TGX_TRY(distinct_prepare_numeric(st, slot, c, facts, &ready, err));
-  return distinct_run_numeric(st, slot, c, ready, stats_slot, err, orig);
+  return distinct_run_numeric(st, slot, c, ready, stats_slot, err, orig, batch);
 }
 
 tgx_status tgx::distinct_resolve(tgx_state *st, size_t slot, tgx_error *err) {
diff --git a/term_amd/csrc/internal.h b/term_amd/csrc/internal.h
--- a/term_amd/csrc/internal.h
+++ b/term_amd/csrc/internal.h
@@ -53,7 +53,8 @@
                              ComomentAcc *d_accs, hipStream_t stream);
 void launch_widen32(const void *src, void *dst, int64_t n, int mode, int n_cu, hipStream_t stream);
 void launch_scan_reduce_only(const ScanLaunch &L, int n_cols, int blocks_per_col, ScanPartial *d_partials,
-                             ScanAcc *d_accs, hipStream_t stream, const OutlierStats *outliers = nullptr);
+                             ScanAcc *d_accs, hipStream_t stream);
+void launch_key_stats_reduce(const KeyStatsLaunch &K, int n_cols, ScanAcc *d_accs, hipStream_t stream);
 void launch_count(const CountLaunch &L, int n_cols, int blocks_per_col, unsigned long long *d_block_counts,
                   CountAcc *d_accs, hipStream_t stream);
 size_t comoments_partial_bytes();
@@ -63,14 +64,14 @@
                           unsigned long long *d_counters, hipStream_t stream);
 void launch_distinct_bitmap(const DistinctColDesc &d, const BitmapView &bm,
                             unsigned long long *d_counters, hipStream_t stream);
-int partition_grid(int64_t length, int n_cu);
+int partition_grid(int64_t n_tiles, int n_cu);
 void launch_distinct_init(DistinctSample *sample, OutlierStats *outliers, hipStream_t stream);
-void launch_partition_init(const PartitionParams &p, unsigned long long *totals, hipStream_t stream);
+void launch_partition_init(const KeyPassGroup &all, hipStream_t stream);
 void launch_distinct_sample(const DistinctColDesc &d, DistinctSample *out, hipStream_t stream);
 void launch_distinct_outliers(const DistinctColDesc &d, int64_t base, uint64_t range, const HashSetView &t,
                               unsigned long long *d_counters, hipStream_t stream);
-void launch_partition(const PartitionParams &p, unsigned long long *d_counters, int n_cu, hipStream_t stream);
-hipError_t launch_bucket_apply(const PartitionParams &p, unsigned long long *d_counters, hipStream_t stream);
+void launch_partition(const KeyPassGroup &all, int n_cu, int *grids, hipStream_t stream);
+hipError_t launch_bucket_apply(const KeyPassGroup &all, hipStream_t stream);
 void launch_bitmap_adopt(const uint32_t *seen_slices, const uint32_t *twice_slices, uint32_t n_slices,
                          uint64_t slice_words, uint64_t stride_words, uint32_t *out_seen, uint32_t *out_twice,
                          unsigned long long *d_counters, hipStream_t stream);
diff --git a/term_amd/csrc/kernels/distinct_types.h b/term_amd/csrc/kernels/distinct_types.h
--- a/term_amd/csrc/kernels/distinct_types.h
+++ b/term_amd/csrc/kernels/distinct_types.h
@@ -104,6 +104,15 @@
   struct OutlierStats *outliers;
   uint32_t bucket0, n_lists;
   int32_t force_form;
+  unsigned long long *counters;
+};
+
+constexpr int kMaxKeyPassCols = 8;
+constexpr int kPartitionColsPerLaunch = 2;
+struct KeyPassGroup {
+  PartitionParams cols[kMaxKeyPassCols];
+  int32_t n_cols;
+  int32_t pad;
 };
 
 struct OutlierStats {
@@ -111,6 +120,17 @@
   unsigned long long lo32_sum;
   long long hi32_sum;
   unsigned long long count;
+};
+
+struct KeyStatsCol {
+  const struct ScanPartial *partials;
+  const OutlierStats *outliers;
+  int64_t length;
+  int32_t n_partials;
+  int32_t acc_index;
+};
+struct KeyStatsLaunch {
+  KeyStatsCol cols[kMaxKeyPassCols];
 };
 
 struct DistinctSample {
diff --git a/term_amd/csrc/kernels/partition.hip b/term_amd/csrc/kernels/partition.hip
--- a/term_amd/csrc/kernels/partition.hip
+++ b/term_amd/csrc/kernels/partition.hip
@@ -1,4 +1,6 @@
 #include <hip/hip_runtime.h>
+
+#include <string.h>
 
 #include <type_traits>
 
@@ -343,7 +345,7 @@
 
 template <int KPT, bool STATS>
 __device__ __forceinline__ void partition_relative_plain(const PartitionParams &p, const int64_t (&key)[KPT],
-                                                         uint32_t (&rel)[KPT], uint64_t &ok, unsigned long long &n_out) {
+                                                         uint32_t (&rel)[KPT], uint64_t &ok, uint32_t &n_out) {
 #pragma unroll
   for (int j = 0; j < KPT; j++) {
     const uint64_t r = (uint64_t)key[j] - (uint64_t)p.base;
@@ -388,10 +390,7 @@
 }
 
 template <int THREADS, int KPT, int MAXP, int PAD, bool VALIDITY, bool KEY16, bool STATS, bool FORM_CLUSTERED, bool PACK20 = false>
-__global__ __launch_bounds__(THREADS) __attribute__((amdgpu_waves_per_eu(4, 4))) void partition_kernel(
-    PartitionParams p, unsigned long long *counters) {
-  if ((p.force_form ? p.force_form == 2 : __builtin_amdgcn_readfirstlane((int)p.cursors[2 * p.n_buckets]) != 0) != FORM_CLUSTERED)
-    return;
+__global__ __launch_bounds__(THREADS) __attribute__((amdgpu_waves_per_eu(4, 4))) void partition_kernel(KeyPassGroup g) {
   constexpr int kTile = THREADS * KPT;
   __shared__ uint32_t sorted[kTile];
   __shared__ uint32_t hist[MAXP];
@@ -400,13 +399,22 @@
   __shared__ uint32_t wave_sums[16];
   __shared__ uint32_t long_runs[kTile / 1024 + 1];
   __shared__ uint32_t t_lo, t_hi;
-  const bool wide = (((uintptr_t)p.values + (uintptr_t)p.offset * 8) & 15) == 0;
-  unsigned long long n_valid = 0, n_out = 0;
-  const int64_t n_tiles = (p.length + kTile - 1) / kTile;
-  uint32_t rel[KPT];
   __shared__ uint32_t st_min, st_max;
   __shared__ unsigned long long st_sum, st_cnt;
   __shared__ OutlierStats st_out;
+  uint32_t next_wg = 0;
+#pragma unroll
+  for (int col = 0; col < kPartitionColsPerLaunch; col++) {
+  if (col >= g.n_cols) break;
+  const PartitionParams &p = g.cols[col];
+  if ((p.force_form ? p.force_form == 2 : __builtin_amdgcn_readfirstlane((int)p.cursors[2 * p.n_buckets]) != 0) != FORM_CLUSTERED)
+    continue;
+  const bool wide = (((uintptr_t)p.values + (uintptr_t)p.offset * 8) & 15) == 0;
+  uint32_t n_valid = 0, n_out = 0;
+  const int64_t n_tiles = (p.length + kTile - 1) / kTile;
+  const int64_t first_tile = (blockIdx.x + gridDim.x - next_wg) % gridDim.x;
+  next_wg = (next_wg + (uint32_t)n_tiles % gridDim.x) % gridDim.x;
+  uint32_t rel[KPT];
   if (STATS && threadIdx.x == 0) {
     st_min = 0xFFFFFFFFu;
     st_max = 0;
@@ -421,7 +429,7 @@
   if (STATS) __syncthreads();
   auto tile_loop = [&](auto clustered_tag) __attribute__((always_inline)) {
   constexpr bool CLUSTERED = decltype(clustered_tag)::value;
-  for (int64_t tile = blockIdx.x; tile < n_tiles; tile += gridDim.x) {
+  for (int64_t tile = first_tile; tile < n_tiles; tile += gridDim.x) {
     uint64_t ok;
     {
       int64_t key[KPT];
@@ -559,16 +567,21 @@
       }
     }
   }
-  block_add2_any(n_valid, n_out, &counters[kCntValidRows], &counters[kCntOutOfRange]);
+  block_add2_any((unsigned long long)n_valid, (unsigned long long)n_out, &p.counters[kCntValidRows], &p.counters[kCntOutOfRange]);
+  __syncthreads();
+  }
 }
 
 
 template <int LDS_WORDS, bool KEY16 = false, bool PACK20 = false>
-__global__ __launch_bounds__(kPartitionThreads) void bucket_apply_kernel(PartitionParams p,
-                                                                         unsigned long long *counters) {
+__global__ __launch_bounds__(kPartitionThreads) void bucket_apply_kernel(KeyPassGroup g) {
   __shared__ __attribute__((aligned(16))) uint32_t lds[LDS_WORDS];
   const uint32_t tid = threadIdx.x;
-  const uint32_t b = blockIdx.x;
+  uint32_t b = blockIdx.x;
+  int col = 0;
+  while (col + 1 < g.n_cols && b >= g.cols[col].n_buckets) b -= g.cols[col++].n_buckets;
+  const PartitionParams &p = g.cols[col];
+  unsigned long long *counters = p.counters;
   const uint32_t slice_words = (uint32_t)((1ull << p.sub_bits) >> 5);
   uint32_t *l_seen = lds;
   uint32_t *l_twice = lds + slice_words;
@@ -731,7 +744,9 @@
   block_add2_any(n_seen, n_twice, &counters[kCntDistinct], &counters[kCntTwice]);
 }
 
-__global__ __launch_bounds__(1024) void partition_init_kernel(PartitionParams p, unsigned long long *totals) {
+__global__ __launch_bounds__(1024) void partition_init_kernel(KeyPassGroup g) {
+  const PartitionParams &p = g.cols[blockIdx.x];
+  unsigned long long *totals = p.counters;
   unsigned long long *cursors = p.cursors;
   const uint32_t n_buckets = p.n_buckets;
   OutlierStats *outliers = p.outliers;
@@ -800,70 +815,77 @@
   }
 }
 
-int partition_grid(int64_t length, int n_cu) {
-  int64_t n_tiles = (length + kPartitionTile - 1) / kPartitionTile;
+int partition_grid(int64_t n_tiles, int n_cu) {
   int grid = (int)(n_tiles < (int64_t)n_cu ? n_tiles : (int64_t)n_cu);
   return grid < 1 ? 1 : grid;
 }
 
-void launch_partition(const PartitionParams &p, unsigned long long *d_counters, int n_cu,
-                      hipStream_t stream) {
-  const int grid = partition_grid(p.length, n_cu);
-  const bool plain = p.force_form != 2, in_order = p.force_form != 1;
-#define TGX_PART(VAL, K16, ST)                                                                                      \
-  do {                                                                                                              \
-    if (plain)                                                                                                      \
-      hipLaunchKernelGGL((partition_kernel<kPartitionThreads, kPartitionKeysPerThread, (int)kMaxPartitions, kRunPad4, VAL, K16, ST, false>), \
-                         dim3(grid), dim3(kPartitionThreads), 0, stream, p, d_counters);                            \
-    if (in_order)                                                                                                   \
-      hipLaunchKernelGGL((partition_kernel<kPartitionThreads, kPartitionKeysPerThread, (int)kMaxPartitions, kRunPad4, VAL, K16, ST, true>), \
-                         dim3(grid), dim3(kPartitionThreads), 0, stream, p, d_counters);                            \
-  } while (0)
-#define TGX_PART20(VAL, ST)                                                                                         \
-  do {                                                                                                              \
-    if (plain)                                                                                                      \
-      hipLaunchKernelGGL((partition_kernel<kPartitionThreads, kPartitionKeysPerThread, (int)kMaxPartitions, kRunPad4, VAL, false, ST, false, true>), \
-                         dim3(grid), dim3(kPartitionThreads), 0, stream, p, d_counters);                            \
-    if (in_order)                                                                                                   \
-      hipLaunchKernelGGL((partition_kernel<kPartitionThreads, kPartitionKeysPerThread, (int)kMaxPartitions, kRunPad4, VAL, false, ST, true, true>), \
-                         dim3(grid), dim3(kPartitionThreads), 0, stream, p, d_counters);                            \
-  } while (0)
-  if (p.key16 == 2) {
-    if (p.stats) {
-      if (p.validity) TGX_PART20(true, true); else TGX_PART20(false, true);
-    } else {
-      if (p.validity) TGX_PART20(true, false); else TGX_PART20(false, false);
-    }
-    return;
-  }
-  if (p.stats) {
-    if (p.key16) {
-      if (p.validity) TGX_PART(true, true, true); else TGX_PART(false, true, true);
-    } else {
-      if (p.validity) TGX_PART(true, false, true); else TGX_PART(false, false, true);
-    }
-  } else if (p.key16) {
-    if (p.validity) TGX_PART(true, true, false); else TGX_PART(false, true, false);
-  } else {
-    if (p.validity) TGX_PART(true, false, false); else TGX_PART(false, false, false);
-  }
-#undef TGX_PART
-#undef TGX_PART20
-}
-
-hipError_t launch_bucket_apply(const PartitionParams &p, unsigned long long *d_counters,
-                               hipStream_t stream) {
-  const size_t words = ((size_t)1 << p.sub_bits) / 32 * (p.want_multiplicity ? 2 : 1);
-  const dim3 grid(p.n_buckets), block(kPartitionThreads);
-#define TGX_APPLY(W)                                                                                  \
-  if (words <= W) {                                                                                   \
-    if (p.key16 == 2)                                                                                 \
-      hipLaunchKernelGGL((bucket_apply_kernel<W, false, true>), grid, block, 0, stream, p, d_counters); \
-    else if (p.key16)                                                                                 \
-      hipLaunchKernelGGL((bucket_apply_kernel<W, true>), grid, block, 0, stream, p, d_counters);      \
-    else                                                                                              \
-      hipLaunchKernelGGL((bucket_apply_kernel<W, false>), grid, block, 0, stream, p, d_counters);     \
-    return hipGetLastError();                                                                         \
+namespace {
+
+template <bool VAL, bool K16, bool ST, bool P20>
+void launch_partition_forms(const KeyPassGroup &g, int grid, bool plain, bool in_order, hipStream_t stream) {
+  if (plain)
+    hipLaunchKernelGGL((partition_kernel<kPartitionThreads, kPartitionKeysPerThread, (int)kMaxPartitions, kRunPad4, VAL, K16, ST, false, P20>),
+                       dim3(grid), dim3(kPartitionThreads), 0, stream, g);
+  if (in_order)
+    hipLaunchKernelGGL((partition_kernel<kPartitionThreads, kPartitionKeysPerThread, (int)kMaxPartitions, kRunPad4, VAL, K16, ST, true, P20>),
+                       dim3(grid), dim3(kPartitionThreads), 0, stream, g);
+}
+template <bool VAL, bool ST>
+void launch_partition_format(const KeyPassGroup &g, int grid, bool plain, bool in_order, hipStream_t stream) {
+  const int32_t format = g.cols[0].key16;
+  if (format == 2)
+    launch_partition_forms<VAL, false, ST, true>(g, grid, plain, in_order, stream);
+  else if (format == 1)
+    launch_partition_forms<VAL, true, ST, false>(g, grid, plain, in_order, stream);
+  else
+    launch_partition_forms<VAL, false, ST, false>(g, grid, plain, in_order, stream);
+}
+
+int partition_instance(const PartitionParams &p) { return p.key16 * 4 + (p.stats ? 2 : 0); }
+
+}
+
+void launch_partition(const KeyPassGroup &all, int n_cu, int *grids, hipStream_t stream) {
+  bool done[kMaxKeyPassCols] = {};
+  for (int c0 = 0; c0 < all.n_cols; c0++) {
+    if (done[c0]) continue;
+    KeyPassGroup g;
+    memset(&g, 0, sizeof(g));
+    const int inst = partition_instance(all.cols[c0]);
+    int members[kPartitionColsPerLaunch];
+    int64_t n_tiles = 0;
+    bool plain = false, in_order = false;
+    bool val = false;
+    for (int c = c0; c < all.n_cols && g.n_cols < kPartitionColsPerLaunch; c++) {
+      if (done[c] || partition_instance(all.cols[c]) != inst) continue;
+      done[c] = true;
+      members[g.n_cols] = c;
+      g.cols[g.n_cols++] = all.cols[c];
+      n_tiles += (all.cols[c].length + kPartitionTile - 1) / kPartitionTile;
+      plain |= all.cols[c].force_form != 2;
+      in_order |= all.cols[c].force_form != 1;
+      val |= all.cols[c].validity != nullptr;
+    }
+    const int grid = partition_grid(n_tiles, n_cu);
+    for (int k = 0; k < g.n_cols; k++) grids[members[k]] = grid;
+    const bool st = (inst & 2) != 0;
+    if (val && st) launch_partition_format<true, true>(g, grid, plain, in_order, stream);
+    else if (val) launch_partition_format<true, false>(g, grid, plain, in_order, stream);
+    else if (st) launch_partition_format<false, true>(g, grid, plain, in_order, stream);
+    else launch_partition_format<false, false>(g, grid, plain, in_order, stream);
+  }
+}
+
+namespace {
+
+template <bool K16, bool P20>
+hipError_t launch_bucket_apply_format(const KeyPassGroup &g, size_t words, uint32_t n_blocks, hipStream_t stream) {
+  const dim3 grid(n_blocks), block(kPartitionThreads);
+#define TGX_APPLY(W)                                                                       \
+  if (words <= W) {                                                                        \
+    hipLaunchKernelGGL((bucket_apply_kernel<W, K16, P20>), grid, block, 0, stream, g);     \
+    return hipGetLastError();                                                              \
   }
   TGX_APPLY(1024)
   TGX_APPLY(2048)
@@ -875,8 +897,36 @@
   return hipErrorInvalidValue;
 }
 
-void launch_partition_init(const PartitionParams &p, unsigned long long *totals, hipStream_t stream) {
-  hipLaunchKernelGGL(partition_init_kernel, dim3(1), dim3(1024), 0, stream, p, totals);
-}
-
-}
+}
+
+hipError_t launch_bucket_apply(const KeyPassGroup &all, hipStream_t stream) {
+  for (int32_t format = 0; format < 3; format++) {
+    KeyPassGroup g;
+    memset(&g, 0, sizeof(g));
+    size_t words = 0;
+    uint32_t n_blocks = 0;
+    for (int c = 0; c < all.n_cols; c++) {
+      const PartitionParams &p = all.cols[c];
+      if (p.key16 != format) continue;
+      int at = g.n_cols++;
+      auto expected = [](const PartitionParams &q) { return q.length / (int64_t)(q.n_lists ? q.n_lists : 1); };
+      for (; at > 0 && expected(g.cols[at - 1]) < expected(p); at--) g.cols[at] = g.cols[at - 1];
+      g.cols[at] = p;
+      const size_t w = ((size_t)1 << p.sub_bits) / 32 * (p.want_multiplicity ? 2 : 1);
+      words = w > words ? w : words;
+      n_blocks += p.n_buckets;
+    }
+    if (g.n_cols == 0) continue;
+    const hipError_t e = format == 2   ? launch_bucket_apply_format<false, true>(g, words, n_blocks, stream)
+                         : format == 1 ? launch_bucket_apply_format<true, false>(g, words, n_blocks, stream)
+                                       : launch_bucket_apply_format<false, false>(g, words, n_blocks, stream);
+    if (e != hipSuccess) return e;
+  }
+  return hipSuccess;
+}
+
+void launch_partition_init(const KeyPassGroup &all, hipStream_t stream) {
+  hipLaunchKernelGGL(partition_init_kernel, dim3(all.n_cols), dim3(1024), 0, stream, all);
+}
+
+}
diff --git a/term_amd/csrc/kernels/scan.hip b/term_amd/csrc/kernels/scan.hip
--- a/term_amd/csrc/kernels/scan.hip
+++ b/term_amd/csrc/kernels/scan.hip
@@ -1028,16 +1028,10 @@
   pair_body<XF, YF, KLL>(P, ox, oy, oc, wave, lane, pvx, pvy);
 }
 
-__global__ __launch_bounds__(64) void scan_reduce_kernel(const ScanLaunch L,
-                                                          const ScanPartial *__restrict__ partials,
-                                                          int blocks_per_col,
-                                                          ScanAcc *__restrict__ accs,
-                                                          const OutlierStats *__restrict__ outliers) {
-  const int col = blockIdx.x;
+__device__ __forceinline__ void reduce_column_partials(const ScanColDesc &c, const ScanPartial *__restrict__ p,
+                                                       int blocks_per_col, ScanAcc &acc,
+                                                       const OutlierStats *__restrict__ outliers) {
   const int lane = threadIdx.x;
-  if (L.acc_index[col] < 0) return;
-  const ScanColDesc c = L.cols[col];
-  const ScanPartial *p = partials + (size_t)col * blocks_per_col;
   LaneAcc a;
   acc_init(a);
   if (outliers && lane == 0 && outliers->count) {
@@ -1077,7 +1071,25 @@
     LaneAcc b = acc_shfl_down(a, d);
     acc_merge(a, b, c.is_float);
   }
-  if (lane == 0) scan_fold(accs[L.acc_index[col]], a, c);
+  if (lane == 0) scan_fold(acc, a, c);
+}
+
+__global__ __launch_bounds__(64) void scan_reduce_kernel(const ScanLaunch L,
+                                                          const ScanPartial *__restrict__ partials,
+                                                          int blocks_per_col,
+                                                          ScanAcc *__restrict__ accs) {
+  const int col = blockIdx.x;
+  if (L.acc_index[col] < 0) return;
+  const ScanColDesc c = L.cols[col];
+  reduce_column_partials(c, partials + (size_t)col * blocks_per_col, blocks_per_col, accs[L.acc_index[col]], nullptr);
+}
+
+__global__ __launch_bounds__(64) void key_stats_reduce_kernel(const KeyStatsLaunch K, ScanAcc *__restrict__ accs) {
+  const KeyStatsCol k = K.cols[blockIdx.x];
+  ScanColDesc c;
+  memset(&c, 0, sizeof(c));
+  c.length = k.length;
+  reduce_column_partials(c, k.partials, k.n_partials, accs[k.acc_index], k.outliers);
 }
 
 __global__ __launch_bounds__(256) void scan_pivot_kernel(const ScanLaunch L,
@@ -1378,9 +1390,12 @@
 }
 
 void launch_scan_reduce_only(const ScanLaunch &L, int n_cols, int blocks_per_col, ScanPartial *d_partials,
-                             ScanAcc *d_accs, hipStream_t stream, const OutlierStats *outliers) {
-  hipLaunchKernelGGL(scan_reduce_kernel, dim3(n_cols), dim3(64), 0, stream, L, d_partials, blocks_per_col,
-                     d_accs, outliers);
+                             ScanAcc *d_accs, hipStream_t stream) {
+  hipLaunchKernelGGL(scan_reduce_kernel, dim3(n_cols), dim3(64), 0, stream, L, d_partials, blocks_per_col, d_accs);
+}
+
+void launch_key_stats_reduce(const KeyStatsLaunch &K, int n_cols, ScanAcc *d_accs, hipStream_t stream) {
+  hipLaunchKernelGGL(key_stats_reduce_kernel, dim3(n_cols), dim3(64), 0, stream, K, d_accs);
 }
 
 void launch_count(const CountLaunch &L, int n_cols, int blocks_per_col, unsigned long long *d_block_counts,
diff --git a/term_amd/csrc/update.cpp b/term_amd/csrc/update.cpp
--- a/term_amd/csrc/update.cpp
+++ b/term_amd/csrc/update.cpp
@@ -493,13 +493,15 @@
       f->stats_by_partition[t.scan_slot] = (int)q;
   }
   update_mark("prepared");
+  KeyPassBatch key_pass;
   for (size_t q = 0; q < plan->distinct.size(); q++) {
     const DistinctTask &t = plan->distinct[q];
     if (!numeric_pass(q)) continue;
     TGX_TRY(distinct_update(st, q, dev[t.column], f->key_facts[q], f->dprep[q], err, nullptr, f->stats_slot(plan, q),
-                            &columns[t.column]));
+                            &columns[t.column], &key_pass));
     f->distinct_done[q] = 1;
   }
+  if (!key_pass.cols.empty()) TGX_TRY(key_pass_run(st, key_pass, err));
   update_mark("keys_queued");
   if (!st->keys_ready) HIP_TRY(hipEventCreateWithFlags(&st->keys_ready, hipEventDisableTiming));
   HIP_TRY(hipEventRecord(st->keys_ready, st->stream));
```

Measured after the change: 41.70 billion rows/s. No clear change (-0.6%).
